# sangminwoo/SVOL

Hardware: AMD Instinct MI355X
Metric: frames/sec (fwd+matcher+bwd), T=32·P=196·d=256 (higher is better)
Workload: dtype bf16

## Files before the change

### include/svol_hip.h

```cpp
#ifndef SVOL_HIP_H
#define SVOL_HIP_H

#include <stdint.h>

#ifdef __cplusplus
extern "C" {
#endif

#define SVOL_F32 0
#define SVOL_BF16 1
#define SVOL_F16 2

#define SVOL_OK 0
#define SVOL_E_INVALID (-1)
#define SVOL_E_UNSUPPORTED (-2)
#define SVOL_E_LAUNCH (-3)

#define SVOL_ACT_NONE 0
#define SVOL_ACT_RELU 1
#define SVOL_ACT_GELU 2
#define SVOL_ACT_SIGMOID 3
#define SVOL_ACT_GELU_D 5
#define SVOL_ACT_RELU_RES 4

int svol_abi_version(void);
const char* svol_strerror(int code);

int svol_cast(const void* src, int dtype_src, void* dst, int dtype_dst, int64_t n, void* stream);
int svol_cast_transpose(const float* src, void* dst, void* dstT, int dtype, int64_t R, int64_t C, void* stream);
int svol_cast_transpose_multi(const void* descs, int32_t n_desc, int64_t total_tiles, int dtype, void* stream);
int svol_cast_split(const float* src, int64_t ld_src, void* dst_hilo, int64_t R, int64_t C, void* stream);

int svol_adamw_flat(float* p, const float* g, float* m, float* v, int64_t n, float lr, float beta1, float beta2, float eps,
                    float weight_decay, int64_t step, float grad_scale, void* stream);
int svol_adamw_flat_zero(float* p, float* g, float* m, float* v, int64_t n, float lr, float beta1, float beta2, float eps,
                         float weight_decay, int64_t step, float grad_scale, void* stream);
int svol_grad_finite(const float* g, int64_t n, float* scaler_state, void* stream);
int svol_adamw_flat_scaled(float* p, const float* g, float* m, float* v, int64_t n, float lr, float beta1, float beta2, float eps,
                           float weight_decay, float grad_mul, const float* scaler_state, void* stream);
int svol_loss_scaler_update(float* scaler_state, float growth_factor, float backoff_factor, int64_t growth_interval, float min_scale,
                            float max_scale, void* stream);
int svol_sgd_flat(float* p, const float* g, float* buf, int64_t n, float lr, float momentum, float weight_decay, float grad_scale,
                  void* stream);
int svol_sgd_flat_zero(float* p, float* g, float* buf, int64_t n, float lr, float momentum, float weight_decay, float grad_scale,
                       void* stream);
int svol_sgd_flat_scaled(float* p, const float* g, float* buf, int64_t n, float lr, float momentum, float weight_decay, float grad_mul,
                         const float* scaler_state, void* stream);
int svol_adam_flat(float* p, const float* g, float* m, float* v, int64_t n, float lr, float beta1, float beta2, float eps,
                   float weight_decay, int64_t step, float grad_scale, void* stream);
int svol_adam_flat_zero(float* p, float* g, float* m, float* v, int64_t n, float lr, float beta1, float beta2, float eps,
                        float weight_decay, int64_t step, float grad_scale, void* stream);
int svol_adam_flat_scaled(float* p, const float* g, float* m, float* v, int64_t n, float lr, float beta1, float beta2, float eps,
                          float weight_decay, float grad_mul, const float* scaler_state, void* stream);
int64_t svol_grad_sqnorm_ws_bytes(int64_t n);
int svol_grad_sqnorm(const float* g, int64_t n, float* ws, float* out, void* stream);
int svol_grad_clip_state(const float* sq, int32_t nb, float grad_mul, float max_norm, float loss_scale, int64_t steps_taken,
                         float* scaler_state, float* state_out, void* stream);
int svol_sgd_flat_grouped(float* p, float* g, float* buf, int64_t n, const int32_t* seg_end, const int32_t* seg_group, int32_t nseg,
                          const float* hyper, int32_t ngroups, const float* state, float grad_mul, int zero, void* stream);
int svol_adam_flat_grouped(float* p, float* g, float* m, float* v, int64_t n, const int32_t* seg_end, const int32_t* seg_group,
                           int32_t nseg, const float* hyper, int32_t ngroups, const float* state, const float* step_count,
                           float grad_mul, int zero, void* stream);
int svol_adamw_flat_grouped(float* p, float* g, float* m, float* v, int64_t n, const int32_t* seg_end, const int32_t* seg_group,
                            int32_t nseg, const float* hyper, int32_t ngroups, const float* state, const float* step_count,
                            float grad_mul, int zero, void* stream);
int svol_flat_step_advance(float* step_count, const float* state, void* stream);
int svol_ema_flat(float* ema, const float* p, int64_t n, float decay, int warmup, int64_t step, const float* state,
                  const float* step_count, void* stream);

int svol_gemm_nt(const void* A, int64_t lda, const void* A2, int64_t n_split, const void* B, int64_t ldb,
                 void* C, int64_t ldc, const float* bias, const float* colscale, int act, void* pre_act_out,
                 int64_t ldp, const void* residual, int64_t ldr, int out_f32, int64_t M, int64_t N, int64_t K,
                 int dtype, void* stream);
int svol_gemm_nt_split(const void* A, int64_t lda, const void* W_hilo, int64_t ldw, void* C, int64_t ldc, const float* bias,
                       int64_t M, int64_t N, int64_t K, void* stream);
int svol_gemm_nt_dgelu(const void* A, int64_t lda, const void* B, int64_t ldb, void* C, int64_t ldc,
                       const void* pre, int64_t ldp, float* colsum, int64_t M, int64_t N, int64_t K, int dtype,
                       void* stream);
int svol_gemm_nt_dact(const void* A, int64_t lda, const void* B, int64_t ldb, void* C, int64_t ldc,
                      const void* aux, int64_t ldaux, int act, float* colsum, int64_t M, int64_t N, int64_t K,
                      int dtype, void* stream);

int svol_gemm_tn(const void* A, int64_t lda, const void* B, int64_t ldb, float* C, int64_t ldc, float* colsum,
                 int64_t Mc, int64_t N, int64_t K, int dtype, void* stream);
#define SVOL_TN_GROUP_MAX 6
typedef struct svol_tn_problem {
    const void* A; int64_t lda;
    const void* B; int64_t ldb;
    float* C; int64_t ldc;
    float* colsum;
    int64_t Mc, N, K;
} svol_tn_problem;
int svol_gemm_tn_grouped(const svol_tn_problem* problems, int32_t n, int dtype, void* stream);
int svol_colsum(const void* X, int64_t ldx, float* out, int64_t M, int64_t N, int dtype, void* stream);
int svol_act_bwd(const void* dy, const void* aux, void* dpre, int act, int64_t n, int dtype, void* stream);

int svol_layernorm_fwd(const void* x, int x_f32, const float* gamma, const float* beta, float* y32, void* y,
                       void* ypos, const void* pos, int64_t pos_rows, float* mean, float* rstd, int64_t M, int64_t D,
                       float dropout_p, uint64_t seed, const int64_t* seed_offset_dev, int dtype, void* stream);
int svol_layernorm_bwd(const float* dy32, const void* dy, const void* dy2, const void* x, int x_f32,
                       const float* gamma, const float* mean, const float* rstd, float* dx32, void* dx,
                       float* dgamma, float* dbeta, float* dx_colsum, int64_t M, int64_t D, float dropout_p,
                       uint64_t seed, const int64_t* seed_offset_dev, int dtype, void* stream);

int svol_dropout(const void* x, void* y, int64_t n, int64_t row_len, float p, uint64_t seed, int dtype, void* stream);
int svol_dropout_add(const float* t32, const float* res32, float* out32, int64_t n, int64_t row_len, float p, uint64_t seed, void* stream);
int svol_dropout_sd(const void* x, void* y, int64_t n, int64_t row_len, float p, uint64_t seed, const int64_t* seed_step_dev, int dtype,
                    void* stream);
int svol_dropout_add_sd(const float* t32, const float* res32, float* out32, int64_t n, int64_t row_len, float p, uint64_t seed,
                        const int64_t* seed_step_dev, void* stream);

int svol_posenc_sine(const float* mask, void* pos, int64_t B, int64_t L, int64_t D, int dtype, void* stream);

int64_t svol_attn_ws_bytes(int64_t B, int64_t H, int64_t Lq, int64_t Lk, int64_t dh);
int svol_attn_fwd(const void* q, int64_t ldq, const void* k, int64_t ldk, const void* v, int64_t ldv, void* o,
                  int64_t ldo, float* lse2, const float* kbias, int64_t B, int64_t H, int64_t Lq, int64_t Lk,
                  int64_t dh, float scale, float q_premul, void* ws, int64_t ws_bytes, int dtype, void* stream);
int svol_attn_bwd(const void* q, int64_t ldq, const void* k, int64_t ldk, const void* v, int64_t ldv, const void* o,
                  int64_t ldo, const void* d_o, int64_t lddo, const float* lse2, float* delta, const float* kbias,
                  void* dq, int64_t lddq, void* dk, int64_t lddk, void* dv, int64_t lddv, int64_t B, int64_t H,
                  int64_t Lq, int64_t Lk, int64_t dh, float scale, float q_premul, void* ws, int64_t ws_bytes,
                  int dtype, void* stream);

#define SVOL_ATTN_DQ_PREZEROED 1
int64_t svol_attn_bwd_sp_image_bytes(int64_t B, int64_t H, int64_t Lq, int64_t Lk, int64_t dh, int64_t ws_bytes, int dtype);
int svol_attn_bwd_zero_ws(void* ws, int64_t ws_bytes, int64_t B, int64_t H, int64_t Lq, int64_t Lk, int64_t dh, int dtype, void* stream);
int svol_attn_bwd_ex(const void* q, int64_t ldq, const void* k, int64_t ldk, const void* v, int64_t ldv, const void* o,
                     int64_t ldo, const void* d_o, int64_t lddo, const float* lse2, float* delta, const float* kbias,
                     void* dq, int64_t lddq, void* dk, int64_t lddk, void* dv, int64_t lddv, int64_t B, int64_t H,
                     int64_t Lq, int64_t Lk, int64_t dh, float scale, float q_premul, void* ws, int64_t ws_bytes,
                     int dtype, int flags, void* ev_prep, void* stream);

int svol_attn_fwd_dropout(const void* q, int64_t ldq, const void* k, int64_t ldk, const void* v, int64_t ldv, void* o,
                          int64_t ldo, float* lse2, const float* kbias, int64_t B, int64_t H, int64_t Lq, int64_t Lk,
                          int64_t dh, float scale, float q_premul, void* ws, int64_t ws_bytes, float dropout_p, uint64_t seed,
                          int dtype, void* stream);
int svol_attn_bwd_dropout(const void* q, int64_t ldq, const void* k, int64_t ldk, const void* v, int64_t ldv, const void* o,
                          int64_t ldo, const void* d_o, int64_t lddo, const float* lse2, float* delta, const float* kbias,
                          void* dq, int64_t lddq, void* dk, int64_t lddk, void* dv, int64_t lddv, int64_t B, int64_t H,
                          int64_t Lq, int64_t Lk, int64_t dh, float scale, float q_premul, void* ws, int64_t ws_bytes,
                          float dropout_p, uint64_t seed, int dtype, void* stream);
int svol_attn_fwd_dropout_sd(const void* q, int64_t ldq, const void* k, int64_t ldk, const void* v, int64_t ldv, void* o,
                             int64_t ldo, float* lse2, const float* kbias, int64_t B, int64_t H, int64_t Lq, int64_t Lk,
                             int64_t dh, float scale, float q_premul, void* ws, int64_t ws_bytes, float dropout_p, uint64_t seed,
                             const int64_t* seed_step_dev, int dtype, void* stream);
int svol_attn_bwd_dropout_sd(const void* q, int64_t ldq, const void* k, int64_t ldk, const void* v, int64_t ldv, const void* o,
                             int64_t ldo, const void* d_o, int64_t lddo, const float* lse2, float* delta, const float* kbias,
                             void* dq, int64_t lddq, void* dk, int64_t lddk, void* dv, int64_t lddv, int64_t B, int64_t H,
                             int64_t Lq, int64_t Lk, int64_t dh, float scale, float q_premul, void* ws, int64_t ws_bytes,
                             float dropout_p, uint64_t seed, const int64_t* seed_step_dev, int dtype, void* stream);

int svol_gate_fwd(const float* x32, const void* pos, const float* u, const float* gamma, const float* beta,
                  float* y32, void* y, void* ypos, float* a, float* mean, float* rstd, float* ws, int64_t B,
                  int64_t L, int64_t D, int64_t H, int dtype, void* stream);
int svol_gate_bwd(const float* dy32, const void* dy, const void* dy2, const float* x32, const void* pos,
                  const float* u, const float* gamma, const float* a, const float* mean, const float* rstd,
                  const float* ws, float* ws2, float* dx32, float* du, float* dgamma, float* dbeta, int64_t B,
                  int64_t L, int64_t D, int64_t H, int dtype, void* stream);

int svol_layernorm_gate_scores_fwd(const float* x32, const float* gamma, const float* beta, float* y32, void* y, void* ypos,
                                   const void* pos, float* mean, float* rstd, const float* u_next, float* scores_next,
                                   int64_t B, int64_t L, int64_t D, int64_t H, int dtype, void* stream);
int svol_gate_fwd_scored(const float* x32, const void* pos, const float* u, const float* gamma, const float* beta,
                         float* y32, void* y, void* ypos, float* a, float* mean, float* rstd, float* ws, int64_t B,
                         int64_t L, int64_t D, int64_t H, int dtype, void* stream);

int svol_gate_vectors_fwd(const float* skch, const float* W_in, const float* b_in, float* q_out, float* u_out, int64_t B, int64_t D,
                          int64_t H, void* stream);
int svol_gate_vectors_bwd(const float* du, const float* skch, const float* W_in, const float* q, float* dq_ws, float* dskch,
                          float* dW_in, float* db_in, int64_t B, int64_t D, int64_t H, void* stream);
#define SVOL_GATE_VEC_MAX_LAYERS 8
int svol_gate_vectors_fwd_multi(const float* skch, const float* const* W_in, const float* const* b_in, float* const* q_out,
                                float* const* u_out, int64_t n_layers, int64_t B, int64_t D, int64_t H, void* stream);
int svol_gate_vectors_bwd_multi(const float* const* du, const float* skch, const float* const* W_in, const float* const* q,
                                float* const* dq_ws, float* const* dskch, float* const* dW_in, float* const* db_in, int64_t n_layers,
                                int64_t B, int64_t D, int64_t H, void* stream);

int svol_match_cost(const float* logits, const float* boxes, const float* tgt_boxes, const int32_t* pred_off,
                    const int32_t* pred_cnt, const int32_t* tgt_off, const int32_t* tgt_cnt,
                    const int64_t* cost_off, float* cost, int32_t n_problems, float w_bbox, float w_giou,
                    float w_class, int32_t* box_status, void* stream);
int svol_lsap_batched(const float* cost, const int64_t* cost_off, const int32_t* pred_off, const int32_t* pred_cnt,
                      const int32_t* tgt_off, const int32_t* tgt_cnt, int32_t* match, int32_t* status,
                      int32_t n_problems, int32_t max_dim, void* stream);
int svol_heads_fwd(const float* hs, const float* Wc, const float* bc, const float* W0, const float* b0, const float* W1, const float* b1,
                   const float* W2, const float* b2, float* logits, float* h1, float* h2, float* boxes, int64_t R, int64_t D, void* stream);
int svol_heads_bwd(const float* dlogits, const float* dboxes, const float* hs, const float* h1, const float* h2, const float* boxes,
                   const float* Wc, const float* W0, const float* W1, const float* W2, float* dhs, float* gp0, float* gp1, float* dWc,
                   float* dbc, float* dW2, float* db2, int64_t R, int64_t D, void* stream);
int svol_set_loss_bwd(const float* g_label, const float* g_bbox, const float* g_giou, const float* dl, float* dlogits, float* dboxes,
                      int64_t n_layers, int64_t rows_per_layer, void* stream);
int svol_weighted_total(const float* x, const float* w, int64_t n, float* out, void* stream);
int svol_weighted_total_bwd(const float* w, const float* dout, int64_t n, float* dx, void* stream);
int svol_lsap_solve(const double* cost, int64_t nr, int64_t nc, int64_t* rows, int64_t* cols);
int svol_set_loss(const float* logits, const float* boxes, const float* tgt_boxes, const int32_t* match,
                  float* losses, float* g_label, float* g_bbox, float* g_giou, int32_t n_layers,
                  int32_t rows_per_layer, float eos_coef, const int32_t* rebase_vid_off, int32_t rows_per_video,
                  const int32_t* status, const int32_t* box_status, int32_t problems_per_layer, void* stream);

int svol_postprocess(const float* logits, const float* boxes, float* out, int64_t B, int64_t N, int64_t chunk, void* stream);
int svol_eval_max_iou(const double* pred_box, const int32_t* pred_off, const double* gt_box, const int32_t* gt_off,
                      const int32_t* gt_rec, double* out, int64_t n_gt, int32_t k, void* stream);
int svol_eval_ap(const double* pred_box, const double* pred_score, const int32_t* pred_frame, const int32_t* grp_pred_off,
                 const double* gt_box, const int32_t* gt_frame, const int32_t* grp_gt_off, const double* thresholds,
                 int32_t n_thresholds, int32_t* ws_order, unsigned char* ws_u8, double* ws_f64, double* ap, int64_t n_pred,
                 int64_t n_gt, int64_t n_groups, void* stream);

int svol_ingest_resize(const uint8_t* src, int64_t n, int64_t H, int64_t W, int64_t s_n, int64_t s_h, int64_t s_w,
                       const int32_t* xtab, int64_t kx, const int32_t* ytab, int64_t ky, const float* lut, const uint8_t* flip,
                       void* out, int64_t o_n, int64_t o_c, int64_t o_h, int64_t o_w, int64_t OH, int64_t OW, int out_dtype,
                       void* stream);
int svol_ingest_resample(const uint8_t* src, int64_t n, int64_t H, int64_t W, int64_t s_n, int64_t s_h, int64_t s_w, int src_channels,
                         int invert, const int32_t* xtab, int64_t kx, const int32_t* ytab, int64_t ky, const float* lut,
                         const uint8_t* flip, void* out, int64_t o_n, int64_t o_c, int64_t o_h, int64_t o_w, int64_t OH, int64_t OW,
                         int out_dtype, void* stream);

int svol_patchify(const float* pixel_values, void* out, int64_t n, int64_t C, int64_t H, int64_t W, int64_t p, int dtype,
                  void* stream);
int svol_vit_embed(const float* patch_proj, const float* cls_token, const float* pos_embed, float* x32, void* x, int64_t n,
                   int64_t P, int64_t D, int dtype, void* stream);
int svol_im2col(const void* x, int64_t sn, int64_t sh, int64_t sw, int64_t sc, int src_dtype, void* cols, int64_t ldcols,
                int64_t N, int64_t H, int64_t W, int64_t C, int64_t kh, int64_t kw, int64_t stride, int64_t pad, int dtype,
                void* stream);
int svol_conv_nhwc(const void* x, const void* w, int64_t ldw, void* y, const float* bias, int act, const void* residual,
                   int64_t N, int64_t H, int64_t W, int64_t C, int64_t Cout, int64_t kh, int64_t kw, int64_t stride,
                   int64_t pad, int dtype, void* stream);
int svol_maxpool_nhwc(const void* x, void* y, int64_t N, int64_t H, int64_t W, int64_t C, int64_t k, int64_t stride,
                      int64_t pad, int dtype, void* stream);
int svol_avgpool_nhwc(const void* x, float* y, int64_t N, int64_t HW, int64_t C, int dtype, void* stream);
int svol_bn_colstats(const void* z, const float* shift, float shift_scale, float* sum, float* sumsq, int64_t M, int64_t C, int dtype,
                     void* stream);
int svol_bn_finalize(const float* sum, const float* sumsq_centered, const float* pivot, const float* gamma, const float* beta,
                     float* running_mean, float* running_var, float momentum, float eps, int64_t M, int64_t C, float* mean, float* rstd,
                     float* scale, float* shift, void* stream);
int svol_conv_weight_pack(const float* w, void* out, int64_t Cout, int64_t Cin, int64_t kh, int64_t kw, int64_t Kp, int flip, int dtype,
                          void* stream);
int svol_conv_weight_unpack_add(const float* dwp, float* grad, int64_t Cout, int64_t Cin, int64_t kh, int64_t kw, int64_t Kp, void* stream);
int svol_conv_wgrad_nhwc(const void* dz, const void* x, float* dwp, int64_t N, int64_t H, int64_t W, int64_t C, int64_t Cout, int64_t kh, int64_t kw,
                         int64_t stride, int64_t pad, int64_t Kp, int dtype, void* stream);
int svol_bn_apply(const void* z, const float* scale, const float* shift, const void* residual, int relu, void* y, int64_t M, int64_t C,
                  int dtype, void* stream);
int svol_bn_bwd_reduce(const void* dy, const void* y, const void* z, const float* mean, const float* rstd, float* sum_g, float* sum_gx,
                       int64_t M, int64_t C, int dtype, void* stream);
int svol_bn_bwd_apply(const void* dy, const void* y, const void* z, const float* mean, const float* rstd, const float* gamma,
                      const float* sum_g, const float* sum_gx, void* dz, void* dres, int64_t M, int64_t C, int dtype, void* stream);
int svol_col2im_nhwc(const void* dcols, int64_t ldcols, void* dx, int64_t N, int64_t H, int64_t W, int64_t C, int64_t kh, int64_t kw,
                     int64_t stride, int64_t pad, int dtype, void* stream);
int svol_maxpool_idx_nhwc(const void* x, void* y, uint8_t* idx, int64_t N, int64_t H, int64_t W, int64_t C, int64_t k, int64_t stride,
                          int64_t pad, int dtype, void* stream);
int svol_maxpool_bwd_nhwc(const void* dy, const uint8_t* idx, void* dx, int64_t N, int64_t H, int64_t W, int64_t C, int64_t k,
                          int64_t stride, int64_t pad, int dtype, void* stream);
int svol_attn_weights_mean(const void* q, int64_t ldq, const void* k, int64_t ldk, const float* lse2, const float* kbias,
                           float* att, int64_t B, int64_t H, int64_t Lq, int64_t Lk, int64_t dh, float scale,
                           float q_premul, int dtype, void* stream);
int svol_attn_small_fwd(const void* q, int64_t ldq, const void* k, int64_t ldk, const void* v, int64_t ldv, void* o, int64_t ldo,
                        int64_t n_seq, int64_t H, int64_t L, int64_t dh, float scale, int dtype, void* stream);
int svol_attn_small_fwd_lse(const void* q, int64_t ldq, const void* k, int64_t ldk, const void* v, int64_t ldv, void* o, int64_t ldo,
                            float* lse2, int64_t n_seq, int64_t H, int64_t L, int64_t dh, float scale, int dtype, void* stream);
int svol_attn_small_bwd(const void* q, int64_t ldq, const void* k, int64_t ldk, const void* v, int64_t ldv, const void* o, int64_t ldo,
                        const void* dout, int64_t lddo, const float* lse2, void* dq, int64_t lddq, void* dk, int64_t lddk, void* dv,
                        int64_t lddv, int64_t n_seq, int64_t H, int64_t L, int64_t dh, float scale, int dtype, void* stream);
int svol_attn_small_fwd_h16(const void* q, int64_t ldq, const void* k, int64_t ldk, const void* v, int64_t ldv, void* o, int64_t ldo,
                            int64_t n_seq, int64_t H, int64_t L, int64_t dh, float scale, int dtype, void* stream);
int svol_attn_small_fwd_lse_h16(const void* q, int64_t ldq, const void* k, int64_t ldk, const void* v, int64_t ldv, void* o, int64_t ldo,
                                float* lse2, int64_t n_seq, int64_t H, int64_t L, int64_t dh, float scale, int dtype, void* stream);
int svol_attn_small_bwd_h16(const void* q, int64_t ldq, const void* k, int64_t ldk, const void* v, int64_t ldv, const void* o, int64_t ldo,
                            const void* dout, int64_t lddo, const float* lse2, void* dq, int64_t lddq, void* dk, int64_t lddk, void* dv,
                            int64_t lddv, int64_t n_seq, int64_t H, int64_t L, int64_t dh, float scale, int dtype, void* stream);

int svol_attn_cls_fwd(const void* q, int64_t ldq, const void* k, int64_t ldk, const void* v, int64_t ldv, void* o, int64_t ldo, float* lse2,
                      int64_t n, int64_t H, int64_t L, int64_t dh, float scale, int dtype, void* stream);
int svol_attn_cls_bwd(const void* q, int64_t ldq, const void* k, int64_t ldk, const void* v, int64_t ldv, const void* o, int64_t ldo,
                      const void* dout, int64_t lddo, const float* lse2, void* dq, int64_t lddq, void* dk, int64_t lddk, void* dv,
                      int64_t lddv, int64_t n, int64_t H, int64_t L, int64_t dh, float scale, int dtype, void* stream);
int svol_attn_cls_fwd_h16(const void* q, int64_t ldq, const void* k, int64_t ldk, const void* v, int64_t ldv, void* o, int64_t ldo, float* lse2,
                          int64_t n, int64_t H, int64_t L, int64_t dh, float scale, int dtype, void* stream);
int svol_attn_cls_bwd_h16(const void* q, int64_t ldq, const void* k, int64_t ldk, const void* v, int64_t ldv, const void* o, int64_t ldo,
                          const void* dout, int64_t lddo, const float* lse2, void* dq, int64_t lddq, void* dk, int64_t lddk, void* dv,
                          int64_t lddv, int64_t n, int64_t H, int64_t L, int64_t dh, float scale, int dtype, void* stream);
int64_t svol_attn_fewkeys_chunk_rows(int64_t Lq);
int64_t svol_attn_fewkeys_ws_bytes(int64_t B, int64_t H, int64_t Lq, int64_t Lk, int64_t dh);
int svol_attn_fewkeys_fwd(const void* q, int64_t ldq, const void* k, int64_t ldk, const void* v, int64_t ldv, void* o, int64_t ldo, float* lse2,
                          const float* kbias, int64_t B, int64_t H, int64_t Lq, int64_t Lk, int64_t dh, float scale, float q_premul, int dtype,
                          void* stream);
int svol_attn_fewkeys_bwd(const void* q, int64_t ldq, const void* k, int64_t ldk, const void* v, int64_t ldv, const void* o, int64_t ldo,
                          const void* d_o, int64_t lddo, const float* lse2, const float* kbias, void* dq, int64_t lddq, void* dk, int64_t lddk,
                          void* dv, int64_t lddv, int64_t B, int64_t H, int64_t Lq, int64_t Lk, int64_t dh, float scale, float q_premul,
                          void* ws, int64_t ws_bytes, int dtype, void* stream);
int svol_softmax_xent(const float* logits, int64_t ld, const int64_t* targets, float* loss, float* dlogits, int64_t lddl, int32_t* correct,
                      int64_t n, int64_t C, void* stream);


#define SVOL_DIM_B 0
#define SVOL_DIM_L 1
#define SVOL_DIM_N 2
#define SVOL_DIM_D 3
#define SVOL_DIM_H 4
#define SVOL_DIM_F 5
#define SVOL_DIM_DTYPE 6
#define SVOL_DIM_QDTYPE 7
#define SVOL_DIM_ATTN_WS_BYTES 8
#define SVOL_DIM_COUNT 9

#define SVOL_BLK_VIDEO_HALF 0
#define SVOL_BLK_QUERY_SELF 1
#define SVOL_BLK_QUERY_CROSS 2
const char* svol_block_slot_names(int block);
int svol_block_trace_dump(char* buf, int64_t cap);
int svol_clock_probe(uint64_t* samples, int32_t* count, int32_t max_samples, const int32_t* stop, int64_t period_us,
                     int64_t max_ms, int32_t* wall_khz, void* stream);


#define SVOL_VH_SLOTS(X) \
    X(X32) X(POS) X(U) X(G1) X(BT1) X(G2) X(BT2) X(G3) X(BT3) X(B_IN) X(B_O) X(B_FC1) X(B_FC2) X(QSCALE) \
    X(W_IN) X(WV_HILO) X(W_O) X(W_FC1) X(W_FC2) X(W_IN_T) X(W_O_T) X(W_FC1_T) X(W_FC2_T) \
    X(Y1) X(Y1POS) X(A) X(MEAN1) X(RSTD1) X(GATE_WS) X(GATE_PRE) X(U_NEXT) X(GATE_WS_NEXT) \
    X(QKV) X(O) X(LSE) X(S2) X(Y2) X(MEAN2) X(RSTD2) X(PRE) X(HID) X(S3) \
    X(MEAN3) X(RSTD3) X(M32) X(M) X(MPOS) X(Y1_32) X(Y2_32) X(ATTN_WS) \
    X(DM32) X(DM) X(DMPOS) X(DS32_3) X(DS3) X(DPRE) X(DY2) X(DS32_2) X(G2D) X(DO) X(DQKV) X(DELTA) X(DXQP) X(DXQ) X(GATE_WS2) \
    X(DX32) X(DU) \
    X(DG1) X(DBT1) X(DG2) X(DBT2) X(DG3) X(DBT3) X(DW_IN) X(DB_IN) X(DW_O) X(DB_O) X(DW_FC1) X(DB_FC1) X(DW_FC2) X(DB_FC2) \
    X(EV_A0) X(EV_A1) X(EV_CLEAN_IN) X(EV_PREP) X(ATTN_WS_NEXT) X(ZERO_STREAM) X(EV_CLEAN_OUT)
#define SVOL_QS_SLOTS(X) \
    X(O32) X(O) X(OPOS) X(QPOS) X(B_IN) X(B_O) X(G4) X(BT4) X(QSCALE) X(W_IN) X(WV_HILO) X(W_O) X(W_IN_T) X(W_O_T) \
    X(QKV) X(OA) X(LSE) X(S4) X(MEAN4) X(RSTD4) X(Y32) X(Y) X(YPOS) X(ATTN_WS) \
    X(DY32) X(DY) X(DYPOS) X(G) X(DOA) X(DQKV) X(DELTA) X(DO32) X(DXQ) X(DXQP) X(DQPOS) \
    X(DW_IN) X(DB_IN) X(DW_O) X(DB_O) X(DG4) X(DBT4)
#define SVOL_QC_SLOTS(X) \
    X(O32) X(O) X(OPOS) X(MV) X(MPOS) X(KBIAS) X(QPOS) X(B_IN) X(B_O) X(G5) X(BT5) X(B_FC1) X(B_FC2) X(G6) X(BT6) X(QSCALE) \
    X(W_INQ) X(W_INQ_T) X(W_KV) X(W_KV_T) X(WV_HILO) X(W_O) X(W_O_T) X(W_FC1) X(W_FC1_T) X(W_FC2) X(W_FC2_T) \
    X(Q) X(QC) X(KV) X(OA) X(OAQ) X(LSE) X(S5) X(Y5_32) X(Y5) X(MEAN5) X(RSTD5) X(PRE) X(HID) X(S6) X(MEAN6) X(RSTD6) \
    X(Y32) X(Y) X(YPOS) X(ATTN_WS) \
    X(DY32) X(DY) X(DYPOS) X(DS32_6) X(DS6) X(DPRE) X(DY5) X(DS32_5) X(G5D) X(DOAQ) X(DOA) X(DQC) X(DQ) X(DKV) X(DELTA) \
    X(DO32) X(DXQP) X(DMPOS) X(DMV) X(DQPOS) \
    X(DW_IN) X(DB_IN) X(DW_O) X(DB_O) X(DG5) X(DBT5) X(DW_FC1) X(DB_FC1) X(DW_FC2) X(DB_FC2) X(DG6) X(DBT6)
#define SVOL_SLOT_ENUM_VH(n) SVOL_VH_##n,
#define SVOL_SLOT_ENUM_QS(n) SVOL_QS_##n,
#define SVOL_SLOT_ENUM_QC(n) SVOL_QC_##n,
enum { SVOL_VH_SLOTS(SVOL_SLOT_ENUM_VH) SVOL_VH_COUNT };
enum { SVOL_QS_SLOTS(SVOL_SLOT_ENUM_QS) SVOL_QS_COUNT };
enum { SVOL_QC_SLOTS(SVOL_SLOT_ENUM_QC) SVOL_QC_COUNT };

int svol_video_half_fwd(const int64_t* dims, void* const* slots, void* stream);
int svol_video_half_bwd(const int64_t* dims, void* const* slots, int phase, void* stream);
int svol_video_half_wgrad(const int64_t* dims, void* const* slots, void* stream);
int svol_video_half_wgrad_part(const int64_t* dims, void* const* slots, int part, void* stream);
int svol_query_self_fwd(const int64_t* dims, void* const* slots, void* stream);
int svol_query_self_bwd(const int64_t* dims, void* const* slots, void* stream);
int svol_query_self_wgrad(const int64_t* dims, void* const* slots, void* stream);
int svol_query_cross_fwd(const int64_t* dims, void* const* slots, void* stream);
int svol_query_cross_bwd(const int64_t* dims, void* const* slots, void* stream);
int svol_query_cross_wgrad(const int64_t* dims, void* const* slots, void* stream);

#ifdef __cplusplus
}
#endif
#endif
```

### svol_amd/_lib.py

```python
from __future__ import annotations

import ctypes
import os

_HERE = os.path.dirname(os.path.abspath(__file__))
LIB_PATH = os.path.join(_HERE, 'libsvol_hip.so')

_p = ctypes.c_void_p
_i64 = ctypes.c_int64
_i32 = ctypes.c_int32
_int = ctypes.c_int
_f32 = ctypes.c_float
_u64 = ctypes.c_uint64

SIGNATURES = {
    'svol_block_trace_dump': [ctypes.c_char_p, _i64],
    'svol_lsap_solve': [_p, _i64, _i64, _p, _p],
    'svol_heads_fwd': [_p] * 13 + [_i64, _i64, _p],
    'svol_heads_bwd': [_p] * 17 + [_i64, _i64, _p],
    'svol_set_loss_bwd': [_p] * 6 + [_i64, _i64, _p],
    'svol_weighted_total': [_p, _p, _i64, _p, _p],
    'svol_weighted_total_bwd': [_p, _p, _i64, _p, _p],
    'svol_cast': [_p, _int, _p, _int, _i64, _p],
    'svol_cast_transpose': [_p, _p, _p, _int, _i64, _i64, _p],
    'svol_cast_split': [_p, _i64, _p, _i64, _i64, _p],
    'svol_gemm_nt_split': [_p, _i64, _p, _i64, _p, _i64, _p, _i64, _i64, _i64, _p],
    'svol_gemm_nt': [_p, _i64, _p, _i64, _p, _i64, _p, _i64, _p, _p, _int, _p, _i64, _p, _i64, _int, _i64, _i64, _i64,
                     _int, _p],
    'svol_gemm_nt_dgelu': [_p, _i64, _p, _i64, _p, _i64, _p, _i64, _p, _i64, _i64, _i64, _int, _p],
    'svol_gemm_nt_dact': [_p, _i64, _p, _i64, _p, _i64, _p, _i64, _int, _p, _i64, _i64, _i64, _int, _p],
    'svol_gemm_tn': [_p, _i64, _p, _i64, _p, _i64, _p, _i64, _i64, _i64, _int, _p],
    'svol_gemm_tn_grouped': [_p, _i32, _int, _p],
    'svol_colsum': [_p, _i64, _p, _i64, _i64, _int, _p],
    'svol_act_bwd': [_p, _p, _p, _int, _i64, _int, _p],
    'svol_layernorm_fwd': [_p, _int, _p, _p, _p, _p, _p, _p, _i64, _p, _p, _i64, _i64, _f32, _u64, _p, _int, _p],
    'svol_layernorm_bwd': [_p, _p, _p, _p, _int, _p, _p, _p, _p, _p, _p, _p, _p, _i64, _i64, _f32, _u64, _p, _int, _p],
    'svol_cast_transpose_multi': [_p, _int, _i64, _int, _p],
    'svol_postprocess': [_p, _p, _p, _i64, _i64, _i64, _p],
    'svol_eval_max_iou': [_p, _p, _p, _p, _p, _p, _i64, _int, _p],
    'svol_eval_ap': [_p, _p, _p, _p, _p, _p, _p, _p, _int, _p, _p, _p, _p, _i64, _i64, _i64, _p],
    'svol_patchify': [_p, _p, _i64, _i64, _i64, _i64, _i64, _int, _p],
    'svol_vit_embed': [_p, _p, _p, _p, _p, _i64, _i64, _i64, _int, _p],
    'svol_ingest_resize': [_p, _i64, _i64, _i64, _i64, _i64, _i64, _p, _i64, _p, _i64, _p, _p, _p, _i64, _i64, _i64, _i64, _i64, _i64, _int, _p],
    'svol_ingest_resample': [_p, _i64, _i64, _i64, _i64, _i64, _i64, _int, _int, _p, _i64, _p, _i64, _p, _p, _p, _i64, _i64, _i64, _i64, _i64, _i64, _int, _p],
    'svol_adamw_flat': [_p, _p, _p, _p, _i64, _f32, _f32, _f32, _f32, _f32, _i64, _f32, _p],
    'svol_adamw_flat_zero': [_p, _p, _p, _p, _i64, _f32, _f32, _f32, _f32, _f32, _i64, _f32, _p],
    'svol_grad_finite': [_p, _i64, _p, _p],
    'svol_adamw_flat_scaled': [_p, _p, _p, _p, _i64, _f32, _f32, _f32, _f32, _f32, _f32, _p, _p],
    'svol_loss_scaler_update': [_p, _f32, _f32, _i64, _f32, _f32, _p],
    'svol_sgd_flat': [_p, _p, _p, _i64, _f32, _f32, _f32, _f32, _p],
    'svol_sgd_flat_zero': [_p, _p, _p, _i64, _f32, _f32, _f32, _f32, _p],
    'svol_sgd_flat_scaled': [_p, _p, _p, _i64, _f32, _f32, _f32, _f32, _p, _p],
    'svol_adam_flat': [_p, _p, _p, _p, _i64, _f32, _f32, _f32, _f32, _f32, _i64, _f32, _p],
    'svol_adam_flat_zero': [_p, _p, _p, _p, _i64, _f32, _f32, _f32, _f32, _f32, _i64, _f32, _p],
    'svol_adam_flat_scaled': [_p, _p, _p, _p, _i64, _f32, _f32, _f32, _f32, _f32, _f32, _p, _p],
    'svol_grad_sqnorm_ws_bytes': [_i64],
    'svol_grad_sqnorm': [_p, _i64, _p, _p, _p],
    'svol_grad_clip_state': [_p, _i32, _f32, _f32, _f32, _i64, _p, _p, _p],
    'svol_sgd_flat_grouped': [_p, _p, _p, _i64, _p, _p, _i32, _p, _i32, _p, _f32, _int, _p],
    'svol_adam_flat_grouped': [_p, _p, _p, _p, _i64, _p, _p, _i32, _p, _i32, _p, _p, _f32, _int, _p],
    'svol_adamw_flat_grouped': [_p, _p, _p, _p, _i64, _p, _p, _i32, _p, _i32, _p, _p, _f32, _int, _p],
    'svol_flat_step_advance': [_p, _p, _p],
    'svol_ema_flat': [_p, _p, _i64, _f32, _int, _i64, _p, _p, _p],
    'svol_conv_nhwc': [_p, _p, _i64, _p, _p, _int, _p, _i64, _i64, _i64, _i64, _i64, _i64, _i64, _i64, _i64, _int, _p],
    'svol_im2col': [_p, _i64, _i64, _i64, _i64, _int, _p, _i64, _i64, _i64, _i64, _i64, _i64, _i64, _i64, _i64, _int, _p],
    'svol_maxpool_nhwc': [_p, _p, _i64, _i64, _i64, _i64, _i64, _i64, _i64, _int, _p],
    'svol_avgpool_nhwc': [_p, _p, _i64, _i64, _i64, _int, _p],
    'svol_bn_colstats': [_p, _p, _f32, _p, _p, _i64, _i64, _int, _p],
    'svol_bn_finalize': [_p, _p, _p, _p, _p, _p, _p, _f32, _f32, _i64, _i64, _p, _p, _p, _p, _p],
    'svol_conv_weight_pack': [_p, _p, _i64, _i64, _i64, _i64, _i64, _int, _int, _p],
    'svol_conv_weight_unpack_add': [_p, _p, _i64, _i64, _i64, _i64, _i64, _p],
    'svol_conv_wgrad_nhwc': [_p, _p, _p, _i64, _i64, _i64, _i64, _i64, _i64, _i64, _i64, _i64, _i64, _int, _p],
    'svol_bn_apply': [_p, _p, _p, _p, _int, _p, _i64, _i64, _int, _p],
    'svol_bn_bwd_reduce': [_p, _p, _p, _p, _p, _p, _p, _i64, _i64, _int, _p],
    'svol_bn_bwd_apply': [_p, _p, _p, _p, _p, _p, _p, _p, _p, _p, _i64, _i64, _int, _p],
    'svol_col2im_nhwc': [_p, _i64, _p, _i64, _i64, _i64, _i64, _i64, _i64, _i64, _i64, _int, _p],
    'svol_maxpool_idx_nhwc': [_p, _p, _p, _i64, _i64, _i64, _i64, _i64, _i64, _i64, _int, _p],
    'svol_maxpool_bwd_nhwc': [_p, _p, _p, _i64, _i64, _i64, _i64, _i64, _i64, _i64, _int, _p],
    'svol_attn_weights_mean': [_p, _i64, _p, _i64, _p, _p, _p, _i64, _i64, _i64, _i64, _i64, _f32, _f32, _int, _p],
    'svol_attn_small_fwd': [_p, _i64, _p, _i64, _p, _i64, _p, _i64, _i64, _i64, _i64, _i64, _f32, _int, _p],
    'svol_attn_small_fwd_lse': [_p, _i64, _p, _i64, _p, _i64, _p, _i64, _p, _i64, _i64, _i64, _i64, _f32, _int, _p],
    'svol_attn_small_bwd': [_p, _i64, _p, _i64, _p, _i64, _p, _i64, _p, _i64, _p, _p, _i64, _p, _i64, _p, _i64, _i64, _i64, _i64,
                            _i64, _f32, _int, _p],
    'svol_attn_cls_fwd': [_p, _i64, _p, _i64, _p, _i64, _p, _i64, _p, _i64, _i64, _i64, _i64, _f32, _int, _p],
    'svol_attn_cls_bwd': [_p, _i64, _p, _i64, _p, _i64, _p, _i64, _p, _i64, _p, _p, _i64, _p, _i64, _p, _i64, _i64, _i64, _i64,
                          _i64, _f32, _int, _p],
    'svol_attn_small_fwd_h16': [_p, _i64, _p, _i64, _p, _i64, _p, _i64, _i64, _i64, _i64, _i64, _f32, _int, _p],
    'svol_attn_small_fwd_lse_h16': [_p, _i64, _p, _i64, _p, _i64, _p, _i64, _p, _i64, _i64, _i64, _i64, _f32, _int, _p],
    'svol_attn_small_bwd_h16': [_p, _i64, _p, _i64, _p, _i64, _p, _i64, _p, _i64, _p, _p, _i64, _p, _i64, _p, _i64, _i64, _i64, _i64,
                                _i64, _f32, _int, _p],
    'svol_attn_cls_fwd_h16': [_p, _i64, _p, _i64, _p, _i64, _p, _i64, _p, _i64, _i64, _i64, _i64, _f32, _int, _p],
    'svol_attn_cls_bwd_h16': [_p, _i64, _p, _i64, _p, _i64, _p, _i64, _p, _i64, _p, _p, _i64, _p, _i64, _p, _i64, _i64, _i64, _i64,
                              _i64, _f32, _int, _p],
    'svol_attn_fewkeys_chunk_rows': [_i64],
    'svol_attn_fewkeys_ws_bytes': [_i64, _i64, _i64, _i64, _i64],
    'svol_attn_fewkeys_fwd': [_p, _i64, _p, _i64, _p, _i64, _p, _i64, _p, _p, _i64, _i64, _i64, _i64, _i64, _f32, _f32, _int, _p],
    'svol_attn_fewkeys_bwd': [_p, _i64, _p, _i64, _p, _i64, _p, _i64, _p, _i64, _p, _p, _p, _i64, _p, _i64, _p, _i64,
                              _i64, _i64, _i64, _i64, _i64, _f32, _f32, _p, _i64, _int, _p],
    'svol_softmax_xent': [_p, _i64, _p, _p, _p, _i64, _p, _i64, _i64, _p],
    'svol_posenc_sine': [_p, _p, _i64, _i64, _i64, _int, _p],
    'svol_attn_ws_bytes': [_i64, _i64, _i64, _i64, _i64],
    'svol_attn_fwd': [_p, _i64, _p, _i64, _p, _i64, _p, _i64, _p, _p, _i64, _i64, _i64, _i64, _i64, _f32, _f32, _p, _i64,
                      _int, _p],
    'svol_attn_bwd': [_p, _i64, _p, _i64, _p, _i64, _p, _i64, _p, _i64, _p, _p, _p, _p, _i64, _p, _i64, _p, _i64,
                      _i64, _i64, _i64, _i64, _i64, _f32, _f32, _p, _i64, _int, _p],
    'svol_attn_bwd_ex': [_p, _i64, _p, _i64, _p, _i64, _p, _i64, _p, _i64, _p, _p, _p, _p, _i64, _p, _i64, _p, _i64,
                         _i64, _i64, _i64, _i64, _i64, _f32, _f32, _p, _i64, _int, _int, _p, _p],
    'svol_attn_bwd_sp_image_bytes': [_i64, _i64, _i64, _i64, _i64, _i64, _int],
    'svol_attn_bwd_zero_ws': [_p, _i64, _i64, _i64, _i64, _i64, _i64, _int, _p],
    'svol_attn_fwd_dropout': [_p, _i64, _p, _i64, _p, _i64, _p, _i64, _p, _p, _i64, _i64, _i64, _i64, _i64, _f32, _f32, _p, _i64,
                              _f32, _u64, _int, _p],
    'svol_attn_bwd_dropout': [_p, _i64, _p, _i64, _p, _i64, _p, _i64, _p, _i64, _p, _p, _p, _p, _i64, _p, _i64, _p, _i64,
                              _i64, _i64, _i64, _i64, _i64, _f32, _f32, _p, _i64, _f32, _u64, _int, _p],
    'svol_dropout': [_p, _p, _i64, _i64, _f32, _u64, _int, _p],
    'svol_dropout_add': [_p, _p, _p, _i64, _i64, _f32, _u64, _p],
    'svol_attn_fwd_dropout_sd': [_p, _i64, _p, _i64, _p, _i64, _p, _i64, _p, _p, _i64, _i64, _i64, _i64, _i64, _f32, _f32, _p, _i64,
                                 _f32, _u64, _p, _int, _p],
    'svol_attn_bwd_dropout_sd': [_p, _i64, _p, _i64, _p, _i64, _p, _i64, _p, _i64, _p, _p, _p, _p, _i64, _p, _i64, _p, _i64,
                                 _i64, _i64, _i64, _i64, _i64, _f32, _f32, _p, _i64, _f32, _u64, _p, _int, _p],
    'svol_dropout_sd': [_p, _p, _i64, _i64, _f32, _u64, _p, _int, _p],
    'svol_dropout_add_sd': [_p, _p, _p, _i64, _i64, _f32, _u64, _p, _p],
    'svol_gate_fwd': [_p, _p, _p, _p, _p, _p, _p, _p, _p, _p, _p, _p, _i64, _i64, _i64, _i64, _int, _p],
    'svol_gate_bwd': [_p, _p, _p, _p, _p, _p, _p, _p, _p, _p, _p, _p, _p, _p, _p, _p, _i64, _i64, _i64, _i64, _int,
                      _p],
    'svol_clock_probe': [_p, _p, _int, _p, _i64, _i64, _p, _p],
    'svol_gate_fwd_scored': [_p, _p, _p, _p, _p, _p, _p, _p, _p, _p, _p, _p, _i64, _i64, _i64, _i64, _int, _p],
    'svol_layernorm_gate_scores_fwd': [_p, _p, _p, _p, _p, _p, _p, _p, _p, _p, _p, _i64, _i64, _i64, _i64, _int, _p],
    'svol_gate_vectors_fwd': [_p, _p, _p, _p, _p, _i64, _i64, _i64, _p],
    'svol_gate_vectors_bwd': [_p, _p, _p, _p, _p, _p, _p, _p, _i64, _i64, _i64, _p],
    'svol_gate_vectors_fwd_multi': [_p, _p, _p, _p, _p, _i64, _i64, _i64, _i64, _p],
    'svol_gate_vectors_bwd_multi': [_p, _p, _p, _p, _p, _p, _p, _p, _i64, _i64, _i64, _i64, _p],
    'svol_match_cost': [_p, _p, _p, _p, _p, _p, _p, _p, _p, _i32, _f32, _f32, _f32, _p, _p],
    'svol_lsap_batched': [_p, _p, _p, _p, _p, _p, _p, _p, _i32, _i32, _p],
    'svol_set_loss': [_p, _p, _p, _p, _p, _p, _p, _p, _i32, _i32, _f32, _p, _i32, _p, _p, _i32, _p],
    'svol_video_half_fwd': [_p, _p, _p],
    'svol_video_half_bwd': [_p, _p, _int, _p],
    'svol_video_half_wgrad': [_p, _p, _p],
    'svol_video_half_wgrad_part': [_p, _p, _int, _p],
    'svol_query_self_fwd': [_p, _p, _p],
    'svol_query_self_bwd': [_p, _p, _p],
    'svol_query_self_wgrad': [_p, _p, _p],
    'svol_query_cross_fwd': [_p, _p, _p],
    'svol_query_cross_bwd': [_p, _p, _p],
    'svol_query_cross_wgrad': [_p, _p, _p],
}



class TnProblem(ctypes.Structure):
    _fields_ = [('A', _p), ('lda', _i64), ('B', _p), ('ldb', _i64), ('C', _p), ('ldc', _i64), ('colsum', _p),
                ('Mc', _i64), ('N', _i64), ('K', _i64)]


_LIB = None


class SvolHipError(RuntimeError):
    pass


def lib():
    global _LIB
    if _LIB is None:
        if not os.path.exists(LIB_PATH):
            raise SvolHipError(
                f'{LIB_PATH} not found: the SVOL hot path has no CPU fallback. '
                'Build it with `python -m svol_amd.build` (hipcc, gfx950).')
        L = ctypes.CDLL(LIB_PATH)
        L.svol_abi_version.restype = _int
        L.svol_abi_version.argtypes = []
        L.svol_strerror.restype = ctypes.c_char_p
        L.svol_strerror.argtypes = [_int]
        for name, at in SIGNATURES.items():
            f = getattr(L, name)
            f.restype = _int
            f.argtypes = at
        L.svol_attn_ws_bytes.restype = _i64
        L.svol_attn_bwd_sp_image_bytes.restype = _i64
        L.svol_grad_sqnorm_ws_bytes.restype = _i64
        L.svol_attn_fewkeys_chunk_rows.restype = _i64
        L.svol_attn_fewkeys_ws_bytes.restype = _i64
        L.svol_block_slot_names.restype = ctypes.c_char_p
        L.svol_block_slot_names.argtypes = [_int]
        _LIB = L
    return _LIB


def check(rc: int, name: str):
    if rc != 0:
        msg = lib().svol_strerror(rc).decode()
        raise SvolHipError(f'{name} failed: {msg} (code {rc})')
```

### svol_amd/blocks.py

```python
from __future__ import annotations

import ctypes
import math
import os
import weakref

import torch

from . import _lib, layers, ops, params, wgrad

ENABLED = os.environ.get('SVOL_NO_BLOCKS') is None
GATE_SCORES_FUSE = os.environ.get('SVOL_GATE_SCORES_FUSE') is not None
VH, QS, QC = 0, 1, 2
_F32, _BF16 = 0, 1
_ESZ = {torch.float32: 4, torch.bfloat16: 2, torch.float16: 2}
_SLOTS = {}


def _slots(block):
    m = _SLOTS.get(block)
    if m is None:
        names = _lib.lib().svol_block_slot_names(block).decode().rstrip(',').split(',')
        m = _SLOTS[block] = {n: i for i, n in enumerate(names)}
    return m
# ... 30 lines not shown
            self.off[name] = (n, nbytes)
            n += _align(nbytes)
        self.total = max(n, 256)

    def fill(self, tbl, base):
        for name, (o, _) in self.off.items():
            tbl.arr[tbl.idx[name]] = base + o

    def view(self, arena, name, dtype, shape):
        o, nb = self.off[name]
        return arena[o:o + nb].view(dtype).view(shape)


_LAYOUTS = {}


def _layout(key, make):
    lay = _LAYOUTS.get(key)
    if lay is None:
        lay = _LAYOUTS[key] = _Layout(make())
    return lay


_SCRATCH = {}


def _scratch(dev, nbytes):
    key = (dev, ops._stream())
    t = _SCRATCH.get(key)
    if t is None or t.numel() < nbytes:
        t = _SCRATCH[key] = torch.empty((_align(nbytes, 1 << 20),), dtype=torch.uint8, device=dev)
    return t


def _dims(B, L, N, D, H, F, dt, qdt, ws_bytes):
    return (ctypes.c_int64 * 9)(B, L, N, D, H, F, ops._DT[dt], ops._DT[qdt], ws_bytes)


def _c(t):
    return t if t is None or t.is_contiguous() else t.contiguous()


_VH_PARAMS = [
    ('DG1', lambda l: l.norm1.weight), ('DBT1', lambda l: l.norm1.bias),
    ('DW_IN', lambda l: l.content_self_attn.in_proj_weight), ('DB_IN', lambda l: l.content_self_attn.in_proj_bias),
    ('DW_O', lambda l: l.content_self_attn.out_proj.weight), ('DB_O', lambda l: l.content_self_attn.out_proj.bias),
    ('DG2', lambda l: l.norm2.weight), ('DBT2', lambda l: l.norm2.bias),
    ('DW_FC1', lambda l: l.mlp1.fc1.weight), ('DB_FC1', lambda l: l.mlp1.fc1.bias),
    ('DW_FC2', lambda l: l.mlp1.fc2.weight), ('DB_FC2', lambda l: l.mlp1.fc2.bias),
    ('DG3', lambda l: l.norm3.weight), ('DBT3', lambda l: l.norm3.bias)]
_QS_PARAMS = [
    ('DW_IN', lambda l: l.token_self_attn.in_proj_weight), ('DB_IN', lambda l: l.token_self_attn.in_proj_bias),
    ('DW_O', lambda l: l.token_self_attn.out_proj.weight), ('DB_O', lambda l: l.token_self_attn.out_proj.bias),
    ('DG4', lambda l: l.norm4.weight), ('DBT4', lambda l: l.norm4.bias)]
_QC_PARAMS = [
    ('DW_IN', lambda l: l.content_token_cross_attn.in_proj_weight), ('DB_IN', lambda l: l.content_token_cross_attn.in_proj_bias),
    ('DW_O', lambda l: l.content_token_cross_attn.out_proj.weight), ('DB_O', lambda l: l.content_token_cross_attn.out_proj.bias),
    ('DG5', lambda l: l.norm5.weight), ('DBT5', lambda l: l.norm5.bias),
    ('DW_FC1', lambda l: l.mlp2.fc1.weight), ('DB_FC1', lambda l: l.mlp2.fc1.bias),
    ('DW_FC2', lambda l: l.mlp2.fc2.weight), ('DB_FC2', lambda l: l.mlp2.fc2.bias),
    ('DG6', lambda l: l.norm6.weight), ('DBT6', lambda l: l.norm6.bias)]
_PARAMS = {VH: _VH_PARAMS, QS: _QS_PARAMS, QC: _QC_PARAMS}


class BlockPlan:

    def __init__(self, block, layer, dt, qdt):
        self.block, self.dt, self.qdt = block, dt, qdt
        self.layer = weakref.ref(layer)
        self.params = [g(layer) for _, g in _PARAMS[block]]
        self.grad_slots = [n for n, _ in _PARAMS[block]]
        self.tpl = _Table(block)
        self.keep = []
        D = layer.d_model
        self.split_v = params.SPLIT_V and D % 32 == 0
        t = self.tpl
        W = params.weights
        dev = self.params[0].device

        self.casts = []
        self.epoch = W.epoch

        def both(name, w, dtype):
            got = wc, wt = W.get(w, dtype)
            t.set_t(name, wc)
            t.set_t(name + '_T', wt)
            self.keep += [wc, wt]
            self.casts.append((W.get, (w, dtype), got))

        wdt = dt if block == VH else qdt
        adt = qdt if block == QS else dt
        for slot, p in zip(self.grad_slots, self.params):
            if p.dim() == 1:
                t.set_t(slot[1:], p)
            elif block == QC and slot == 'DW_IN':
                both('W_INQ', p, qdt)
                both('W_KV', p, dt)
            else:
                both(slot[1:], p, wdt)
        if adt == torch.bfloat16 and self.split_v:
            w_in = self.params[self.grad_slots.index('DW_IN')]
            hl = W.get_split(w_in, 2 * D, D)
            t.set_t('WV_HILO', hl)
            self.keep.append(hl)
            self.casts.append((W.get_split, (w_in, 2 * D, D), hl))
        if adt != torch.float32:
            q = layers._qscale(D, layers.LOG2E / math.sqrt(D // layer.nhead), dev)
            t.set_t('QSCALE', q)
            self.keep.append(q)
        self.sinks = [params.claim(p, p.requires_grad) for p in self.params]
        self.nosink = [(i, p.numel()) for i, (p, s) in enumerate(zip(self.params, self.sinks)) if s is None]
        for name, s in zip(self.grad_slots, self.sinks):
            if s is not None:
                t.set_t(name, s.view)
        self.graph_params = self.params if (self.nosink or any(s.owner is None for s in self.sinks)) else []
        cnt = {}
        for s in self.sinks:
            if s is not None and s.owner is not None:
                cnt[(id(s.owner), s.bucket)] = (s.owner, s.bucket, cnt.get((id(s.owner), s.bucket), (None, None, 0))[2] + 1)
        self.notify = list(cnt.values())
        self.key = self._key()

    def _key(self):
        k = []
        for p in self.params:
            g = p.grad
            s = getattr(p, '_svol_sink', None)
            k.append((p.data_ptr(), g.data_ptr() if (g is not None and s is not None) else 0, p.requires_grad))
        return (params.SPLIT_V, tuple(k))

    def valid(self):
        return self.layer() is not None and self._key() == self.key

    def fresh_copies(self):
        for again, args, got in self.casts:
            if again(*args) is not got:
                return False
        return True

    def grad_buffers(self, tbl, dev):
        if not self.nosink:
            return None
        offs, n = [], 0
        for _, numel in self.nosink:
            offs.append(n)
            n += (numel + 3) // 4 * 4
        flat = torch.zeros((n,), dtype=torch.float32, device=dev)
        out = {}
        base = flat.data_ptr()
        for (i, numel), o in zip(self.nosink, offs):
            tbl.set(self.grad_slots[i], base + o * 4)
            out[i] = flat[o:o + numel].view_as(self.params[i])
        return out

    def inputs(self, *tensors):
        if self.graph_params or not any(t_.requires_grad for t_ in tensors):
            return self.params
        return ()

    def done(self, in_graph):
        if not in_graph:
            for owner, bi, n in self.notify:
                owner.params_done(bi, n)

    def grads_out(self, bufs, needs, in_graph):
        res = []
        if not in_graph:
            return res
        for i, p in enumerate(self.params):
            if bufs is not None and i in bufs and needs[i]:
                res.append(bufs[i])
            else:
                res.append(None)
        return res


_PLANS = weakref.WeakKeyDictionary()


def plan(layer, block, dt, qdt):
    per = _PLANS.get(layer)
    if per is None:
        per = _PLANS[layer] = {}
    k = (block, dt, qdt)
    pl = per.get(k)
    if pl is None or not pl.valid() or not pl.fresh_copies():
        pl = per[k] = BlockPlan(block, layer, dt, qdt)
    return pl


def _call(name, ctx, *extra, stream=None):
    rc = getattr(_lib.lib(), name)(ctx.dims, ctx.tbl.arr, *extra, ops._stream() if stream is None else stream)
    _lib.check(rc, name)


def _open(ctx, pl, block, key, dims, n_par, dev, fwd_items, scr_items, **inputs):
    ctx.set_materialize_grads(False)
    lay = _layout(('f', block) + key, fwd_items)
    slay = _layout(('s', block) + key, scr_items)
    arena = torch.empty((lay.total,), dtype=torch.uint8, device=dev)
    tbl = _Table(block, pl.tpl)
    lay.fill(tbl, arena.data_ptr())
    slay.fill(tbl, _scratch(dev, slay.total).data_ptr())
    for name, t in inputs.items():
        tbl.set(name, t.data_ptr())
    ctx.pl, ctx.tbl, ctx.dims, ctx.arena, ctx.key, ctx.n_par = pl, tbl, dims, arena, (block,) + key, n_par
    return lay


def _no_grads(ctx, n_in):
    ctx.pl.done(ctx.n_par > 0)
    return (None,) * (n_in + ctx.n_par)


def _open_bwd(ctx, dev, bwd_items, **grads):
    tbl = ctx.tbl
    lay = _layout(('b',) + ctx.key, bwd_items)
    tmp = torch.empty((lay.total,), dtype=torch.uint8, device=dev)
    lay.fill(tbl, tmp.data_ptr())
    gs = []
    for name, g in grads.items():
        g = _c(g)
        tbl.set_t(name, g)
        if g is not None:
            gs.append(g)
    slay = _layout(('s',) + ctx.key, None)
    slay.fill(tbl, _scratch(dev, slay.total).data_ptr())
    return lay, tmp, ctx.pl.grad_buffers(tbl, dev), gs


def _close_bwd(ctx, name, bufs, keep, n_in):
    if bufs is not None or not wgrad.issue(lambda ws: _call(name, ctx, stream=ws.cuda_stream), keep, ops._current_stream_obj()):
        _call(name, ctx)
    in_graph = ctx.n_par > 0
    ctx.pl.done(in_graph)
    return tuple(ctx.pl.grads_out(bufs, ctx.needs_input_grad[n_in:], in_graph))


def _maybe_events(name, meta):
    tm = ops.timer
    if not tm.enabled or name not in tm.names:
        return None
    e0, e1 = torch.cuda.Event(enable_timing=True), torch.cuda.Event(enable_timing=True)
    e0.record()
    e1.record()
    tm.records.setdefault((name, meta), []).append((e0, e1))
    return e0, e1


DQ_PREZERO = os.environ.get('SVOL_DQ_PREZERO') is not None and os.environ.get('SVOL_NO_DQ_PREZERO') is None
_DQ_PREZERO = {}


class _DqPrezero:
    __slots__ = ('bufs', 'side', 'ev_prep', 'clean_ev', 'clean', 'nxt')

    def __init__(self, dev, wsb):
        self.bufs = [torch.empty((_align(wsb, 1 << 20),), dtype=torch.uint8, device=dev) for _ in range(2)]
        self.side = torch.cuda.Stream(device=dev)
        self.ev_prep = torch.cuda.Event()
        self.clean_ev = [torch.cuda.Event(), torch.cuda.Event()]
        for e_ in [self.ev_prep] + self.clean_ev:
            e_.record()
        self.clean = [False, False]
        self.nxt = 0

    def bind(self, tbl):
        i = self.nxt
        tbl.set('ATTN_WS', self.bufs[i].data_ptr())
        tbl.set('EV_CLEAN_IN', self.clean_ev[i].cuda_event if self.clean[i] else None)
        tbl.set('EV_PREP', self.ev_prep.cuda_event)
        tbl.set('ATTN_WS_NEXT', self.bufs[1 - i].data_ptr())
        tbl.set('ZERO_STREAM', self.side.cuda_stream)
        tbl.set('EV_CLEAN_OUT', self.clean_ev[1 - i].cuda_event)
        self.clean[i] = False

    def advance(self, tbl):
        i = self.nxt
        self.clean[1 - i] = True
        self.nxt = 1 - i
        for n_ in ('EV_CLEAN_IN', 'EV_PREP', 'ATTN_WS_NEXT', 'ZERO_STREAM', 'EV_CLEAN_OUT'):
            tbl.set(n_, None)


def _dq_prezero(dev, B, H, L, dh, dt, wsb):
    if not DQ_PREZERO or dt == torch.float32 or torch.cuda.is_current_stream_capturing():
        return None
    key = (dev, ops._stream(), B, H, L, dh, dt, wsb)
    st = _DQ_PREZERO.get(key)
    if st is None:
        img = _lib.lib().svol_attn_bwd_sp_image_bytes(B, H, L, L, dh, wsb, ops._DT[dt])
        st = _DQ_PREZERO[key] = _DqPrezero(dev, wsb) if img > 0 else False
    return st or None


def _vh_fwd_layout(B, L, D, H, F, e):
    M = B * L
    return [('Y1', M * D * e), ('Y1POS', M * D * e), ('A', M * 4), ('MEAN1', M * 4), ('RSTD1', M * 4), ('GATE_WS', B * H * (L + 2) * 4),
            ('QKV', M * 3 * D * e), ('O', M * D * e), ('LSE', B * H * L * 4), ('S2', M * D * 4), ('Y2', M * D * e), ('MEAN2', M * 4),
            ('RSTD2', M * 4), ('PRE', M * F * e), ('HID', M * F * e), ('S3', M * D * 4), ('MEAN3', M * 4), ('RSTD3', M * 4),
            ('M32', M * D * 4), ('M', M * D * e), ('MPOS', M * D * e)]


def _vh_bwd_layout(B, L, D, H, F, e):
    M = B * L
    return [('DS32_3', M * D * 4), ('DS3', M * D * e), ('DPRE', M * F * e), ('DY2', M * D * e), ('DS32_2', M * D * 4), ('G2D', M * D * e),
            ('DO', M * D * e), ('DQKV', M * 3 * D * e), ('DELTA', 3 * B * H * L * 4), ('DXQ', M * D * e),
            ('GATE_WS2', (B * L + B * H) * 4), ('DX32', M * D * 4)]


def _attn_events(tbl, ev):
    tbl.set('EV_A0', ev[0].cuda_event if ev else None)
    tbl.set('EV_A1', ev[1].cuda_event if ev else None)


class VideoHalfFn(torch.autograd.Function):

    @staticmethod
    def forward(ctx, pl, x32, pos, u, u_next, sc_in, *params):
        B, L, D = x32.shape
        layer = pl.layer()
        H, F = layer.nhead, layer.mlp1.fc1.weight.shape[0]
        dt = pl.dt
        e = _ESZ[dt]
        dev = x32.device
        M = B * L
        x2, pos2, u = _c(x32.reshape(M, D)), _c(pos.reshape(M, D)), _c(u)
        assert x2.dtype == torch.float32 and pos2.dtype == dt and u.dtype == torch.float32
        wsb = ops.attn_ws_bytes(dt, B, H, L, L, D // H)
        lay = _open(ctx, pl, VH, (B, L, D, H, F, dt), _dims(B, L, 0, D, H, F, dt, dt, wsb), len(params), dev,
                    lambda: _vh_fwd_layout(B, L, D, H, F, e),
                    lambda: [('Y1_32', M * D * 4), ('Y2_32', M * D * 4), ('ATTN_WS', max(wsb, 16))], X32=x2, POS=pos2, U=u)
        tbl = ctx.tbl
        if sc_in is not None:
            assert sc_in.dtype == torch.float32 and sc_in.numel() == B * H * (L + 2) and sc_in.is_contiguous()
            tbl.set('GATE_WS', sc_in.data_ptr())
            tbl.set('GATE_PRE', sc_in.data_ptr())
        if u_next is not None:
            u_next = u_next.contiguous()
            assert u_next.dtype == torch.float32 and u_next.shape == u.shape and L % 4 == 0
            sc_next = torch.empty((B * H * (L + 2),), dtype=torch.float32, device=dev)
            tbl.set('U_NEXT', u_next.data_ptr())
            tbl.set('GATE_WS_NEXT', sc_next.data_ptr())
        else:
            sc_next = torch.empty((0,), dtype=torch.float32, device=dev)
        ctx.big = wgrad.attn_forward(B * H * L * L)
        _attn_events(tbl, _maybe_events('attn_fwd', (B, H, L, L, D // H)))
        _call('svol_video_half_fwd', ctx)
        _attn_events(tbl, None)
        tbl.set('U_NEXT', None)
        tbl.set('GATE_WS_NEXT', None)
        ctx.shape = (B, L, D, H, F)
        ctx.sc_in = sc_in
        ctx.save_for_backward(x2, pos2, u)
        ctx.mark_non_differentiable(sc_next)
        return (lay.view(ctx.arena, 'M32', torch.float32, (B, L, D)), lay.view(ctx.arena, 'M', dt, (B, L, D)),
                lay.view(ctx.arena, 'MPOS', dt, (B, L, D)), sc_next)

    @staticmethod
    def backward(ctx, dm32, dm, dmpos, _dsc=None):
        if dm32 is None and dm is None and dmpos is None:
            return _no_grads(ctx, 6)
        tbl = ctx.tbl
        B, L, D, H, F = ctx.shape
        dt = ctx.pl.dt
        dev = ctx.saved_tensors[0].device
        du = torch.zeros((B, H, D), dtype=torch.float32, device=dev)
        tbl.set('DU', du.data_ptr())
        lay, tmp, bufs, gs = _open_bwd(ctx, dev, lambda: _vh_bwd_layout(B, L, D, H, F, _ESZ[dt]), DM32=dm32, DM=dm, DMPOS=dmpos)
        _call('svol_video_half_bwd', ctx, 1)
        wgrad.attn_backward(B * H * L * L)
        _attn_events(tbl, _maybe_events('attn_bwd', (B, H, L, L, D // H)))
        pz = _dq_prezero(dev, B, H, L, D // H, dt, ctx.dims[8]) if ctx.big else None
        if pz is not None:
            pz.bind(tbl)
        _call('svol_video_half_bwd', ctx, 2)
        if pz is not None:
            pz.advance(tbl)
        _attn_events(tbl, None)
        pg = _close_bwd(ctx, 'svol_video_half_wgrad', bufs, [ctx.arena, tmp] + gs, 6)
        dx32 = lay.view(tmp, 'DX32', torch.float32, (B, L, D))
        return (None, dx32, None, du if ctx.needs_input_grad[3] else None, None, None) + pg


def gate_scores_fusable(L, D, H):
    return GATE_SCORES_FUSE and L % 4 == 0 and D % 4 == 0 and D <= 256 and H <= 8


def video_half(layer, x32, pos, u, dt, u_next=None, sc_in=None):
    pl = plan(layer, VH, dt, dt)
    if u_next is not None and not gate_scores_fusable(x32.shape[1], x32.shape[2], layer.nhead):
        u_next = None
    m32, m, mpos, sc = VideoHalfFn.apply(pl, x32, pos, u, u_next, sc_in, *pl.inputs(x32, u))
    return m32, m, mpos, (sc if u_next is not None else None)


def _qpos_target(ctx, qpos, need, N, D):
    g = s = None
    if need and qpos.requires_grad:
        s = params.claim(qpos, True) if (qpos.is_leaf and qpos.dtype == torch.float32) else None
        if s is None:
            g = torch.zeros((N, D), dtype=torch.float32, device=qpos.device)
    ctx.tbl.set_t('DQPOS', s.view if s is not None else g)
    return g


def _qpos_grad(g, qdt):
    return ops.cast(g, qdt) if (g is not None and qdt != torch.float32) else g


class QuerySelfFn(torch.autograd.Function):

    @staticmethod
    def forward(ctx, pl, o32, o, opos, qpos, *params):
        B, N, D = o.shape
        H, qdt = pl.layer().nhead, pl.qdt
        e, R = _ESZ[qdt], B * N
        o32_, o_, opos_, qpos_ = _c(o32), _c(o), _c(opos), _c(qpos)
        assert o32_.dtype == torch.float32 and o_.dtype == qdt and opos_.dtype == qdt and qpos_.dtype == qdt
        wsb = ops.attn_ws_bytes(qdt, B, H, N, N, D // H)
        lay = _open(ctx, pl, QS, (B, N, D, H, qdt), _dims(B, 0, N, D, H, 0, qdt, qdt, wsb), len(params), o.device,
                    lambda: [('QKV', R * 3 * D * e), ('OA', R * D * e), ('LSE', B * H * N * 4), ('S4', R * D * 4), ('MEAN4', R * 4),
                             ('RSTD4', R * 4), ('Y32', R * D * 4), ('Y', R * D * e), ('YPOS', R * D * e)],
                    lambda: [('ATTN_WS', max(wsb, 16))], O32=o32_, O=o_, OPOS=opos_, QPOS=qpos_)
        _call('svol_query_self_fwd', ctx)
        ctx.shape = (B, N, D, H)
        ctx.save_for_backward(o32_, o_, opos_, qpos)
        return (lay.view(ctx.arena, 'Y32', torch.float32, (B, N, D)), lay.view(ctx.arena, 'Y', qdt, (B, N, D)),
                lay.view(ctx.arena, 'YPOS', qdt, (B, N, D)))

    @staticmethod
    def backward(ctx, dy32, dy, dypos):
        if dy32 is None and dy is None and dypos is None:
            return _no_grads(ctx, 5)
        B, N, D, H = ctx.shape
        o32_, o_, opos_, qpos = ctx.saved_tensors
        qdt = ctx.pl.qdt
        e, R = _ESZ[qdt], B * N
        gq = _qpos_target(ctx, qpos, ctx.needs_input_grad[4], N, D)
        lay, tmp, bufs, gs = _open_bwd(ctx, o_.device, lambda: [('G', R * D * e), ('DOA', R * D * e), ('DQKV', R * 3 * D * e),
                                                               ('DELTA', 3 * B * H * N * 4), ('DO32', R * D * 4), ('DXQ', R * D * e),
                                                               ('DXQP', R * D * e)], DY32=dy32, DY=dy, DYPOS=dypos)
        _call('svol_query_self_bwd', ctx)
        pg = _close_bwd(ctx, 'svol_query_self_wgrad', bufs, [ctx.arena, tmp, o_, opos_], 5)
        v = lambda n_, dt_: lay.view(tmp, n_, dt_, (B, N, D))
        return (None, v('DO32', torch.float32), v('DXQ', qdt), v('DXQP', qdt), _qpos_grad(gq, qdt)) + pg


def query_self(layer, out, qpos, dt, qdt):
    pl = plan(layer, QS, dt, qdt)
    o32, o, opos = out
    return QuerySelfFn.apply(pl, o32, o, opos, qpos, *pl.inputs(o32, o, opos))


def _qc_fwd_layout(B, N, L, D, H, F, e, qe):
    R, M = B * N, B * L
    return [('Q', R * D * qe), ('QC', R * D * e), ('KV', M * 2 * D * e), ('OA', R * D * e), ('OAQ', R * D * qe), ('LSE', B * H * N * 4),
            ('S5', R * D * 4), ('Y5_32', R * D * 4), ('Y5', R * D * qe), ('MEAN5', R * 4), ('RSTD5', R * 4), ('PRE', R * F * qe),
            ('HID', R * F * qe), ('S6', R * D * 4), ('MEAN6', R * 4), ('RSTD6', R * 4), ('Y32', R * D * 4), ('Y', R * D * qe),
            ('YPOS', R * D * qe)]


def _qc_bwd_layout(B, N, L, D, H, F, e, qe, merged):
    R, M = B * N, B * L
    return [('DS32_6', R * D * 4), ('DS6', R * D * qe), ('DPRE', R * F * qe), ('DY5', R * D * qe), ('G5D', R * D * qe), ('DOAQ', R * D * qe),
            ('DOA', R * D * e), ('DQC', R * D * e), ('DQ', R * D * qe), ('DKV', M * 2 * D * e), ('DELTA', 3 * B * H * N * 4),
            ('DO32', R * D * 4), ('DXQP', R * D * qe)] + ([] if merged else [('DMPOS', M * D * e)]) + [('DMV', M * D * e)]


class QueryCrossFn(torch.autograd.Function):

    @staticmethod
    def forward(ctx, pl, o32, o, opos, mv, mpos, kbias, qpos, merged, *params):
        B, N, D = o.shape
        L = mv.shape[1]
        layer = pl.layer()
        H, F = layer.nhead, layer.mlp2.fc1.weight.shape[0]
        dt, qdt = pl.dt, pl.qdt
        e, qe = _ESZ[dt], _ESZ[qdt]
        o32_, o_, opos_, mv_, mpos_, kb_, qpos_ = _c(o32), _c(o), _c(opos), _c(mv), _c(mpos), _c(kbias), _c(qpos)
        assert o32_.dtype == torch.float32 and o_.dtype == qdt and opos_.dtype == qdt and qpos_.dtype == qdt
        assert mv_.dtype == dt and mpos_.dtype == dt and kb_.dtype == torch.float32
        wsb = ops.attn_ws_bytes(dt, B, H, N, L, D // H)
        lay = _open(ctx, pl, QC, (B, N, L, D, H, F, dt, qdt, merged), _dims(B, L, N, D, H, F, dt, qdt, wsb), len(params), o.device,
                    lambda: _qc_fwd_layout(B, N, L, D, H, F, e, qe), lambda: [('ATTN_WS', max(wsb, 16))],
                    O32=o32_, O=o_, OPOS=opos_, MV=mv_, MPOS=mpos_, KBIAS=kb_, QPOS=qpos_)
        _call('svol_query_cross_fwd', ctx)
        ctx.shape = (B, N, L, D, H, F)
        ctx.merged = merged
        ctx.save_for_backward(o32_, o_, opos_, mv_, mpos_, kb_, qpos)
        return (lay.view(ctx.arena, 'Y32', torch.float32, (B, N, D)), lay.view(ctx.arena, 'Y', qdt, (B, N, D)),
                lay.view(ctx.arena, 'YPOS', qdt, (B, N, D)))

    @staticmethod
    def backward(ctx, dy32, dy, dypos):
        if dy32 is None and dy is None and dypos is None:
            return _no_grads(ctx, 9)
        B, N, L, D, H, F = ctx.shape
        o32_, o_, opos_, mv_, mpos_, kb_, qpos = ctx.saved_tensors
        dt, qdt = ctx.pl.dt, ctx.pl.qdt
        gq = _qpos_target(ctx, qpos, ctx.needs_input_grad[7], N, D)
        lay, tmp, bufs, gs = _open_bwd(ctx, o_.device, lambda: _qc_bwd_layout(B, N, L, D, H, F, _ESZ[dt], _ESZ[qdt], ctx.merged),
                                       DY32=dy32, DY=dy, DYPOS=dypos)
        _call('svol_query_cross_bwd', ctx)
        pg = _close_bwd(ctx, 'svol_query_cross_wgrad', bufs, [ctx.arena, tmp, opos_, mv_, mpos_], 9)
        vq = lambda n_, dt_: lay.view(tmp, n_, dt_, (B, N, D))
        vm = lambda n_: lay.view(tmp, n_, dt, (B, L, D))
        return (None, vq('DO32', torch.float32), None, vq('DXQP', qdt), vm('DMV'), None if ctx.merged else vm('DMPOS'), None,
                _qpos_grad(gq, qdt), None) + pg


def query_cross(layer, out, mv, mpos, kbias, qpos, dt, qdt):
    pl = plan(layer, QC, dt, qdt)
    o32, o, opos = out
    fn = mv.grad_fn
    merged = fn is not None and fn is mpos.grad_fn and isinstance(fn, VideoHalfFn._backward_cls)
    return QueryCrossFn.apply(pl, o32, o, opos, mv, mpos, kbias, qpos, merged, *pl.inputs(o32, opos, mv, mpos))


def trace_dump() -> str:
    buf = ctypes.create_string_buffer(1 << 20)
    _lib.check(_lib.lib().svol_block_trace_dump(buf, len(buf)), 'svol_block_trace_dump')
    return buf.value.decode()
```

### svol_amd/csrc/blocks.hip

```cpp
#include <math.h>
#include <stdio.h>
#include <stdlib.h>
#include <string.h>

#include <map>
#include <mutex>
#include <string>
#include <vector>

#include "common.h"

namespace {

const bool kTrace = getenv("SVOL_BLOCK_TRACE") != nullptr;
struct TraceRec { const char* prog; const char* site; hipEvent_t e0, e1; };
std::mutex g_trace_mu;
std::vector<TraceRec> g_trace_log;
struct Trace {
    const char* prog;
    hipStream_t s;
    hipEvent_t last = nullptr;
    Trace* prev;
    static thread_local Trace* cur;
    Trace(const char* prog_, void* s_) : prog(prog_), s(static_cast<hipStream_t>(s_)), prev(cur) {
        cur = this;
        if (kTrace && hipEventCreate(&last) == hipSuccess) (void)hipEventRecord(last, s);
    }
    ~Trace() { cur = prev; }
    void mark(const char* site) {
        if (!kTrace || !last) return;
        hipEvent_t e;
        if (hipEventCreate(&e) != hipSuccess) return;
        (void)hipEventRecord(e, s);
        std::lock_guard<std::mutex> lk(g_trace_mu);
        g_trace_log.push_back({prog, site, last, e});
        last = e;
    }
};
thread_local Trace* Trace::cur = nullptr;

struct Dims {
    int64_t B, L, N, D, H, F, ws_bytes;
    int dt, qdt;
    explicit Dims(const int64_t* d)
        : B(d[SVOL_DIM_B]), L(d[SVOL_DIM_L]), N(d[SVOL_DIM_N]), D(d[SVOL_DIM_D]), H(d[SVOL_DIM_H]), F(d[SVOL_DIM_F]),
          ws_bytes(d[SVOL_DIM_ATTN_WS_BYTES]), dt((int)d[SVOL_DIM_DTYPE]), qdt((int)d[SVOL_DIM_QDTYPE]) {}
    bool ok() const {
        return B > 0 && D > 0 && H > 0 && D % H == 0 && (dt == SVOL_F32 || svol_is16(dt)) && (qdt == SVOL_F32 || svol_is16(qdt));
    }
};

inline int esz(int dtype) { return svol_is16(dtype) ? 2 : 4; }
inline void* at(void* p, int64_t elems, int dtype) { return p ? static_cast<char*>(p) + elems * esz(dtype) : nullptr; }
inline const void* at(const void* p, int64_t elems, int dtype) { return p ? static_cast<const char*>(p) + elems * esz(dtype) : nullptr; }
inline float* f32(void* p) { return static_cast<float*>(p); }

inline float attn_scale(int64_t dh) { return (float)(1.0 / sqrt((double)dh)); }
inline float attn_premul(int64_t dh, int dtype) { return svol_is16(dtype) ? (float)(1.4426950408889634 / sqrt((double)dh)) : 0.f; }

inline int nt(const void* A, int64_t lda, const void* W, int64_t ldw, void* C, int64_t ldc, const void* bias, const void* colscale,
              int64_t M, int64_t N, int64_t K, int dtype, void* s) {
    return svol_gemm_nt(A, lda, nullptr, 0, W, ldw, C, ldc, static_cast<const float*>(bias), static_cast<const float*>(colscale),
                        SVOL_ACT_NONE, nullptr, 0, nullptr, 0, 0, M, N, K, dtype, s);
}
inline int nt_res(const void* A, int64_t lda, const void* W, int64_t ldw, void* C32, const void* bias, const void* res32, int64_t M,
                  int64_t N, int64_t K, int dtype, void* s) {
    return svol_gemm_nt(A, lda, nullptr, 0, W, ldw, C32, N, static_cast<const float*>(bias), nullptr, SVOL_ACT_NONE, nullptr, 0, res32, N,
                        1, M, N, K, dtype, s);
}

#define RUN(expr)                                 \
    do {                                          \
        const int rc_ = (expr);                   \
        if (rc_) return rc_;                      \
        if (kTrace && Trace::cur) Trace::cur->mark(#expr); \
    } while (0)

#define SLOT_NAME(n) #n ","
const char* const kVhNames = SVOL_VH_SLOTS(SLOT_NAME);
const char* const kQsNames = SVOL_QS_SLOTS(SLOT_NAME);
const char* const kQcNames = SVOL_QC_SLOTS(SLOT_NAME);

inline void record(void* ev, void* stream) {
    if (ev) (void)hipEventRecord(static_cast<hipEvent_t>(ev), static_cast<hipStream_t>(stream));
}

}


extern "C" {

int svol_block_trace_dump(char* buf, int64_t cap) {
    if (!buf || cap <= 0) return SVOL_E_INVALID;
    buf[0] = 0;
    if (!kTrace) return SVOL_OK;
    if (hipDeviceSynchronize() != hipSuccess) return SVOL_E_LAUNCH;
    std::lock_guard<std::mutex> lk(g_trace_mu);
    static const bool timeline = getenv("SVOL_BLOCK_TRACE") && atoi(getenv("SVOL_BLOCK_TRACE")) == 2;
    if (timeline && !g_trace_log.empty()) {
        std::string out;
        char line[256];
        const hipEvent_t ref = g_trace_log.front().e0;
        for (const TraceRec& r : g_trace_log) {
            float t0 = 0.f, t1 = 0.f;
            if (hipEventElapsedTime(&t0, ref, r.e0) != hipSuccess || hipEventElapsedTime(&t1, ref, r.e1) != hipSuccess) continue;
            std::string site(r.site);
            const size_t c = site.find(',');
            if (c != std::string::npos) site.resize(c);
            snprintf(line, sizeof line, "%9.3f %9.3f  %-20s %s\n", t0, t1, r.prog, site.c_str());
            out += line;
        }
        std::map<hipEvent_t, int> seen_;
        for (const TraceRec& r : g_trace_log) { seen_[r.e0] = 1; seen_[r.e1] = 1; }
        for (auto& kv : seen_) (void)hipEventDestroy(kv.first);
        g_trace_log.clear();
        strncpy(buf, out.c_str(), (size_t)cap - 1);
        buf[cap - 1] = 0;
        return SVOL_OK;
    }
    std::map<std::string, std::pair<double, int>> acc;
    std::vector<std::string> order;
    std::map<hipEvent_t, int> seen;
    for (const TraceRec& r : g_trace_log) {
        float ms = 0.f;
        if (hipEventElapsedTime(&ms, r.e0, r.e1) != hipSuccess) continue;
        std::string site(r.site);
        const size_t c = site.find(',');
        if (c != std::string::npos) site.resize(c);
        const std::string key = std::string(r.prog) + " | " + site;
        if (!acc.count(key)) order.push_back(key);
        acc[key].first += ms;
        acc[key].second += 1;
    }
    for (const TraceRec& r : g_trace_log) { seen[r.e0] = 1; seen[r.e1] = 1; }
    for (auto& kv : seen) (void)hipEventDestroy(kv.first);
    g_trace_log.clear();
    std::string out;
    char line[256];
    for (const std::string& k : order) {
        snprintf(line, sizeof line, "%-110s calls %6d  avg_us %9.1f  total_ms %9.3f\n", k.c_str(), acc[k].second,
                 acc[k].first / acc[k].second * 1e3, acc[k].first);
        out += line;
    }
    strncpy(buf, out.c_str(), (size_t)cap - 1);
    buf[cap - 1] = 0;
    return SVOL_OK;
}

const char* svol_block_slot_names(int block) {
    switch (block) {
        case SVOL_BLK_VIDEO_HALF: return kVhNames;
        case SVOL_BLK_QUERY_SELF: return kQsNames;
        case SVOL_BLK_QUERY_CROSS: return kQcNames;
        default: return "";
    }
}

int svol_video_half_fwd(const int64_t* dims, void* const* p, void* s) {
    if (!dims || !p) return SVOL_E_INVALID;
    Trace tr_("video_half_fwd", s);
    const Dims d(dims);
    if (!d.ok() || d.L <= 0 || d.F <= 0) return SVOL_E_INVALID;
    const int64_t M = d.B * d.L, D = d.D, F = d.F, dh = D / d.H;
    const int dt = d.dt, xf = dt != SVOL_F32;
#define P(n) p[SVOL_VH_##n]
    if (P(GATE_PRE))
        RUN(svol_gate_fwd_scored(f32(P(X32)), P(POS), f32(P(U)), f32(P(G1)), f32(P(BT1)), f32(P(Y1_32)), P(Y1), P(Y1POS), f32(P(A)),
                                 f32(P(MEAN1)), f32(P(RSTD1)), f32(P(GATE_WS)), d.B, d.L, D, d.H, dt, s));
    else
        RUN(svol_gate_fwd(f32(P(X32)), P(POS), f32(P(U)), f32(P(G1)), f32(P(BT1)), f32(P(Y1_32)), P(Y1), P(Y1POS), f32(P(A)), f32(P(MEAN1)),
                          f32(P(RSTD1)), f32(P(GATE_WS)), d.B, d.L, D, d.H, dt, s));
    RUN(nt(P(Y1POS), D, P(W_IN), D, P(QKV), 3 * D, P(B_IN), P(QSCALE), M, 2 * D, D, dt, s));
    if (P(WV_HILO))
        RUN(svol_gemm_nt_split(P(Y1), D, P(WV_HILO), 2 * D, at(P(QKV), 2 * D, dt), 3 * D, f32(P(B_IN)) + 2 * D, M, D, D, s));
    else
        RUN(nt(P(Y1), D, at(P(W_IN), 2 * D * D, dt), D, at(P(QKV), 2 * D, dt), 3 * D, f32(P(B_IN)) + 2 * D, nullptr, M, D, D, dt, s));
    record(P(EV_A0), s);
    RUN(svol_attn_fwd(P(QKV), 3 * D, at(P(QKV), D, dt), 3 * D, at(P(QKV), 2 * D, dt), 3 * D, P(O), D, f32(P(LSE)), nullptr, d.B, d.H, d.L,
                      d.L, dh, attn_scale(dh), attn_premul(dh, dt), P(ATTN_WS), d.ws_bytes, dt, s));
    record(P(EV_A1), s);
    RUN(nt_res(P(O), D, P(W_O), D, P(S2), P(B_O), P(Y1_32), M, D, D, dt, s));
    RUN(svol_layernorm_fwd(P(S2), xf, f32(P(G2)), f32(P(BT2)), f32(P(Y2_32)), P(Y2), nullptr, nullptr, 0, f32(P(MEAN2)), f32(P(RSTD2)), M,
                           D, 0.f, 0, nullptr, dt, s));
    RUN(svol_gemm_nt(P(Y2), D, nullptr, 0, P(W_FC1), D, P(HID), F, f32(P(B_FC1)), nullptr, SVOL_ACT_GELU_D, P(PRE), F, nullptr, 0, 0, M, F, D, dt, s));
    RUN(nt_res(P(HID), F, P(W_FC2), F, P(S3), P(B_FC2), P(Y2_32), M, D, F, dt, s));
    if (P(U_NEXT) && P(GATE_WS_NEXT))
        RUN(svol_layernorm_gate_scores_fwd(f32(P(S3)), f32(P(G3)), f32(P(BT3)), f32(P(M32)), P(M), P(MPOS), P(POS), f32(P(MEAN3)),
                                           f32(P(RSTD3)), f32(P(U_NEXT)), f32(P(GATE_WS_NEXT)), d.B, d.L, D, d.H, dt, s));
    else
        RUN(svol_layernorm_fwd(P(S3), xf, f32(P(G3)), f32(P(BT3)), f32(P(M32)), P(M), P(MPOS), P(POS), M, f32(P(MEAN3)), f32(P(RSTD3)), M, D,
                               0.f, 0, nullptr, dt, s));
    return SVOL_OK;
}

int svol_video_half_bwd(const int64_t* dims, void* const* p, int phase, void* s) {
    if (!dims || !p || phase < 0 || phase > 2) return SVOL_E_INVALID;
    Trace tr_(phase == 2 ? "video_half_bwd.2" : "video_half_bwd.1", s);
    const Dims d(dims);
    if (!d.ok() || d.L <= 0 || d.F <= 0) return SVOL_E_INVALID;
    const int64_t M = d.B * d.L, D = d.D, F = d.F, dh = D / d.H;
    const int dt = d.dt, xf = dt != SVOL_F32;
    if (phase != 2) {
        RUN(svol_layernorm_bwd(f32(P(DM32)), P(DM), P(DMPOS), P(S3), xf, f32(P(G3)), f32(P(MEAN3)), f32(P(RSTD3)), f32(P(DS32_3)), P(DS3),
                               f32(P(DG3)), f32(P(DBT3)), f32(P(DB_FC2)), M, D, 0.f, 0, nullptr, dt, s));
        RUN(svol_gemm_nt_dact(P(DS3), D, P(W_FC2_T), D, P(DPRE), F, P(PRE), F, SVOL_ACT_GELU_D, f32(P(DB_FC1)), M, F, D, dt, s));
        RUN(nt(P(DPRE), F, P(W_FC1_T), F, P(DY2), D, nullptr, nullptr, M, D, F, dt, s));
        RUN(svol_layernorm_bwd(f32(P(DS32_3)), P(DY2), nullptr, P(S2), xf, f32(P(G2)), f32(P(MEAN2)), f32(P(RSTD2)), f32(P(DS32_2)), P(G2D),
                               f32(P(DG2)), f32(P(DBT2)), f32(P(DB_O)), M, D, 0.f, 0, nullptr, dt, s));
        RUN(nt(P(G2D), D, P(W_O_T), D, P(DO), D, nullptr, nullptr, M, D, D, dt, s));
    }
    if (phase != 1) {
        int aflags = 0;
        if (P(EV_CLEAN_IN)) {
            if (hipStreamWaitEvent(static_cast<hipStream_t>(s), static_cast<hipEvent_t>(P(EV_CLEAN_IN)), 0) != hipSuccess) return SVOL_E_LAUNCH;
            aflags = SVOL_ATTN_DQ_PREZEROED;
        }
        record(P(EV_A0), s);
        RUN(svol_attn_bwd_ex(P(QKV), 3 * D, at(P(QKV), D, dt), 3 * D, at(P(QKV), 2 * D, dt), 3 * D, P(O), D, P(DO), D, f32(P(LSE)),
                             f32(P(DELTA)), nullptr, P(DQKV), 3 * D, at(P(DQKV), D, dt), 3 * D, at(P(DQKV), 2 * D, dt), 3 * D, d.B, d.H, d.L,
                             d.L, dh, attn_scale(dh), attn_premul(dh, dt), P(ATTN_WS), d.ws_bytes, dt, aflags, P(EV_PREP), s));
        record(P(EV_A1), s);
        if (P(ATTN_WS_NEXT) && P(ZERO_STREAM) && P(EV_PREP) && P(EV_CLEAN_OUT)) {
            hipStream_t zs = static_cast<hipStream_t>(P(ZERO_STREAM));
            if (hipStreamWaitEvent(zs, static_cast<hipEvent_t>(P(EV_PREP)), 0) != hipSuccess) return SVOL_E_LAUNCH;
            const int zrc = svol_attn_bwd_zero_ws(P(ATTN_WS_NEXT), d.ws_bytes, d.B, d.H, d.L, d.L, dh, dt, zs);
            if (zrc) return zrc;
            record(P(EV_CLEAN_OUT), zs);
        }
        RUN(nt(P(DQKV), 3 * D, P(W_IN_T), 3 * D, P(DXQ), D, nullptr, nullptr, M, D, 3 * D, dt, s));
        RUN(svol_gate_bwd(f32(P(DS32_2)), P(DXQ), nullptr, f32(P(X32)), P(POS), f32(P(U)), f32(P(G1)), f32(P(A)), f32(P(MEAN1)),
                          f32(P(RSTD1)), f32(P(GATE_WS)), f32(P(GATE_WS2)), f32(P(DX32)), f32(P(DU)), f32(P(DG1)), f32(P(DBT1)), d.B, d.L,
                          D, d.H, dt, s));
    }
    return SVOL_OK;
}

int svol_video_half_wgrad_part(const int64_t* dims, void* const* p, int part, void* s) {
    if (!dims || !p || part < 0 || part > 2) return SVOL_E_INVALID;
    Trace tr_(part == 1 ? "video_half_wgrad.1" : part == 2 ? "video_half_wgrad.2" : "video_half_wgrad", s);
    const Dims d(dims);
    if (!d.ok()) return SVOL_E_INVALID;
    const int64_t M = d.B * d.L, D = d.D, F = d.F;
    const int dt = d.dt;
    const svol_tn_problem pr[5] = {
        {P(DS3), D, P(HID), F, f32(P(DW_FC2)), F, nullptr, M, D, F},
        {P(DPRE), F, P(Y2), D, f32(P(DW_FC1)), D, nullptr, M, F, D},
        {P(G2D), D, P(O), D, f32(P(DW_O)), D, nullptr, M, D, D},
        {P(DQKV), 3 * D, P(Y1POS), D, f32(P(DW_IN)), D, f32(P(DB_IN)), M, 2 * D, D},
        {at(P(DQKV), 2 * D, dt), 3 * D, P(Y1), D, f32(P(DW_IN)) + 2 * D * D, D, f32(P(DB_IN)) + 2 * D, M, D, D}};
    if (part == 1) RUN(svol_gemm_tn_grouped(pr, 3, dt, s));
    else if (part == 2) RUN(svol_gemm_tn_grouped(pr + 3, 2, dt, s));
    else RUN(svol_gemm_tn_grouped(pr, 5, dt, s));
    return SVOL_OK;
}

int svol_video_half_wgrad(const int64_t* dims, void* const* p, void* s) { return svol_video_half_wgrad_part(dims, p, 0, s); }
#undef P

int svol_query_self_fwd(const int64_t* dims, void* const* p, void* s) {
    if (!dims || !p) return SVOL_E_INVALID;
    Trace tr_("query_self_fwd", s);
    const Dims d(dims);
    if (!d.ok() || d.N <= 0) return SVOL_E_INVALID;
    const int64_t R = d.B * d.N, D = d.D, dh = D / d.H;
    const int qdt = d.qdt, xf = qdt != SVOL_F32;
#define P(n) p[SVOL_QS_##n]
    RUN(nt(P(OPOS), D, P(W_IN), D, P(QKV), 3 * D, P(B_IN), P(QSCALE), R, 2 * D, D, qdt, s));
    if (P(WV_HILO))
        RUN(svol_gemm_nt_split(P(O), D, P(WV_HILO), 2 * D, at(P(QKV), 2 * D, qdt), 3 * D, f32(P(B_IN)) + 2 * D, R, D, D, s));
    else
        RUN(nt(P(O), D, at(P(W_IN), 2 * D * D, qdt), D, at(P(QKV), 2 * D, qdt), 3 * D, f32(P(B_IN)) + 2 * D, nullptr, R, D, D, qdt, s));
    RUN(svol_attn_fwd(P(QKV), 3 * D, at(P(QKV), D, qdt), 3 * D, at(P(QKV), 2 * D, qdt), 3 * D, P(OA), D, f32(P(LSE)), nullptr, d.B, d.H,
                      d.N, d.N, dh, attn_scale(dh), attn_premul(dh, qdt), P(ATTN_WS), d.ws_bytes, qdt, s));
    RUN(nt_res(P(OA), D, P(W_O), D, P(S4), P(B_O), P(O32), R, D, D, qdt, s));
    RUN(svol_layernorm_fwd(P(S4), xf, f32(P(G4)), f32(P(BT4)), f32(P(Y32)), P(Y), P(YPOS), P(QPOS), d.N, f32(P(MEAN4)), f32(P(RSTD4)), R, D,
                           0.f, 0, nullptr, qdt, s));
    return SVOL_OK;
}

int svol_query_self_bwd(const int64_t* dims, void* const* p, void* s) {
    if (!dims || !p) return SVOL_E_INVALID;
    Trace tr_("query_self_bwd", s);
    const Dims d(dims);
    if (!d.ok() || d.N <= 0) return SVOL_E_INVALID;
    const int64_t R = d.B * d.N, D = d.D, dh = D / d.H;
    const int qdt = d.qdt, xf = qdt != SVOL_F32;
    RUN(svol_layernorm_bwd(f32(P(DY32)), P(DY), P(DYPOS), P(S4), xf, f32(P(G4)), f32(P(MEAN4)), f32(P(RSTD4)), f32(P(DO32)), P(G),
                           f32(P(DG4)), f32(P(DBT4)), f32(P(DB_O)), R, D, 0.f, 0, nullptr, qdt, s));
    if (P(DQPOS) && P(DYPOS))
        RUN(svol_colsum(P(DYPOS), d.N * D, f32(P(DQPOS)), d.B, d.N * D, qdt, s));
    RUN(nt(P(G), D, P(W_O_T), D, P(DOA), D, nullptr, nullptr, R, D, D, qdt, s));
    RUN(svol_attn_bwd(P(QKV), 3 * D, at(P(QKV), D, qdt), 3 * D, at(P(QKV), 2 * D, qdt), 3 * D, P(OA), D, P(DOA), D, f32(P(LSE)),
                      f32(P(DELTA)), nullptr, P(DQKV), 3 * D, at(P(DQKV), D, qdt), 3 * D, at(P(DQKV), 2 * D, qdt), 3 * D, d.B, d.H, d.N,
                      d.N, dh, attn_scale(dh), attn_premul(dh, qdt), P(ATTN_WS), d.ws_bytes, qdt, s));
    RUN(nt(P(DQKV), 3 * D, P(W_IN_T), 3 * D, P(DXQP), D, nullptr, nullptr, R, D, 2 * D, qdt, s));
    RUN(nt(at(P(DQKV), 2 * D, qdt), 3 * D, at(P(W_IN_T), 2 * D, qdt), 3 * D, P(DXQ), D, nullptr, nullptr, R, D, D, qdt, s));
    return SVOL_OK;
}

int svol_query_self_wgrad(const int64_t* dims, void* const* p, void* s) {
    if (!dims || !p) return SVOL_E_INVALID;
    Trace tr_("query_self_wgrad", s);
    const Dims d(dims);
    if (!d.ok()) return SVOL_E_INVALID;
    const int64_t R = d.B * d.N, D = d.D;
    const int qdt = d.qdt;
    const svol_tn_problem pr[3] = {
        {P(G), D, P(OA), D, f32(P(DW_O)), D, nullptr, R, D, D},
        {P(DQKV), 3 * D, P(OPOS), D, f32(P(DW_IN)), D, f32(P(DB_IN)), R, 2 * D, D},
        {at(P(DQKV), 2 * D, qdt), 3 * D, P(O), D, f32(P(DW_IN)) + 2 * D * D, D, f32(P(DB_IN)) + 2 * D, R, D, D}};
    RUN(svol_gemm_tn_grouped(pr, 3, qdt, s));
    return SVOL_OK;
#undef P
}

int svol_query_cross_fwd(const int64_t* dims, void* const* p, void* s) {
    if (!dims || !p) return SVOL_E_INVALID;
    Trace tr_("query_cross_fwd", s);
    const Dims d(dims);
    if (!d.ok() || d.N <= 0 || d.L <= 0 || d.F <= 0) return SVOL_E_INVALID;
    const int64_t R = d.B * d.N, M = d.B * d.L, D = d.D, F = d.F, dh = D / d.H;
    const int dt = d.dt, qdt = d.qdt, xf = qdt != SVOL_F32;
    const bool mixed = qdt != dt;
#define P(n) p[SVOL_QC_##n]
    if (mixed) {
        RUN(nt(P(OPOS), D, P(W_INQ), D, P(Q), D, P(B_IN), P(QSCALE), R, D, D, qdt, s));
        RUN(svol_cast(P(Q), qdt, P(QC), dt, R * D, s));
    } else {
        RUN(nt(P(OPOS), D, P(W_KV), D, P(QC), D, P(B_IN), P(QSCALE), R, D, D, dt, s));
    }
    RUN(nt(P(MPOS), D, at(P(W_KV), D * D, dt), D, P(KV), 2 * D, f32(P(B_IN)) + D, nullptr, M, D, D, dt, s));
    if (P(WV_HILO))
        RUN(svol_gemm_nt_split(P(MV), D, P(WV_HILO), 2 * D, at(P(KV), D, dt), 2 * D, f32(P(B_IN)) + 2 * D, M, D, D, s));
    else
        RUN(nt(P(MV), D, at(P(W_KV), 2 * D * D, dt), D, at(P(KV), D, dt), 2 * D, f32(P(B_IN)) + 2 * D, nullptr, M, D, D, dt, s));
    RUN(svol_attn_fwd(P(QC), D, P(KV), 2 * D, at(P(KV), D, dt), 2 * D, P(OA), D, f32(P(LSE)), f32(P(KBIAS)), d.B, d.H, d.N, d.L, dh,
                      attn_scale(dh), attn_premul(dh, dt), P(ATTN_WS), d.ws_bytes, dt, s));
    const void* oq = P(OA);
    if (mixed) {
        RUN(svol_cast(P(OA), dt, P(OAQ), qdt, R * D, s));
        oq = P(OAQ);
    }
    RUN(nt_res(oq, D, P(W_O), D, P(S5), P(B_O), P(O32), R, D, D, qdt, s));
    RUN(svol_layernorm_fwd(P(S5), xf, f32(P(G5)), f32(P(BT5)), f32(P(Y5_32)), P(Y5), nullptr, nullptr, 0, f32(P(MEAN5)), f32(P(RSTD5)), R,
                           D, 0.f, 0, nullptr, qdt, s));
    RUN(svol_gemm_nt(P(Y5), D, nullptr, 0, P(W_FC1), D, P(HID), F, f32(P(B_FC1)), nullptr, SVOL_ACT_GELU, P(PRE), F, nullptr, 0, 0, R, F, D,
                     qdt, s));
    RUN(nt_res(P(HID), F, P(W_FC2), F, P(S6), P(B_FC2), P(Y5_32), R, D, F, qdt, s));
    RUN(svol_layernorm_fwd(P(S6), xf, f32(P(G6)), f32(P(BT6)), f32(P(Y32)), P(Y), P(YPOS), P(QPOS), d.N, f32(P(MEAN6)), f32(P(RSTD6)), R, D,
                           0.f, 0, nullptr, qdt, s));
    return SVOL_OK;
}

int svol_query_cross_bwd(const int64_t* dims, void* const* p, void* s) {
    if (!dims || !p) return SVOL_E_INVALID;
    Trace tr_("query_cross_bwd", s);
    const Dims d(dims);
    if (!d.ok() || d.N <= 0 || d.L <= 0 || d.F <= 0) return SVOL_E_INVALID;
    const int64_t R = d.B * d.N, M = d.B * d.L, D = d.D, F = d.F, dh = D / d.H;
    const int dt = d.dt, qdt = d.qdt, xf = qdt != SVOL_F32;
    const bool mixed = qdt != dt;
    RUN(svol_layernorm_bwd(f32(P(DY32)), P(DY), P(DYPOS), P(S6), xf, f32(P(G6)), f32(P(MEAN6)), f32(P(RSTD6)), f32(P(DS32_6)), P(DS6),
                           f32(P(DG6)), f32(P(DBT6)), f32(P(DB_FC2)), R, D, 0.f, 0, nullptr, qdt, s));
    if (P(DQPOS) && P(DYPOS)) RUN(svol_colsum(P(DYPOS), d.N * D, f32(P(DQPOS)), d.B, d.N * D, qdt, s));
    RUN(svol_gemm_nt_dact(P(DS6), D, P(W_FC2_T), D, P(DPRE), F, P(PRE), F, SVOL_ACT_GELU, f32(P(DB_FC1)), R, F, D, qdt, s));
    RUN(nt(P(DPRE), F, P(W_FC1_T), F, P(DY5), D, nullptr, nullptr, R, D, F, qdt, s));
    RUN(svol_layernorm_bwd(f32(P(DS32_6)), P(DY5), nullptr, P(S5), xf, f32(P(G5)), f32(P(MEAN5)), f32(P(RSTD5)), f32(P(DO32)), P(G5D),
                           f32(P(DG5)), f32(P(DBT5)), f32(P(DB_O)), R, D, 0.f, 0, nullptr, qdt, s));
    RUN(nt(P(G5D), D, P(W_O_T), D, P(DOAQ), D, nullptr, nullptr, R, D, D, qdt, s));
    const void* d_o = P(DOAQ);
    if (mixed) {
        RUN(svol_cast(P(DOAQ), qdt, P(DOA), dt, R * D, s));
        d_o = P(DOA);
    }
    RUN(svol_attn_bwd(P(QC), D, P(KV), 2 * D, at(P(KV), D, dt), 2 * D, P(OA), D, d_o, D, f32(P(LSE)), f32(P(DELTA)), f32(P(KBIAS)), P(DQC), D,
                      P(DKV), 2 * D, at(P(DKV), D, dt), 2 * D, d.B, d.H, d.N, d.L, dh, attn_scale(dh), attn_premul(dh, dt), P(ATTN_WS),
                      d.ws_bytes, dt, s));
    if (P(DMPOS)) {
        RUN(nt(P(DKV), 2 * D, at(P(W_KV_T), D, dt), 3 * D, P(DMPOS), D, nullptr, nullptr, M, D, D, dt, s));
        RUN(nt(at(P(DKV), D, dt), 2 * D, at(P(W_KV_T), 2 * D, dt), 3 * D, P(DMV), D, nullptr, nullptr, M, D, D, dt, s));
    } else {
        RUN(nt(P(DKV), 2 * D, at(P(W_KV_T), D, dt), 3 * D, P(DMV), D, nullptr, nullptr, M, D, 2 * D, dt, s));
    }
    const void* dq = P(DQC);
    if (mixed) {
        RUN(svol_cast(P(DQC), dt, P(DQ), qdt, R * D, s));
        dq = P(DQ);
    }
    RUN(nt(dq, D, mixed ? P(W_INQ_T) : P(W_KV_T), 3 * D, P(DXQP), D, nullptr, nullptr, R, D, D, qdt, s));
    return SVOL_OK;
}

int svol_query_cross_wgrad(const int64_t* dims, void* const* p, void* s) {
    if (!dims || !p) return SVOL_E_INVALID;
    Trace tr_("query_cross_wgrad", s);
    const Dims d(dims);
    if (!d.ok()) return SVOL_E_INVALID;
    const int64_t R = d.B * d.N, M = d.B * d.L, D = d.D, F = d.F;
    const int dt = d.dt, qdt = d.qdt;
    const bool mixed = qdt != dt;
    const svol_tn_problem pv[2] = {
        {P(DKV), 2 * D, P(MPOS), D, f32(P(DW_IN)) + D * D, D, f32(P(DB_IN)) + D, M, D, D},
        {at(P(DKV), D, dt), 2 * D, P(MV), D, f32(P(DW_IN)) + 2 * D * D, D, f32(P(DB_IN)) + 2 * D, M, D, D}};
    RUN(svol_gemm_tn_grouped(pv, 2, dt, s));
    const svol_tn_problem pq[4] = {
        {P(DS6), D, P(HID), F, f32(P(DW_FC2)), F, nullptr, R, D, F},
        {P(DPRE), F, P(Y5), D, f32(P(DW_FC1)), D, nullptr, R, F, D},
        {P(G5D), D, mixed ? P(OAQ) : P(OA), D, f32(P(DW_O)), D, nullptr, R, D, D},
        {mixed ? P(DQ) : P(DQC), D, P(OPOS), D, f32(P(DW_IN)), D, f32(P(DB_IN)), R, D, D}};
    RUN(svol_gemm_tn_grouped(pq, 4, qdt, s));
    return SVOL_OK;
#undef P
}

}
```

### svol_amd/csrc/common.h

```cpp
#pragma once
#include <hip/hip_runtime.h>
#include <stdint.h>

#include "../../include/svol_hip.h"

typedef __bf16 bf16_t;
typedef __attribute__((ext_vector_type(8))) __bf16 bf16x8;
typedef __attribute__((ext_vector_type(4))) __bf16 bf16x4;
typedef __attribute__((ext_vector_type(2))) __bf16 bf16x2;
typedef _Float16 f16_t;
typedef __attribute__((ext_vector_type(8))) _Float16 f16x8;
typedef __attribute__((ext_vector_type(4))) _Float16 f16x4;
typedef __attribute__((ext_vector_type(2))) _Float16 f16x2;
typedef __attribute__((ext_vector_type(4))) float f32x4;
typedef __attribute__((ext_vector_type(16))) float f32x16;

#ifdef SVOL_H16_FP16
typedef f16_t h16_t;
typedef f16x8 h16x8;
typedef f16x4 h16x4;
typedef f16x2 h16x2;
#define SVOL_MFMA_16x16x32_H16 __builtin_amdgcn_mfma_f32_16x16x32_f16
#define SVOL_MFMA_32x32x16_H16 __builtin_amdgcn_mfma_f32_32x32x16_f16
#define SVOL_DS_READ_TR16_H16 svol_ds_read_tr16_f16
#define SVOL_H16_ASM "f16"
#define SVOL_H16_ONE2 0x3C003C00u
#define SVOL_H16_NINF_LO 0x0000FC00u
#define SVOL_H16_DTYPE SVOL_F16
#define SVOL_H16_NEG_BIG (-6.0e4f)
#define SVOL_H16_PSUM_MAX 6.5e4f
#define svol_gemm_nt_bf16_fast svol_gemm_nt_f16_fast
#define svol_gemm_tn_bf16_fast svol_gemm_tn_f16_fast
#define svol_gemm_tn_bf16_grouped svol_gemm_tn_f16_grouped
#define svol_conv_wgrad_bf16_fast svol_conv_wgrad_f16_fast
#define svol_conv_nhwc_bf16_launch svol_conv_nhwc_f16_launch
#define svol_gemm_ws_bf16 svol_gemm_ws_f16
#define svol_gemm_n256_bf16 svol_gemm_n256_f16
#define svol_attn_fwd_bf16_launch svol_attn_fwd_f16_launch
#define svol_attn_bwd_bf16_launch svol_attn_bwd_f16_launch
#define svol_attn_ws_floats_bf16 svol_attn_ws_floats_f16
#define svol_attn_sp_image_bytes_bf16 svol_attn_sp_image_bytes_f16
#define svol_attn_sp_zero_bf16_launch svol_attn_sp_zero_f16_launch
#else
typedef bf16_t h16_t;
typedef bf16x8 h16x8;
typedef bf16x4 h16x4;
typedef bf16x2 h16x2;
#define SVOL_MFMA_16x16x32_H16 __builtin_amdgcn_mfma_f32_16x16x32_bf16
#define SVOL_MFMA_32x32x16_H16 __builtin_amdgcn_mfma_f32_32x32x16_bf16
#define SVOL_DS_READ_TR16_H16 __builtin_amdgcn_ds_read_tr16_b64_v4bf16
#define SVOL_H16_ASM "bf16"
#define SVOL_H16_ONE2 0x3F803F80u
#define SVOL_H16_NINF_LO 0x0000FF80u
#define SVOL_H16_DTYPE SVOL_BF16
#define SVOL_H16_NEG_BIG (-3.0e38f)
#define SVOL_H16_PSUM_MAX 1.0e30f
#endif
typedef __attribute__((ext_vector_type(4))) short i16x4;
__device__ __forceinline__ f16x4 svol_ds_read_tr16_f16(__attribute__((address_space(3))) f16x4* p) {
    return __builtin_bit_cast(f16x4, __builtin_amdgcn_ds_read_tr16_b64_v4i16((__attribute__((address_space(3))) i16x4*)p));
}
typedef __attribute__((ext_vector_type(2))) float f32x2;
__device__ __forceinline__ h16x2 cvt_pk_h16(float a, float b) {
#ifdef SVOL_H16_FP16
    return __builtin_convertvector((f32x2){a, b}, f16x2);
#else
    return h16x2{(bf16_t)a, (bf16_t)b};
#endif
}
static inline bool svol_is16(int dtype) { return dtype == SVOL_BF16 || dtype == SVOL_F16; }

template <typename T> struct H16;
template <> struct H16<bf16_t> {
    typedef bf16x8 v8;
    typedef bf16x4 v4;
    typedef __attribute__((address_space(3))) bf16x4* lds_v4_ptr;
    static __device__ __forceinline__ f32x4 mfma16(v8 a, v8 b, f32x4 c) { return __builtin_amdgcn_mfma_f32_16x16x32_bf16(a, b, c, 0, 0, 0); }
    static __device__ __forceinline__ f32x16 mfma32(v8 a, v8 b, f32x16 c) { return __builtin_amdgcn_mfma_f32_32x32x16_bf16(a, b, c, 0, 0, 0); }
    static __device__ __forceinline__ v4 read_tr(lds_v4_ptr p) { return __builtin_amdgcn_ds_read_tr16_b64_v4bf16(p); }
    static __device__ __forceinline__ v4 cvt4(f32x4 x) { return v4{(bf16_t)x[0], (bf16_t)x[1], (bf16_t)x[2], (bf16_t)x[3]}; }
};
template <> struct H16<f16_t> {
    typedef f16x8 v8;
    typedef f16x4 v4;
    typedef __attribute__((address_space(3))) f16x4* lds_v4_ptr;
    static __device__ __forceinline__ f32x4 mfma16(v8 a, v8 b, f32x4 c) { return __builtin_amdgcn_mfma_f32_16x16x32_f16(a, b, c, 0, 0, 0); }
    static __device__ __forceinline__ f32x16 mfma32(v8 a, v8 b, f32x16 c) { return __builtin_amdgcn_mfma_f32_32x32x16_f16(a, b, c, 0, 0, 0); }
    static __device__ __forceinline__ v4 read_tr(lds_v4_ptr p) { return svol_ds_read_tr16_f16(p); }
    static __device__ __forceinline__ v4 cvt4(f32x4 x) { return __builtin_convertvector(x, f16x4); }
};

#define SVOL_CHECK_LAUNCH()                                   \
    do {                                                      \
        if (hipGetLastError() != hipSuccess) return SVOL_E_LAUNCH; \
    } while (0)

static inline bool aligned16(const void* p) { return (reinterpret_cast<uintptr_t>(p) & 15u) == 0; }
__device__ __forceinline__ bool nonfinite(float x) { return !(fabsf(x) <= 3.0e38f); }

#include <cstdlib>
static inline bool svol_deterministic() {
    static const bool det = getenv("SVOL_DETERMINISTIC") != nullptr;
    return det;
}

struct DetScratch {
    float* p = nullptr;
    hipStream_t s;
    DetScratch(size_t floats, hipStream_t s_, bool zero = false) : s(s_) {
        if (floats == 0) return;
        hipStreamCaptureStatus cap = hipStreamCaptureStatusNone;
        if (hipStreamIsCapturing(s, &cap) != hipSuccess || cap != hipStreamCaptureStatusNone) return;
        if (hipMallocAsync(reinterpret_cast<void**>(&p), floats * sizeof(float), s) != hipSuccess) p = nullptr;
        if (p && zero && hipMemsetAsync(p, 0, floats * sizeof(float), s) != hipSuccess) { (void)hipFreeAsync(p, s); p = nullptr; }
    }
    ~DetScratch() { if (p) (void)hipFreeAsync(p, s); }
    DetScratch(const DetScratch&) = delete;
    DetScratch& operator=(const DetScratch&) = delete;
};
#ifdef __HIPCC__
namespace {
__global__ __launch_bounds__(256) void det_fold_kernel(const float* __restrict__ part, int parts, int64_t pstride, float* __restrict__ dst,
                                                       int64_t n, int64_t bpart, int64_t bdst) {
    const int64_t j = (int64_t)blockIdx.x * 256 + threadIdx.x;
    if (j >= n) return;
    const float* q = part + (int64_t)blockIdx.y * bpart + j;
    float* d = dst + (int64_t)blockIdx.y * bdst + j;
    float acc = *d;
    for (int i = 0; i < parts; ++i) acc += q[(int64_t)i * pstride];
    *d = acc;
}
inline void det_fold(const float* part, int parts, int64_t pstride, float* dst, int64_t n, hipStream_t s, int batches = 1, int64_t bpart = 0,
                     int64_t bdst = 0) {
    if (!dst || n <= 0 || parts <= 0) return;
    hipLaunchKernelGGL(det_fold_kernel, dim3((unsigned)((n + 255) / 256), (unsigned)batches), dim3(256), 0, s, part, parts, pstride, dst, n,
                       bpart, bdst);
}
}
#endif

struct HalfPair { unsigned lo, hi; };
__device__ __forceinline__ HalfPair swap_halves(unsigned x) {
    unsigned y = x;
    asm volatile("" : "+v"(y));
    const auto sw = __builtin_amdgcn_permlane32_swap(x, y, false, false);
    return HalfPair{sw[0], sw[1]};
}

__device__ __forceinline__ float to_f32(float x) { return x; }
__device__ __forceinline__ float to_f32(bf16_t x) { return (float)x; }
__device__ __forceinline__ float to_f32(f16_t x) { return (float)x; }
template <typename T> __device__ __forceinline__ T from_f32(float x);
template <> __device__ __forceinline__ float from_f32<float>(float x) { return x; }
template <> __device__ __forceinline__ bf16_t from_f32<bf16_t>(float x) { return (bf16_t)x; }
template <> __device__ __forceinline__ f16_t from_f32<f16_t>(float x) { return (f16_t)x; }

template <typename T> struct Vec4;
template <> struct Vec4<float> {
    f32x4 v;
    __device__ __forceinline__ void load(const float* p) { v = *reinterpret_cast<const f32x4*>(p); }
    __device__ __forceinline__ void store(float* p) const { *reinterpret_cast<f32x4*>(p) = v; }
    __device__ __forceinline__ float get(int i) const { return v[i]; }
    __device__ __forceinline__ void set(int i, float x) { v[i] = x; }
};
template <> struct Vec4<bf16_t> {
    bf16x4 v;
    __device__ __forceinline__ void load(const bf16_t* p) { v = *reinterpret_cast<const bf16x4*>(p); }
    __device__ __forceinline__ void store(bf16_t* p) const { *reinterpret_cast<bf16x4*>(p) = v; }
    __device__ __forceinline__ float get(int i) const { return (float)v[i]; }
    __device__ __forceinline__ void set(int i, float x) { v[i] = (bf16_t)x; }
};

template <> struct Vec4<f16_t> {
    f16x4 v;
    __device__ __forceinline__ void load(const f16_t* p) { v = *reinterpret_cast<const f16x4*>(p); }
    __device__ __forceinline__ void store(f16_t* p) const { *reinterpret_cast<f16x4*>(p) = v; }
    __device__ __forceinline__ float get(int i) const { return (float)v[i]; }
    __device__ __forceinline__ void set(int i, float x) { v[i] = (f16_t)x; }
};

template <int CTRL>
__device__ __forceinline__ float dpp_f32(float x) {
    return __builtin_bit_cast(float, __builtin_amdgcn_mov_dpp(__builtin_bit_cast(int, x), CTRL, 0xf, 0xf, false));
}
__device__ __forceinline__ HalfPair swap_rows16(unsigned x) {
    unsigned y = x;
    asm volatile("" : "+v"(y));
    const auto sw = __builtin_amdgcn_permlane16_swap(x, y, false, false);
    return HalfPair{sw[0], sw[1]};
}
__device__ __forceinline__ float wave_sum(float x) {
    x += dpp_f32<0xB1>(x);
    x += dpp_f32<0x4E>(x);
    x += dpp_f32<0x141>(x);
    x += dpp_f32<0x140>(x);
    const HalfPair a = swap_rows16(__builtin_bit_cast(unsigned, x));
    x = __builtin_bit_cast(float, a.lo) + __builtin_bit_cast(float, a.hi);
    const HalfPair b = swap_halves(__builtin_bit_cast(unsigned, x));
    return __builtin_bit_cast(float, b.lo) + __builtin_bit_cast(float, b.hi);
}
__device__ __forceinline__ float wave_max(float x) {
    x = fmaxf(x, dpp_f32<0xB1>(x));
    x = fmaxf(x, dpp_f32<0x4E>(x));
    x = fmaxf(x, dpp_f32<0x141>(x));
    x = fmaxf(x, dpp_f32<0x140>(x));
    const HalfPair a = swap_rows16(__builtin_bit_cast(unsigned, x));
    x = fmaxf(__builtin_bit_cast(float, a.lo), __builtin_bit_cast(float, a.hi));
    const HalfPair b = swap_halves(__builtin_bit_cast(unsigned, x));
    return fmaxf(__builtin_bit_cast(float, b.lo), __builtin_bit_cast(float, b.hi));
}

__device__ __forceinline__ uint32_t hash_u64(uint64_t x) {
    x ^= x >> 33; x *= 0xff51afd7ed558ccdULL;
    x ^= x >> 33; x *= 0xc4ceb9fe1a85ec53ULL;
    x ^= x >> 33;
    return (uint32_t)x;
}
__device__ __forceinline__ uint32_t drop_seed32(uint64_t seed) { return hash_u64(seed * 0x9E3779B97F4A7C15ULL + 0x632BE59BD9B4E019ULL); }
__device__ __forceinline__ uint64_t drop_seed_at(uint64_t seed, const int64_t* __restrict__ step) {
    return seed + (step ? ((uint64_t)step[0] << 12) : 0ull);
}
__device__ __forceinline__ uint32_t drop_row(uint32_t s0, uint64_t r) {
    return s0 ^ ((uint32_t)r * 0x9E3779B1u) ^ ((uint32_t)(r >> 32) * 0x7F4A7C15u);
}
__device__ __forceinline__ uint32_t drop_bits(uint32_t rowmix, uint32_t khalf) {
    uint32_t x = rowmix ^ (khalf * 0x85EBCA6Bu);
    x ^= x >> 16; x *= 0x7FEB352Du;
    x ^= x >> 15; x *= 0x846CA68Bu;
    x ^= x >> 16;
    return x;
}
__device__ __forceinline__ uint32_t drop_thr16(float p) { return (uint32_t)ceilf(p * 65536.0f); }
__device__ __forceinline__ float drop_pick(uint32_t bits, uint32_t odd, uint32_t thr16, float inv_keep) {
    const uint32_t u = odd ? bits >> 16 : bits & 0xffffu;
    return u < thr16 ? 0.0f : inv_keep;
}
__device__ __forceinline__ float drop_scale_rk(uint32_t rowmix, uint32_t k, float p, float inv_keep) {
    return drop_pick(drop_bits(rowmix, k >> 1), k & 1u, drop_thr16(p), inv_keep);
}
__device__ __forceinline__ float dropout_scale(uint64_t seed, uint64_t r, uint32_t k, float p, float inv_keep) {
    return drop_scale_rk(drop_row(drop_seed32(seed), r), k, p, inv_keep);
}

__device__ __forceinline__ void gelu_parts(float x, float& Phi, float& E) {
    const float z = fabsf(x) * 0.70710678118654752440f;
    const float t = __builtin_amdgcn_rcpf(fmaf(0.3275911f, z, 1.0f));
    E = __builtin_amdgcn_exp2f(x * x * -0.72134752044448170368f);
    float q = fmaf(1.061405429f, t, -1.453152027f);
    q = fmaf(q, t, 1.421413741f);
    q = fmaf(q, t, -0.284496736f);
    q = fmaf(q, t, 0.254829592f);
    const float h = 0.5f * q * t * E;
    Phi = x >= 0.f ? 1.0f - h : h;
}
__device__ __forceinline__ float gelu_fast(float x) {
    float Phi, E;
    gelu_parts(x, Phi, E);
    return x * Phi;
}
__device__ __forceinline__ float dgelu_fast(float x) {
    float Phi, E;
    gelu_parts(x, Phi, E);
    return fmaf(x * 0.39894228040143267794f, E, Phi);
}

__device__ __forceinline__ float dact_fast(float aux, int act) {
    return act == SVOL_ACT_RELU ? (aux > 0.f ? 1.f : 0.f) : (act == SVOL_ACT_GELU_D ? aux : dgelu_fast(aux));
}
__device__ __forceinline__ bool act_is_gelu(int act) { return act == SVOL_ACT_GELU || act == SVOL_ACT_GELU_D; }
__device__ __forceinline__ float pre_save_fast(float v, int act) { return act == SVOL_ACT_GELU_D ? dgelu_fast(v) : v; }

__device__ __forceinline__ float gelu_f(float x) { return 0.5f * x * (1.0f + erff(x * 0.70710678118654752440f)); }
__device__ __forceinline__ float dgelu_f(float x) {
    return 0.5f * (1.0f + erff(x * 0.70710678118654752440f)) + x * 0.39894228040143267794f * __expf(-0.5f * x * x);
}
```

### svol_amd/csrc/gemm.hip

```cpp
#include "gemm_call.h"

namespace {

template <typename T> struct Tr;
template <> struct Tr<bf16_t> { static constexpr int EPC = 8; };
template <> struct Tr<f16_t> { static constexpr int EPC = 8; };
template <> struct Tr<float> { static constexpr int EPC = 4; };

__device__ __forceinline__ void mma_chunk(f32x4& acc, const uint4& a, const uint4& b, bf16_t) {
    acc = __builtin_amdgcn_mfma_f32_16x16x32_bf16(__builtin_bit_cast(bf16x8, a), __builtin_bit_cast(bf16x8, b), acc,
                                                  0, 0, 0);
}
__device__ __forceinline__ void mma_chunk(f32x4& acc, const uint4& a, const uint4& b, f16_t) {
    acc = __builtin_amdgcn_mfma_f32_16x16x32_f16(__builtin_bit_cast(f16x8, a), __builtin_bit_cast(f16x8, b), acc, 0, 0, 0);
}
__device__ __forceinline__ void mma_chunk(f32x4& acc, const uint4& a, const uint4& b, float) {
    f32x4 af = __builtin_bit_cast(f32x4, a), bf = __builtin_bit_cast(f32x4, b);
#pragma unroll
    for (int e = 0; e < 4; ++e) acc = __builtin_amdgcn_mfma_f32_16x16x4f32(af[e], bf[e], acc, 0, 0, 0);
}

struct NtArgs {
    const void* A; const void* A2; const void* B; void* C;
    const float* bias; const float* colscale; void* pre; const void* res;
// ... 327 lines not shown
    if (i >= (int64_t)R * C) return;
    const int r = (int)(i / C), c = (int)(i % C);
    store_split(dstS, r, c, C, src[(int64_t)r * lds + c]);
}
template <typename T>
__global__ __launch_bounds__(256) void cast_transpose_multi_kernel(const CastDesc* __restrict__ descs, int n_desc) {
    __shared__ float tile[32][33];
    __shared__ int which;
    if (threadIdx.x == 0) {
        int lo = 0, hi = n_desc - 1;
        while (lo < hi) {
            const int mid = (lo + hi + 1) >> 1;
            if (descs[mid].tile_begin <= (int)blockIdx.x) lo = mid; else hi = mid - 1;
        }
        which = lo;
    }
    __syncthreads();
    const CastDesc d = descs[which];
    const int t = blockIdx.x - d.tile_begin;
    const int tx = threadIdx.x & 31, ty = threadIdx.x >> 5;
    const int r0 = (t / d.tiles_c) * 32, c0 = (t % d.tiles_c) * 32;
    T* dst = reinterpret_cast<T*>(d.dst);
    T* dstT = reinterpret_cast<T*>(d.dstT);
#pragma unroll
    for (int j = 0; j < 4; ++j) {
        const int r = r0 + ty + 8 * j, c = c0 + tx;
        float v = (r < d.R && c < d.C) ? d.src[(int64_t)r * d.C + c] : 0.f;
        tile[ty + 8 * j][tx] = v;
        if (dst && r < d.R && c < d.C) dst[(int64_t)r * d.C + c] = from_f32<T>(v);
        if (d.dstS && r < d.R && c < d.C) store_split(d.dstS, r, c, d.C, v);
    }
    __syncthreads();
    if (dstT) {
#pragma unroll
        for (int j = 0; j < 4; ++j) {
            const int c = c0 + ty + 8 * j, r = r0 + tx;
            if (r < d.R && c < d.C) dstT[(int64_t)c * d.R + r] = from_f32<T>(tile[tx][ty + 8 * j]);
        }
    }
}

template <typename T>
__global__ void act_bwd_kernel(const T* dy, const T* aux, T* dpre, int act, int64_t n) {
    int64_t i = (int64_t)blockIdx.x * blockDim.x + threadIdx.x;
    const int64_t stride = (int64_t)gridDim.x * blockDim.x;
    for (; i < n; i += stride) {
        const float g = to_f32(dy[i]), a = to_f32(aux[i]);
        float d;
        if (act == SVOL_ACT_RELU) d = a > 0.f ? g : 0.f;
        else if (act == SVOL_ACT_GELU) d = g * dgelu_f(a);
        else if (act == SVOL_ACT_GELU_D) d = g * a;
        else if (act == SVOL_ACT_SIGMOID) d = g * a * (1.f - a);
        else d = g;
        dpre[i] = from_f32<T>(d);
    }
}

struct SkArgs {
    const float* A; const float* B; float* C;
    const float* bias; const float* colscale; float* pre; const float* res; const float* aux; float* colsum;
    int64_t lda, ldb, ldc, ldp, ldr, ldaux;
    int M, N, K, act, epi;
};
constexpr int SKF_T = 32, SKF_LD = SKF_T + 4;

__global__ __launch_bounds__(256) void gemm_nt_f32_skinny(SkArgs p) {
    __shared__ __attribute__((aligned(16))) float red[4][SKF_T][SKF_LD];
    const int tid = threadIdx.x, lane = tid & 63, wave = tid >> 6;
    const int r = lane & 31, h = lane >> 5;
    const int bm = blockIdx.y * SKF_T, bn = blockIdx.x * SKF_T;
    const int kslice = p.K >> 2;
    const int nb = kslice >> 5;
    const bool va = bm + r < p.M, vb = bn + r < p.N;
    const float* pa = p.A + (int64_t)(bm + r) * p.lda + wave * kslice + h * 4;
    const float* pb = p.B + (int64_t)(bn + r) * p.ldb + wave * kslice + h * 4;
    const f32x4 z4 = f32x4{0.f, 0.f, 0.f, 0.f};
    f32x4 a[4], b[4], na[4], nb_[4];
    auto load = [&](f32x4 (&xa)[4], f32x4 (&xb)[4], int bt) {
#pragma unroll
        for (int c = 0; c < 4; ++c) {
            xa[c] = va ? *reinterpret_cast<const f32x4*>(pa + bt * 32 + c * 8) : z4;
            xb[c] = vb ? *reinterpret_cast<const f32x4*>(pb + bt * 32 + c * 8) : z4;
        }
    };
    f32x16 acc;
#pragma unroll
    for (int i = 0; i < 16; ++i) acc[i] = 0.f;
    load(a, b, 0);
    for (int bt = 0; bt < nb; ++bt) {
        if (bt + 1 < nb) load(na, nb_, bt + 1);
#pragma unroll
        for (int c = 0; c < 4; ++c)
#pragma unroll
            for (int e = 0; e < 4; ++e) acc = __builtin_amdgcn_mfma_f32_32x32x2f32(a[c][e], b[c][e], acc, 0, 0, 0);
        if (bt + 1 < nb) {
#pragma unroll
            for (int c = 0; c < 4; ++c) { a[c] = na[c]; b[c] = nb_[c]; }
        }
    }
#pragma unroll
    for (int g = 0; g < 4; ++g)
#pragma unroll
        for (int e = 0; e < 4; ++e) red[wave][8 * g + 4 * h + e][r] = acc[4 * g + e];
    __syncthreads();
    const int row = tid >> 3, c0 = (tid & 7) * 4;
    const int m = bm + row, n0 = bn + c0;
    f32x4 v = *reinterpret_cast<const f32x4*>(&red[0][row][c0]);
#pragma unroll
    for (int w = 1; w < 4; ++w) {
        const f32x4 u = *reinterpret_cast<const f32x4*>(&red[w][row][c0]);
#pragma unroll
        for (int e = 0; e < 4; ++e) v[e] += u[e];
    }
    const bool mv = m < p.M;
    if (p.epi == 0) {
        if (mv) {
#pragma unroll
            for (int e = 0; e < 4; ++e) {
                if (p.bias) v[e] += p.bias[n0 + e];
                if (p.colscale) v[e] *= p.colscale[n0 + e];
            }
            if (p.pre) {
                f32x4 sv = v;
                if (p.act == SVOL_ACT_GELU_D) {
#pragma unroll
                    for (int e = 0; e < 4; ++e) sv[e] = dgelu_f(v[e]);
                }
                *reinterpret_cast<f32x4*>(p.pre + (int64_t)m * p.ldp + n0) = sv;
            }
#pragma unroll
            for (int e = 0; e < 4; ++e) {
                if (p.act == SVOL_ACT_RELU) v[e] = fmaxf(v[e], 0.f);
                else if (act_is_gelu(p.act)) v[e] = gelu_f(v[e]);
                else if (p.act == SVOL_ACT_SIGMOID) v[e] = 1.f / (1.f + __expf(-v[e]));
            }
            if (p.res) {
                const f32x4 rr = *reinterpret_cast<const f32x4*>(p.res + (int64_t)m * p.ldr + n0);
#pragma unroll
                for (int e = 0; e < 4; ++e) v[e] += rr[e];
            }
            if (p.act == SVOL_ACT_RELU_RES) {
#pragma unroll
                for (int e = 0; e < 4; ++e) v[e] = fmaxf(v[e], 0.f);
            }
        }
    } else {
        if (mv) {
            const f32x4 x = *reinterpret_cast<const f32x4*>(p.aux + (int64_t)m * p.ldaux + n0);
#pragma unroll
            for (int e = 0; e < 4; ++e) v[e] *= p.act == SVOL_ACT_RELU ? (x[e] > 0.f ? 1.f : 0.f) : (p.act == SVOL_ACT_GELU_D ? x[e] : dgelu_f(x[e]));
        } else {
            v = f32x4{0.f, 0.f, 0.f, 0.f};
        }
        if (p.colsum) {
            __syncthreads();
            *reinterpret_cast<f32x4*>(&red[0][row][c0]) = v;
            __syncthreads();
            if (tid < SKF_T) {
                float sacc = 0.f;
#pragma unroll 8
                for (int i = 0; i < SKF_T; ++i) sacc += red[0][i][tid];
                atomicAdd(p.colsum + bn + tid, sacc);
            }
        }
    }
    if (mv) *reinterpret_cast<f32x4*>(p.C + (int64_t)m * p.ldc + n0) = v;
}

inline bool skinny_f32_ok(const GemmCall& c) {
    constexpr int64_t max_m = 2048;
    auto rows16 = [](const void* p, int64_t ld) { return !p || (ld % 4 == 0 && aligned16(p)); };
    return c.kwrap == c.K && c.M <= max_m && c.K % 128 == 0 && c.N % 32 == 0 && c.lda % 4 == 0 && c.ldb % 4 == 0 && c.ldc % 4 == 0 && aligned16(c.A) &&
           aligned16(c.B) && aligned16(c.C) && (c.M + 31) / 32 <= 65535 && rows16(c.res, c.ldr) && rows16(c.pre, c.ldp) && rows16(c.aux, c.ldaux);
}

inline int grid_1d(int64_t n, int block) {
    int64_t g = (n + block - 1) / block;
    return (int)(g > 4096 ? 4096 : (g < 1 ? 1 : g));
}

}

static int tn_generic_plan(const svol_tn_problem& q, int dtype, TnArgs& out, int64_t& wgs) {
    const int64_t Mc = q.Mc, N = q.N, K = q.K;
    const int epc = svol_is16(dtype) ? 8 : 4;
    if (N % epc || K % epc || q.lda % epc || q.ldb % epc) return SVOL_E_UNSUPPORTED;
    if (!aligned16(q.A) || !aligned16(q.B)) return SVOL_E_INVALID;
    if (Mc > (1 << 30) || N > (1 << 30) || K > (1 << 30)) return SVOL_E_UNSUPPORTED;
    const int ct = svol_is16(dtype) ? 64 : 32;
    const int64_t tiles = ((N + 127) / 128) * ((K + 127) / 128);
    constexpr int small_wgs = 64;
    const int target_wgs = (dtype == SVOL_F32 && Mc <= 4096) ? small_wgs : (tiles <= 8 ? 256 : 512);
    int64_t want = (target_wgs + tiles - 1) / tiles;
    if (svol_deterministic()) want = 1;
    int64_t chunk = (Mc + want - 1) / want;
    chunk = ((chunk + ct - 1) / ct) * ct;
    const int64_t floor_rows = (dtype == SVOL_F32 && Mc <= 4096) ? ct : 4 * ct;
    if (chunk < floor_rows) chunk = floor_rows;
    int64_t splits = (Mc + chunk - 1) / chunk;
    if (splits > 8 && splits % 8) {
        const int64_t s8 = (splits + 7) / 8 * 8;
        int64_t c8 = (Mc + s8 - 1) / s8;
        c8 = ((c8 + ct - 1) / ct) * ct;
        if (c8 >= floor_rows && (Mc + c8 - 1) / c8 == s8) { chunk = c8; splits = s8; }
    }
    const int64_t ktiles = (K + 127) / 128;
    if (splits * tiles > (1ll << 30)) return SVOL_E_UNSUPPORTED;
    out = TnArgs{q.A, q.B, q.C, q.colsum, q.lda, q.ldb, q.ldc, (int)Mc, (int)N, (int)K, (int)chunk, (int)ktiles, (int)splits};
    wgs = splits * tiles;
    return SVOL_OK;
}

extern "C" {

int svol_abi_version(void) { return 7; }

const char* svol_strerror(int code) {
    switch (code) {
        case SVOL_OK: return "ok";
        case SVOL_E_INVALID: return "invalid argument (null pointer, bad size or misaligned buffer)";
        case SVOL_E_UNSUPPORTED: return "shape not supported by the gfx950 kernels";
        case SVOL_E_LAUNCH: return "kernel launch failed";
        default: return "unknown error";
    }
}

static int gemm_nt_dispatch(const GemmCall& c, const void* A2, int64_t n_split, int dtype) {
    const int64_t M = c.M, N = c.N, K = c.K;
    if (!c.A || !c.B || !c.C || (c.epi && !c.aux) || M < 0 || N < 0 || K <= 0) return SVOL_E_INVALID;
    const bool act_ok = c.epi ? (c.act == SVOL_ACT_GELU || c.act == SVOL_ACT_RELU || c.act == SVOL_ACT_GELU_D) : (c.act != SVOL_ACT_GELU_D || c.pre);
    if (!act_ok) return SVOL_E_INVALID;
    if (M == 0 || N == 0) return SVOL_OK;
    if (c.epi && c.colsum && svol_deterministic()) {
        GemmCall d = c; d.colsum = nullptr;
        const int rc = gemm_nt_dispatch(d, A2, n_split, dtype);
        return rc ? rc : svol_colsum(c.C, c.ldc, c.colsum, M, N, dtype, c.stream);
    }
    if (!c.epi) {
        const int epc = svol_is16(dtype) ? 8 : 4;
        if (!svol_is16(dtype) && dtype != SVOL_F32) return SVOL_E_INVALID;
        if (K % epc || c.lda % epc || c.ldb % epc) return SVOL_E_UNSUPPORTED;
        if (!aligned16(c.A) || !aligned16(c.B) || (A2 && !aligned16(A2))) return SVOL_E_INVALID;
        if (A2 && (n_split % 128)) return SVOL_E_UNSUPPORTED;
        if (M > (1 << 30) || N > (1 << 30) || K > (1 << 30)) return SVOL_E_UNSUPPORTED;
        if ((M + 127) / 128 > 65535) return SVOL_E_UNSUPPORTED;
    }
    if (svol_is16(dtype) && !A2) {
        const int rc = (dtype == SVOL_BF16 ? svol_gemm_nt_bf16_fast : svol_gemm_nt_f16_fast)(c);
        if (rc != SVOL_E_UNSUPPORTED) return rc;
    }
    if (dtype == SVOL_F32 && !A2 && skinny_f32_ok(c)) {
        SkArgs q{(const float*)c.A, (const float*)c.B, (float*)c.C, c.bias, c.colscale, (float*)c.pre, (const float*)c.res, (const float*)c.aux,
                 c.colsum, c.lda, c.ldb, c.ldc, c.ldp, c.ldr, c.ldaux, (int)M, (int)N, (int)K, c.act, c.epi};
        hipLaunchKernelGGL(gemm_nt_f32_skinny, dim3((unsigned)(N / 32), (unsigned)((M + 31) / 32)), dim3(256), 0, c.stream, q);
        SVOL_CHECK_LAUNCH();
        return SVOL_OK;
    }
    if (c.epi) {
        if (c.ldc != N || c.ldaux != N) return SVOL_E_UNSUPPORTED;
        GemmCall g = c;
        g.aux = nullptr; g.ldaux = 0; g.colsum = nullptr; g.act = SVOL_ACT_NONE; g.epi = 0;
        if (const int rc = gemm_nt_dispatch(g, nullptr, 0, dtype)) return rc;
        if (const int rc = svol_act_bwd(c.C, c.aux, c.C, c.act, M * N, dtype, c.stream)) return rc;
        return c.colsum ? svol_colsum(c.C, c.ldc, c.colsum, M, N, dtype, c.stream) : SVOL_OK;
    }
    NtArgs p{c.A, A2, c.B, c.C, c.bias, c.colscale, c.pre, c.res, c.lda, c.ldb, c.ldc, c.ldr, c.ldp, n_split, (int)M, (int)N, (int)K, c.act, (int)c.kwrap};
    const dim3 grid((unsigned)((N + 127) / 128), (unsigned)((M + 127) / 128)), g64((unsigned)((N + 63) / 64), (unsigned)((M + 63) / 64));
    const bool small = (int64_t)grid.x * grid.y < 256 && (M + 63) / 64 <= 65535;
    void (*kern)(NtArgs) = dtype == SVOL_BF16 ? (c.out_f32 ? gemm_nt_kernel<bf16_t, float> : gemm_nt_kernel<bf16_t, bf16_t>)
                           : dtype == SVOL_F16 ? (c.out_f32 ? gemm_nt_kernel<f16_t, float> : gemm_nt_kernel<f16_t, f16_t>)
                           : small ? gemm_nt_kernel<float, float, 64> : gemm_nt_kernel<float, float>;
    hipLaunchKernelGGL(kern, dtype == SVOL_F32 && small ? g64 : grid, dim3(256), 0, c.stream, p);
    SVOL_CHECK_LAUNCH();
    return SVOL_OK;
}

int svol_gemm_nt(const void* A, int64_t lda, const void* A2, int64_t n_split, const void* B, int64_t ldb, void* C,
                 int64_t ldc, const float* bias, const float* colscale, int act, void* pre_act_out, int64_t ldp,
                 const void* residual, int64_t ldr, int out_f32, int64_t M, int64_t N, int64_t K, int dtype, void* stream) {
    GemmCall c{};
    c.A = A; c.lda = lda; c.B = B; c.ldb = ldb; c.C = C; c.ldc = ldc; c.pre = pre_act_out; c.ldp = ldp; c.res = residual; c.ldr = ldr;
    c.bias = bias; c.colscale = colscale; c.act = act; c.out_f32 = out_f32; c.M = M; c.N = N; c.K = K; c.kwrap = K;
    c.stream = reinterpret_cast<hipStream_t>(stream);
    return gemm_nt_dispatch(c, A2, n_split, dtype);
}

int svol_gemm_nt_split(const void* A, int64_t lda, const void* W_hilo, int64_t ldw, void* C, int64_t ldc, const float* bias,
                       int64_t M, int64_t N, int64_t K, void* stream) {
    if (K <= 0 || K % 8) return SVOL_E_UNSUPPORTED;
    GemmCall c{};
    c.A = A; c.lda = lda; c.B = W_hilo; c.ldb = ldw; c.C = C; c.ldc = ldc; c.bias = bias;
    c.M = M; c.N = N; c.K = 2 * K; c.kwrap = K;
    c.stream = reinterpret_cast<hipStream_t>(stream);
    return gemm_nt_dispatch(c, nullptr, 0, SVOL_BF16);
}

int svol_gemm_nt_dact(const void* A, int64_t lda, const void* B, int64_t ldb, void* C, int64_t ldc, const void* aux,
                      int64_t ldaux, int act, float* colsum, int64_t M, int64_t N, int64_t K, int dtype, void* stream) {
    GemmCall c{};
    c.A = A; c.lda = lda; c.B = B; c.ldb = ldb; c.C = C; c.ldc = ldc; c.aux = aux; c.ldaux = ldaux; c.colsum = colsum;
    c.M = M; c.N = N; c.K = K; c.kwrap = K; c.act = act; c.epi = 1;
    c.stream = reinterpret_cast<hipStream_t>(stream);
    return gemm_nt_dispatch(c, nullptr, 0, dtype);
}

int svol_gemm_nt_dgelu(const void* A, int64_t lda, const void* B, int64_t ldb, void* C, int64_t ldc, const void* pre,
                       int64_t ldp, float* colsum, int64_t M, int64_t N, int64_t K, int dtype, void* stream) {
    return svol_gemm_nt_dact(A, lda, B, ldb, C, ldc, pre, ldp, SVOL_ACT_GELU, colsum, M, N, K, dtype, stream);
}

static int gemm_tn_dispatch(const svol_tn_problem& q, int dtype, hipStream_t s) {
    if (!q.A || !q.B || !q.C || q.Mc < 0 || q.N <= 0 || q.K <= 0) return SVOL_E_INVALID;
    if (q.Mc == 0) return SVOL_OK;
    if (!svol_is16(dtype) && dtype != SVOL_F32) return SVOL_E_INVALID;
    if (svol_is16(dtype)) {
        const int rc = (dtype == SVOL_BF16 ? svol_gemm_tn_bf16_fast : svol_gemm_tn_f16_fast)(q, s);
        if (rc != SVOL_E_UNSUPPORTED) return rc;
    }
    TnArgs p{};
    int64_t wgs = 0;
    if (const int rc = tn_generic_plan(q, dtype, p, wgs)) return rc;
    if (dtype == SVOL_BF16) hipLaunchKernelGGL(gemm_tn_kernel<bf16_t>, dim3((unsigned)wgs), dim3(256), 0, s, p);
    else if (dtype == SVOL_F16) hipLaunchKernelGGL(gemm_tn_kernel<f16_t>, dim3((unsigned)wgs), dim3(256), 0, s, p);
    else hipLaunchKernelGGL(gemm_tn_kernel<float>, dim3((unsigned)wgs), dim3(256), 0, s, p);
    SVOL_CHECK_LAUNCH();
    return SVOL_OK;
}

int svol_gemm_tn(const void* A, int64_t lda, const void* B, int64_t ldb, float* C, int64_t ldc, float* colsum, int64_t Mc,
                 int64_t N, int64_t K, int dtype, void* stream) {
    return gemm_tn_dispatch(svol_tn_problem{A, lda, B, ldb, C, ldc, colsum, Mc, N, K}, dtype, reinterpret_cast<hipStream_t>(stream));
}

int svol_gemm_tn_grouped(const svol_tn_problem* pr, int32_t n, int dtype, void* stream) {
    if (!pr || n < 0) return SVOL_E_INVALID;
    if (!svol_is16(dtype) && dtype != SVOL_F32) return SVOL_E_INVALID;
    hipStream_t s = reinterpret_cast<hipStream_t>(stream);
    for (int32_t i0 = 0; i0 < n; i0 += SVOL_TN_GROUP_MAX) {
        const int m = (int)((n - i0 < SVOL_TN_GROUP_MAX) ? n - i0 : SVOL_TN_GROUP_MAX);
        int rc = SVOL_E_UNSUPPORTED;
        bool ok = m > 1;
        for (int i = 0; ok && i < m; ++i) ok = pr[i0 + i].A && pr[i0 + i].B && pr[i0 + i].C && pr[i0 + i].Mc > 0 && pr[i0 + i].N > 0 && pr[i0 + i].K > 0;
        if (ok && svol_is16(dtype)) {
            rc = (dtype == SVOL_BF16 ? svol_gemm_tn_bf16_grouped : svol_gemm_tn_f16_grouped)(pr + i0, m, s);
        } else if (ok) {
            TnGroupArgsG g{};
            g.n = m;
            int64_t tot = 0;
            rc = SVOL_OK;
            for (int i = 0; i < m && rc == SVOL_OK; ++i) {
                int64_t wgs = 0;
                rc = tn_generic_plan(pr[i0 + i], dtype, g.a[i], wgs);
                g.begin[i] = (int)tot;
                tot += wgs;
            }
            if (rc == SVOL_OK && tot <= (1ll << 30)) {
                for (int i = m; i <= SVOL_TN_GROUP_MAX; ++i) g.begin[i] = (int)tot;
                hipLaunchKernelGGL(gemm_tn_grouped_kernel<float>, dim3((unsigned)tot), dim3(256), 0, s, g);
                SVOL_CHECK_LAUNCH();
            } else {
                rc = SVOL_E_UNSUPPORTED;
            }
        }
        if (rc == SVOL_E_UNSUPPORTED) {
            for (int i = 0; i < m; ++i) {
                const int r1 = gemm_tn_dispatch(pr[i0 + i], dtype, s);
                if (r1) return r1;
            }
        } else if (rc) {
            return rc;
        }
    }
    return SVOL_OK;
}

int svol_colsum(const void* X, int64_t ldx, float* out, int64_t M, int64_t N, int dtype, void* stream) {
    if (!X || !out || M < 0 || N <= 0) return SVOL_E_INVALID;
    if (M == 0) return SVOL_OK;
    if (M > (1 << 30) || N > (1 << 30)) return SVOL_E_UNSUPPORTED;
    const int colblocks = (int)((N + 255) / 256);
    int rowblocks = (int)((M + 255) / 256);
    int maxrb = 2048 / colblocks;
    if (maxrb < 1) maxrb = 1;
    if (rowblocks > maxrb) rowblocks = maxrb;
    const int rpb = (int)((M + rowblocks - 1) / rowblocks);
    dim3 grid(colblocks, (unsigned)((M + rpb - 1) / rpb));
    hipStream_t s = reinterpret_cast<hipStream_t>(stream);
    const bool det_mode = svol_deterministic();
    DetScratch det(det_mode ? (size_t)grid.y * (size_t)N : 0, s);
    if (det_mode && !det.p) return SVOL_E_LAUNCH;
    if (dtype == SVOL_BF16)
        hipLaunchKernelGGL(colsum_kernel<bf16_t>, grid, dim3(256), 0, s, (const bf16_t*)X, ldx, out, (int)M, (int)N, rpb, det.p);
    else if (dtype == SVOL_F16)
        hipLaunchKernelGGL(colsum_kernel<f16_t>, grid, dim3(256), 0, s, (const f16_t*)X, ldx, out, (int)M, (int)N, rpb, det.p);
    else if (dtype == SVOL_F32)
        hipLaunchKernelGGL(colsum_kernel<float>, grid, dim3(256), 0, s, (const float*)X, ldx, out, (int)M, (int)N, rpb, det.p);
    else return SVOL_E_INVALID;
    if (det_mode) det_fold(det.p, (int)grid.y, N, out, N, s);
    SVOL_CHECK_LAUNCH();
    return SVOL_OK;
}

int svol_cast(const void* src, int dtype_src, void* dst, int dtype_dst, int64_t n, void* stream) {
    if (!src || !dst || n < 0) return SVOL_E_INVALID;
    if (n == 0) return SVOL_OK;
    hipStream_t s = reinterpret_cast<hipStream_t>(stream);
    const int g = grid_1d(n, 256);
    if (dtype_src == SVOL_F32 && dtype_dst == SVOL_BF16 && n % 8 == 0 && aligned16(src) && aligned16(dst) && n / 8 / 256 < (1ll << 31))
        hipLaunchKernelGGL(cast_f32_bf16_vec8_kernel, dim3((unsigned)((n / 8 + 255) / 256)), dim3(256), 0, s, (const float*)src,
                           (bf16_t*)dst, n / 8);
    else {
#define SVOL_CAST(TS, TD) hipLaunchKernelGGL((cast_kernel<TS, TD>), dim3(g), dim3(256), 0, s, (const TS*)src, (TD*)dst, n)
#define SVOL_CAST_FROM(TS)                                      \
    do {                                                        \
        if (dtype_dst == SVOL_F32) SVOL_CAST(TS, float);        \
        else if (dtype_dst == SVOL_BF16) SVOL_CAST(TS, bf16_t); \
        else if (dtype_dst == SVOL_F16) SVOL_CAST(TS, f16_t);   \
        else return SVOL_E_INVALID;                             \
    } while (0)
        if (dtype_src == SVOL_F32) SVOL_CAST_FROM(float);
        else if (dtype_src == SVOL_BF16) SVOL_CAST_FROM(bf16_t);
        else if (dtype_src == SVOL_F16) SVOL_CAST_FROM(f16_t);
        else return SVOL_E_INVALID;
#undef SVOL_CAST_FROM
#undef SVOL_CAST
    }
    SVOL_CHECK_LAUNCH();
    return SVOL_OK;
}

int svol_cast_transpose(const float* src, void* dst, void* dstT, int dtype, int64_t R, int64_t C, void* stream) {
    if (!src || R <= 0 || C <= 0 || (!dst && !dstT)) return SVOL_E_INVALID;
    if (R > (1 << 30) || C > (1 << 30)) return SVOL_E_UNSUPPORTED;
    dim3 grid((unsigned)((C + 31) / 32), (unsigned)((R + 31) / 32));
    if (grid.y > 65535u) return SVOL_E_UNSUPPORTED;
    hipStream_t s = reinterpret_cast<hipStream_t>(stream);
    if (dtype == SVOL_BF16)
        hipLaunchKernelGGL(cast_transpose_kernel<bf16_t>, grid, dim3(256), 0, s, src, (bf16_t*)dst, (bf16_t*)dstT, (int)R, (int)C);
    else if (dtype == SVOL_F16)
        hipLaunchKernelGGL(cast_transpose_kernel<f16_t>, grid, dim3(256), 0, s, src, (f16_t*)dst, (f16_t*)dstT, (int)R, (int)C);
    else if (dtype == SVOL_F32)
        hipLaunchKernelGGL(cast_transpose_kernel<float>, grid, dim3(256), 0, s, src, (float*)dst, (float*)dstT, (int)R, (int)C);
    else return SVOL_E_INVALID;
    SVOL_CHECK_LAUNCH();
    return SVOL_OK;
}

int svol_cast_split(const float* src, int64_t ld_src, void* dst_hilo, int64_t R, int64_t C, void* stream) {
    if (!src || !dst_hilo || R <= 0 || C <= 0 || ld_src < C) return SVOL_E_INVALID;
    if (R * C > (1ll << 38)) return SVOL_E_UNSUPPORTED;
    hipLaunchKernelGGL(cast_split_kernel<bf16_t>, dim3((unsigned)((R * C + 255) / 256)), dim3(256), 0, reinterpret_cast<hipStream_t>(stream),
                       src, ld_src, dst_hilo, (int)R, (int)C);
    SVOL_CHECK_LAUNCH();
    return SVOL_OK;
}

int svol_cast_transpose_multi(const void* descs, int32_t n_desc, int64_t total_tiles, int dtype, void* stream) {
    static_assert(sizeof(CastDesc) == 48, "descriptor layout is part of the ABI (include/svol_hip.h)");
    if (!descs || n_desc <= 0 || total_tiles <= 0) return SVOL_E_INVALID;
    if (total_tiles > (1ll << 30)) return SVOL_E_UNSUPPORTED;
    hipStream_t s = reinterpret_cast<hipStream_t>(stream);
    const CastDesc* d = reinterpret_cast<const CastDesc*>(descs);
    if (dtype == SVOL_BF16) hipLaunchKernelGGL(cast_transpose_multi_kernel<bf16_t>, dim3((unsigned)total_tiles), dim3(256), 0, s, d, n_desc);
    else if (dtype == SVOL_F16) hipLaunchKernelGGL(cast_transpose_multi_kernel<f16_t>, dim3((unsigned)total_tiles), dim3(256), 0, s, d, n_desc);
    else if (dtype == SVOL_F32) hipLaunchKernelGGL(cast_transpose_multi_kernel<float>, dim3((unsigned)total_tiles), dim3(256), 0, s, d, n_desc);
    else return SVOL_E_INVALID;
    SVOL_CHECK_LAUNCH();
    return SVOL_OK;
}

int svol_act_bwd(const void* dy, const void* aux, void* dpre, int act, int64_t n, int dtype, void* stream) {
    if (!dy || !aux || !dpre || n < 0) return SVOL_E_INVALID;
    if (n == 0) return SVOL_OK;
    hipStream_t s = reinterpret_cast<hipStream_t>(stream);
    const int g = grid_1d(n, 256);
    if (dtype == SVOL_BF16)
        hipLaunchKernelGGL(act_bwd_kernel<bf16_t>, dim3(g), dim3(256), 0, s, (const bf16_t*)dy, (const bf16_t*)aux, (bf16_t*)dpre, act, n);
    else if (dtype == SVOL_F16)
        hipLaunchKernelGGL(act_bwd_kernel<f16_t>, dim3(g), dim3(256), 0, s, (const f16_t*)dy, (const f16_t*)aux, (f16_t*)dpre, act, n);
    else if (dtype == SVOL_F32)
        hipLaunchKernelGGL(act_bwd_kernel<float>, dim3(g), dim3(256), 0, s, (const float*)dy, (const float*)aux, (float*)dpre, act, n);
    else return SVOL_E_INVALID;
    SVOL_CHECK_LAUNCH();
    return SVOL_OK;
}

}
```

### svol_amd/csrc/gemm_call.h

```cpp
#pragma once
#include "common.h"

struct GemmCall {
    const void *A, *B, *res, *aux;
    void *C, *pre;
    const float *bias, *colscale;
    float* colsum;
    int64_t lda, ldb, ldc, ldp, ldr, ldaux, M, N, K, kwrap;
    int act, epi, out_f32;
    hipStream_t stream;
};

#define SVOL_GEMM_H16_ENTRIES(T)                                                                                                  \
    int svol_gemm_nt_##T##_fast(const GemmCall& c);                                                                               \
    int svol_gemm_ws_##T(const GemmCall& c);                                                                                      \
    int svol_gemm_n256_##T(const GemmCall& c);                                                                                    \
    int svol_gemm_tn_##T##_fast(const svol_tn_problem& q, hipStream_t s);                                                         \
    int svol_gemm_tn_##T##_grouped(const svol_tn_problem* pr, int n, hipStream_t s);                                              \
    int svol_conv_wgrad_##T##_fast(const void* dz, const void* x, float* dwp, int64_t N, int64_t H, int64_t W, int64_t C,         \
                                   int64_t Cout, int64_t kh, int64_t kw, int64_t stride, int64_t pad, int64_t Kp, hipStream_t s);  \
    int svol_conv_nhwc_##T##_launch(const void* x, const void* w, int64_t ldw, void* y, const float* bias, int act,               \
                                    const void* residual, int64_t N, int64_t H, int64_t W, int64_t C, int64_t Cout, int64_t kh,  \
                                    int64_t kw, int64_t stride, int64_t pad, hipStream_t s);
SVOL_GEMM_H16_ENTRIES(bf16)
SVOL_GEMM_H16_ENTRIES(f16)
#undef SVOL_GEMM_H16_ENTRIES
```

### svol_amd/csrc/gemm_n256_bf16.hip

```cpp
#include <type_traits>

#include "gemm_call.h"

namespace {

struct N256Args {
    const h16_t* A; const h16_t* W; void* C;
    const float* bias; const float* res;
    int64_t lda, ldw, ldc, ldr;
    int M, K, act, nrt;
    int rpw;
    int kwt;
};

typedef __attribute__((address_space(3))) void* lds_void_ptr;

constexpr int BM = 128, BN = 256, BK = 32, BAL_BM = 256;
constexpr int W_ST = BN * BK * 2;
constexpr int BAL_STG = 3;
template <bool BAL> struct Ring {
    static constexpr int bm = BAL ? BAL_BM : BM, waves = bm / 32, stg = BAL ? BAL_STG : 3;
    static constexpr int a_st = bm * BK * 2, slot = a_st + W_ST, bytes = stg * slot;
    static constexpr int wpw = 16 / waves;
    static constexpr int pieces = 2 + wpw;
    static constexpr int w_base = BAL ? stg * a_st : 0;
    static constexpr int offa(int s) { return BAL ? s * a_st : s * slot; }
    static constexpr int offw(int s) { return BAL ? s * W_ST : s * slot + a_st; }
    static_assert(offa(stg - 1) < 65536 && offw(stg - 1) < 65536 && bytes <= 160 * 1024, "ring does not fit");
};

__device__ __forceinline__ int slot32(int row, int ch) { return ch ^ ((0x78 >> (2 * ((row >> 2) & 3))) & 3); }
__device__ __forceinline__ int wcol(int nt, int i) { return (nt >> 1) * 32 + (i >> 2) * 8 + (nt & 1) * 4 + (i & 3); }

template <int N> __device__ __forceinline__ void n256_wait_vm() { asm volatile("s_waitcnt vmcnt(%0)" ::"n"(N) : "memory"); }
template <int PIECES, int F> __device__ __forceinline__ void n256_wait_slabs(int fly) {
    if constexpr (F == 0) n256_wait_vm<0>();
    else if (fly >= F) n256_wait_vm<PIECES * F>();
    else n256_wait_slabs<PIECES, F - 1>(fly);
}

template <int OFFA, int OFFW>
__device__ __forceinline__ void read_frags(uint4 (&af)[4], uint4 (&wf)[8], const unsigned (&aa)[4], const unsigned (&wa)[8]) {
    asm volatile(
        "ds_read_b128 %0, %12 offset:%c24\n\t"
        "ds_read_b128 %1, %13 offset:%c24\n\t"
        "ds_read_b128 %2, %14 offset:%c24\n\t"
        "ds_read_b128 %3, %15 offset:%c24\n\t"
        "ds_read_b128 %4, %16 offset:%c25\n\t"
        "ds_read_b128 %5, %17 offset:%c25\n\t"
        "ds_read_b128 %6, %18 offset:%c25\n\t"
        "ds_read_b128 %7, %19 offset:%c25\n\t"
        "ds_read_b128 %8, %20 offset:%c25\n\t"
        "ds_read_b128 %9, %21 offset:%c25\n\t"
        "ds_read_b128 %10, %22 offset:%c25\n\t"
        "ds_read_b128 %11, %23 offset:%c25\n\t"
        "s_waitcnt lgkmcnt(0)"
        : "=&v"(af[0]), "=&v"(af[1]), "=&v"(af[2]), "=&v"(af[3]), "=&v"(wf[0]), "=&v"(wf[1]), "=&v"(wf[2]), "=&v"(wf[3]),
          "=&v"(wf[4]), "=&v"(wf[5]), "=&v"(wf[6]), "=&v"(wf[7])
        : "v"(aa[0]), "v"(aa[1]), "v"(aa[2]), "v"(aa[3]), "v"(wa[0]), "v"(wa[1]), "v"(wa[2]), "v"(wa[3]), "v"(wa[4]), "v"(wa[5]),
          "v"(wa[6]), "v"(wa[7]), "n"(OFFA), "n"(OFFW)
        : "memory");
}

template <int S, int STG, class F> __device__ __forceinline__ void ring_pass(F& step, int kt) {
    if constexpr (S < STG) { step(std::integral_constant<int, S>{}, kt + S); ring_pass<S + 1, STG>(step, kt); }
}
template <int S, int STG, class F> __device__ __forceinline__ void ring_tail(F& step, int kt, int nk) {
    if constexpr (S < STG - 1) {
        if (kt < nk) { step(std::integral_constant<int, S>{}, kt); ring_tail<S + 1, STG>(step, kt + 1, nk); }
    }
}

template <bool OUT_F32, bool BAL>
__device__ __forceinline__ void gemm_n256_body(const N256Args& p) {
    using R = Ring<BAL>;
    constexpr int STG = R::stg;
    __shared__ __attribute__((aligned(1024))) char smem[R::bytes];
    const int tid = threadIdx.x, lane = tid & 63;
    const int wave = __builtin_amdgcn_readfirstlane(tid >> 6);
    const int wm = wave >> 1, wn = wave & 1;
    const int fr = lane & 15, fq = lane >> 4;
    const int rt = BAL ? blockIdx.x : blockIdx.x % p.nrt, cg = BAL ? 0 : blockIdx.x / p.nrt;
    const int bm = rt * (BAL ? p.rpw : BM);
    if (bm >= p.M) return;
    const int rows = min(BAL ? p.rpw : BM, p.M - bm);
    const int bn = cg * BN;
    const int ntile = (rows + 15) >> 4;
    const int t0 = BAL ? (wm * ntile) >> 2 : wm * 4;
    const int cnt = BAL ? (((wm + 1) * ntile) >> 2) - t0 : 4;

    const __amdgpu_buffer_rsrc_t rA = __builtin_amdgcn_make_buffer_rsrc(
        (void*)(p.A + (int64_t)bm * p.lda), 0, (int)((((int64_t)rows - 1) * p.lda + p.kwt * BK) * 2), 0x00020000);
    const __amdgpu_buffer_rsrc_t rW =
        __builtin_amdgcn_make_buffer_rsrc((void*)(p.W + (int64_t)bn * p.ldw), 0, (int)((((int64_t)BN - 1) * p.ldw + p.K) * 2), 0x00020000);
    int voffA[2], voffW[R::wpw];
#pragma unroll
    for (int j = 0; j < 2; ++j) {
        const int row = (wave * 2 + j) * 16 + (lane >> 2);
        voffA[j] = (int)(((int64_t)row * p.lda + slot32(row, lane & 3) * 8) * 2);
    }
#pragma unroll
    for (int j = 0; j < R::wpw; ++j) {
        const int rho = (wave * R::wpw + j) * 16 + (lane >> 2);
        const int n = (rho >> 7) * 128 + wcol((rho & 127) >> 4, rho & 15);
        voffW[j] = (int)(((int64_t)n * p.ldw + slot32(rho, lane & 3) * 8) * 2);
    }
    auto issue = [&](int slot, int kt) {
        char* slA = smem + (BAL ? slot * R::a_st : slot * R::slot);
        char* slW = smem + (BAL ? R::w_base + slot * W_ST : slot * R::slot + R::a_st);
        const int so = kt * BK * 2;
        const int soA = (kt >= p.kwt ? kt - p.kwt : kt) * BK * 2;
#pragma unroll
        for (int j = 0; j < 2; ++j)
            __builtin_amdgcn_raw_ptr_buffer_load_lds(rA, (lds_void_ptr)(slA + (wave * 2 + j) * 1024), 16, voffA[j], soA, 0, 0);
#pragma unroll
        for (int j = 0; j < R::wpw; ++j)
            __builtin_amdgcn_raw_ptr_buffer_load_lds(rW, (lds_void_ptr)(slW + (wave * R::wpw + j) * 1024), 16, voffW[j], so, 0, 0);
    };

    const unsigned lds0 = (unsigned)(size_t)(lds_void_ptr)smem;
    unsigned aa[4], wa[8];
#pragma unroll
    for (int mt = 0; mt < 4; ++mt) {
        const int row = (t0 + mt) * 16 + fr;
        aa[mt] = lds0 + (unsigned)(row * 64 + (slot32(row, fq) << 4));
    }
#pragma unroll
    for (int nt = 0; nt < 8; ++nt) {
        const int rho = wn * 128 + nt * 16 + fr;
        wa[nt] = lds0 + (unsigned)(R::w_base + rho * 64 + (slot32(rho, fq) << 4));
    }

    f32x4 acc[8][4];
#pragma unroll
    for (int i = 0; i < 8; ++i)
#pragma unroll
        for (int j = 0; j < 4; ++j) acc[i][j] = f32x4{0.f, 0.f, 0.f, 0.f};

    const int nk = p.K / BK;
#pragma unroll
    for (int s = 0; s < STG - 1; ++s)
        if (s < nk) issue(s, s);
    auto step = [&](auto slot_tag, int kt) {
        constexpr int S = decltype(slot_tag)::value;
        n256_wait_slabs<R::pieces, STG - 2>(nk - 1 - kt);
        __builtin_amdgcn_s_barrier();
        if (kt + STG - 1 < nk) issue((S + STG - 1) % STG, kt + STG - 1);
        uint4 af[4], wf[8];
        read_frags<R::offa(S), R::offw(S)>(af, wf, aa, wa);
        if constexpr (BAL) {
#pragma unroll
            for (int mt = 0; mt < 4; ++mt)
                if (mt < cnt) {
#pragma unroll
                    for (int nt = 0; nt < 8; ++nt)
                        acc[nt][mt] = SVOL_MFMA_16x16x32_H16(__builtin_bit_cast(h16x8, wf[nt]),
                                                                              __builtin_bit_cast(h16x8, af[mt]), acc[nt][mt], 0, 0, 0);
                }
        } else {
#pragma unroll
            for (int nt = 0; nt < 8; ++nt)
#pragma unroll
                for (int mt = 0; mt < 4; ++mt)
                    acc[nt][mt] = SVOL_MFMA_16x16x32_H16(__builtin_bit_cast(h16x8, wf[nt]),
                                                                          __builtin_bit_cast(h16x8, af[mt]), acc[nt][mt], 0, 0, 0);
        }
    };
    int kt = 0;
    for (; kt + STG <= nk; kt += STG) ring_pass<0, STG>(step, kt);
    ring_tail<0, STG>(step, kt, nk);

#pragma unroll
    for (int mt = 0; mt < 4; ++mt) {
        const int lr = (t0 + mt) * 16 + fr;
        const int m = bm + lr;
        if (mt >= cnt || lr >= rows) continue;
#pragma unroll
        for (int pr = 0; pr < 4; ++pr) {
            const int n0 = bn + wn * 128 + pr * 32 + fq * 8;
            float v[8];
#pragma unroll
            for (int e = 0; e < 8; ++e) v[e] = acc[2 * pr + (e >> 2)][mt][e & 3];
            if (p.bias) {
#pragma unroll
                for (int e = 0; e < 8; ++e) v[e] += p.bias[n0 + e];
            }
            if constexpr (OUT_F32) {
                float* C = reinterpret_cast<float*>(p.C) + (int64_t)m * p.ldc + n0;
                if (p.res) {
                    const float* R = p.res + (int64_t)m * p.ldr + n0;
                    const f32x4 r0 = *reinterpret_cast<const f32x4*>(R), r1 = *reinterpret_cast<const f32x4*>(R + 4);
#pragma unroll
                    for (int e = 0; e < 4; ++e) { v[e] += r0[e]; v[4 + e] += r1[e]; }
                }
                *reinterpret_cast<f32x4*>(C) = f32x4{v[0], v[1], v[2], v[3]};
                *reinterpret_cast<f32x4*>(C + 4) = f32x4{v[4], v[5], v[6], v[7]};
            } else {
                if (act_is_gelu(p.act)) {
#pragma unroll
                    for (int e = 0; e < 8; ++e) v[e] = gelu_fast(v[e]);
                }
                if (p.act == SVOL_ACT_RELU) {
#pragma unroll
                    for (int e = 0; e < 8; ++e) v[e] = fmaxf(v[e], 0.f);
                }
                h16x8 o;
#pragma unroll
                for (int e = 0; e < 8; ++e) o[e] = (h16_t)v[e];
                *reinterpret_cast<h16x8*>(reinterpret_cast<h16_t*>(p.C) + (int64_t)m * p.ldc + n0) = o;
            }
        }
    }
}

__global__ __launch_bounds__(256, 2) void gemm_n256_bf16_f32(N256Args p) { gemm_n256_body<true, false>(p); }
__global__ __launch_bounds__(256, 2) void gemm_n256_bf16_b16(N256Args p) { gemm_n256_body<false, false>(p); }
__global__ __launch_bounds__(512, 2) void gemm_n256_bal_bf16_f32(N256Args p) { gemm_n256_body<true, true>(p); }
__global__ __launch_bounds__(512, 2) void gemm_n256_bal_bf16_b16(N256Args p) { gemm_n256_body<false, true>(p); }

}

static int n256_cus() {
    static const int n = [] {
        int dev = 0, cus = 0;
        if (hipGetDevice(&dev) != hipSuccess || hipDeviceGetAttribute(&cus, hipDeviceAttributeMultiprocessorCount, dev) != hipSuccess) return 0;
        return cus;
    }();
    return n;
}

static int n256_plan(const GemmCall& c, N256Args& p, dim3& grid, bool& bal) {
    const int64_t M = c.M, N = c.N, K = c.K;
    if (N % BN || K % BK || K < 512 || M < 4096) return SVOL_E_UNSUPPORTED;
    if (c.epi != 0 || c.pre || c.colscale) return SVOL_E_UNSUPPORTED;
    if (c.kwrap != K && (c.kwrap % BK || 2 * c.kwrap != K)) return SVOL_E_UNSUPPORTED;
    if (c.act != SVOL_ACT_NONE && ((c.act != SVOL_ACT_GELU && c.act != SVOL_ACT_RELU) || c.out_f32)) return SVOL_E_UNSUPPORTED;
    if (c.res && !c.out_f32) return SVOL_E_UNSUPPORTED;
    if (c.lda % 8 || c.ldb % 8 || !aligned16(c.A) || !aligned16(c.B) || !aligned16(c.C)) return SVOL_E_UNSUPPORTED;
    if (c.out_f32 ? (c.ldc % 4 || (c.res && (c.ldr % 4 || !aligned16(c.res)))) : (c.ldc % 8 != 0)) return SVOL_E_UNSUPPORTED;
    if ((int64_t)BM * c.lda * 2 >= (1ll << 31) || (int64_t)BN * c.ldb * 2 >= (1ll << 31)) return SVOL_E_UNSUPPORTED;
    const int64_t ncg = N / BN, cus = n256_cus();
    bal = ncg == 1 && cus > 0 && M > BM * cus && (int64_t)BAL_BM * c.lda * 2 < (1ll << 31);
    int64_t nrt = (M + BM - 1) / BM, rpw = 0;
    if (bal) {
        nrt = cus * ((M + BAL_BM * cus - 1) / (BAL_BM * cus));
        rpw = (M + nrt - 1) / nrt;
    } else if (ncg > 1) nrt = (nrt + 7) / 8 * 8;
    if (nrt * ncg > (1ll << 30)) return SVOL_E_UNSUPPORTED;
    p = N256Args{(const h16_t*)c.A, (const h16_t*)c.B, c.C, c.bias, (const float*)c.res, c.lda, c.ldb, c.ldc, c.ldr, (int)M, (int)K, c.act,
                 (int)nrt, (int)rpw, (int)(c.kwrap / BK)};
    grid = dim3((unsigned)(nrt * ncg));
    return SVOL_OK;
}

int svol_gemm_n256_bf16(const GemmCall& c) {
    N256Args p; dim3 grid; bool bal;
    if (const int rc = n256_plan(c, p, grid, bal)) return rc;
    if (bal) hipLaunchKernelGGL(c.out_f32 ? gemm_n256_bal_bf16_f32 : gemm_n256_bal_bf16_b16, grid, dim3(512), 0, c.stream, p);
    else hipLaunchKernelGGL(c.out_f32 ? gemm_n256_bf16_f32 : gemm_n256_bf16_b16, grid, dim3(256), 0, c.stream, p);
    return hipGetLastError() == hipSuccess ? SVOL_OK : SVOL_E_LAUNCH;
}
```

### svol_amd/csrc/ln_row.h

```cpp
#pragma once
#include "common.h"

namespace {

template <int WPR>
struct LnOwner {
    static_assert(WPR == 1 || WPR == 4, "a row belongs to one wave or to the four waves of a workgroup");
    static __device__ __forceinline__ int lane() { return WPR == 1 ? threadIdx.x & 63 : threadIdx.x; }
    static __device__ __forceinline__ int col(int j) { return (lane() + 64 * WPR * j) * 4; }
    static __device__ __forceinline__ int64_t index() { return WPR == 1 ? (int64_t)blockIdx.x * 4 + (threadIdx.x >> 6) : (int64_t)blockIdx.x; }
    template <int N>
    static __device__ __forceinline__ float (*slots())[4] {
        if constexpr (WPR == 4) {
            __shared__ float s[N][4];
            return s;
        } else {
            return nullptr;
        }
    }
    template <int K>
    static __device__ __forceinline__ void sum(float (&v)[K], float (*slot)[4]) {
#pragma unroll
        for (int k = 0; k < K; ++k) v[k] = wave_sum(v[k]);
        if constexpr (WPR == 4) {
            if ((threadIdx.x & 63) == 0) {
#pragma unroll
                for (int k = 0; k < K; ++k) slot[k][threadIdx.x >> 6] = v[k];
            }
            __syncthreads();
#pragma unroll
            for (int k = 0; k < K; ++k) v[k] = (slot[k][0] + slot[k][1]) + (slot[k][2] + slot[k][3]);
        }
    }
};

template <typename T, int NP>
struct LnFwdRow {
    using Own = LnOwner<1>;
    Vec4<float> t[NP], gv[NP], bv[NP];
    Vec4<T> pv[NP];
    float v[NP][4], mu, rs;

    __device__ __forceinline__ void load(const float* __restrict__ x, const T* __restrict__ pos, int64_t row, const float* __restrict__ gamma,
                                         const float* __restrict__ beta, int D) {
        const float* xl = x + row * D + Own::col(0);
        const T* pl = pos + row * D + Own::col(0);
#pragma unroll
        for (int j = 0; j < NP; ++j) {
            if (Own::col(j) < D) {
                t[j].load(xl + 256 * j);
                pv[j].load(pl + 256 * j);
            }
        }
#pragma unroll
        for (int j = 0; j < NP; ++j) {
            const int c = Own::col(j);
            if (c < D) {
                gv[j].load(gamma + c);
                bv[j].load(beta + c);
            }
        }
    }
    __device__ __forceinline__ void stats(float scale, int D) {
#pragma clang fp contract(off)
        float s = 0.f;
#pragma unroll
        for (int j = 0; j < NP; ++j) {
            const int c = Own::col(j);
#pragma unroll
            for (int e = 0; e < 4; ++e) {
                v[j][e] = c < D ? t[j].get(e) * scale : 0.f;
                s += v[j][e];
            }
        }
        mu = wave_sum(s) / (float)D;
        float q = 0.f;
#pragma unroll
        for (int j = 0; j < NP; ++j) {
            if (Own::col(j) < D) {
#pragma unroll
                for (int e = 0; e < 4; ++e) { const float d = v[j][e] - mu; q += d * d; }
            }
        }
        rs = rsqrtf(wave_sum(q) / (float)D + 1e-5f);
    }
    __device__ __forceinline__ void store(int64_t row, float* __restrict__ y32, T* __restrict__ y, T* __restrict__ ypos, int D,
                                          float (*tp)[4]) const {
#pragma clang fp contract(off)
#pragma unroll
        for (int j = 0; j < NP; ++j) {
            const int c = Own::col(j);
            if (c < D) {
                Vec4<T> o, op;
                Vec4<float> o32;
#pragma unroll
                for (int e = 0; e < 4; ++e) {
                    const float r = __builtin_fmaf((v[j][e] - mu) * rs, gv[j].get(e), bv[j].get(e));
                    o.set(e, r);
                    o32.set(e, r);
                    op.set(e, r + pv[j].get(e));
                    if (tp) tp[j][e] = r + pv[j].get(e);
                }
                if (y32) o32.store(y32 + row * D + c);
                if (y) o.store(y + row * D + c);
                if (ypos) op.store(ypos + row * D + c);
            }
        }
    }
};

template <typename T, typename TX, int NP, int WPR>
struct LnBwdRows {
    using Own = LnOwner<WPR>;
    struct Row { Vec4<float> a32[NP]; Vec4<T> a[NP], b[NP]; Vec4<TX> xv[NP]; float mu, rs; };
    const float* __restrict__ dy32;
    const T* __restrict__ dy;
    const T* __restrict__ dy2;
    const TX* __restrict__ x;
    const float* __restrict__ mean;
    const float* __restrict__ rstd;
    int D;
    float acc[3][NP][4], gm[NP][4];

    __device__ __forceinline__ void init(const float* __restrict__ gamma) {
#pragma unroll
        for (int j = 0; j < NP; ++j) {
            const int c = Own::col(j);
#pragma unroll
            for (int e = 0; e < 4; ++e) {
                acc[0][j][e] = acc[1][j][e] = acc[2][j][e] = 0.f;
                gm[j][e] = c < D ? gamma[c + e] : 0.f;
            }
        }
    }
    __device__ __forceinline__ void fetch(int64_t row, Row& r) const {
#pragma unroll
        for (int j = 0; j < NP; ++j) {
            const int c = Own::col(j);
            if (c < D) {
                if (dy32) r.a32[j].load(dy32 + row * D + c);
                if (dy) r.a[j].load(dy + row * D + c);
                if (dy2) r.b[j].load(dy2 + row * D + c);
                r.xv[j].load(x + row * D + c);
            }
        }
        r.mu = mean[row];
        r.rs = rstd[row];
    }
    __device__ __forceinline__ void row(const Row& cur, int64_t row, float* __restrict__ dx32, T* __restrict__ dx, float p, float inv_keep,
                                        uint64_t seed, float (*slot)[4]) {
#pragma clang fp contract(off)
        const float mu = cur.mu, rs = cur.rs;
        float g[NP][4], xh[NP][4];
        float s[2] = {0.f, 0.f};
#pragma unroll
        for (int j = 0; j < NP; ++j) {
            const int c = Own::col(j);
            if (c < D) {
#pragma unroll
                for (int e = 0; e < 4; ++e) {
                    float d = (dy32 ? cur.a32[j].get(e) : 0.f) + (dy ? cur.a[j].get(e) : 0.f) + (dy2 ? cur.b[j].get(e) : 0.f);
                    if (p > 0.f) d *= dropout_scale(seed, (uint64_t)row, (uint32_t)(c + e), p, inv_keep);
                    const float h = (cur.xv[j].get(e) - mu) * rs;
                    xh[j][e] = h;
                    acc[0][j][e] = __builtin_fmaf(d, h, acc[0][j][e]);
                    acc[1][j][e] += d;
                    const float gg = d * gm[j][e];
                    g[j][e] = gg;
                    s[0] += gg;
                    s[1] += gg * h;
                }
            }
        }
        Own::sum(s, slot);
        const float s1 = s[0] / (float)D, s2 = s[1] / (float)D;
#pragma unroll
        for (int j = 0; j < NP; ++j) {
            const int c = Own::col(j);
            if (c < D) {
                Vec4<T> o;
                Vec4<float> o32;
#pragma unroll
                for (int e = 0; e < 4; ++e) {
                    const float ds = rs * __builtin_fmaf(-xh[j][e], s2, g[j][e] - s1);
                    acc[2][j][e] += ds;
                    o.set(e, ds);
                    o32.set(e, ds);
                }
                if (dx32) o32.store(dx32 + row * D + c);
                if (dx) o.store(dx + row * D + c);
            }
        }
    }
};

template <int WPR, int K, int NP>
__device__ __forceinline__ const float* ln_fold_columns(const float (&part)[K][NP][4], int D) {
    using Own = LnOwner<WPR>;
    __shared__ float red[K][NP * 256 * WPR];
    const int wave = threadIdx.x >> 6;
    for (int w = 0; w < (WPR == 1 ? 4 : 1); ++w) {
        if (WPR == 4 || wave == w) {
#pragma unroll
            for (int j = 0; j < NP; ++j) {
                const int c = Own::col(j);
                if (c < D) {
#pragma unroll
                    for (int e = 0; e < 4; ++e)
#pragma unroll
                        for (int k = 0; k < K; ++k) {
                            if (w == 0) red[k][c + e] = part[k][j][e];
                            else red[k][c + e] += part[k][j][e];
                        }
                }
            }
        }
        __syncthreads();
    }
    return &red[0][0];
}
template <int WPR, int K, int NP>
__device__ __forceinline__ void ln_fold_columns(const float (&part)[K][NP][4], float* const (&sink)[K], float* __restrict__ det_row, int D) {
    const float* red = ln_fold_columns<WPR>(part, D);
    for (int c = threadIdx.x; c < D; c += 256) {
#pragma unroll
        for (int k = 0; k < K; ++k) {
            const float v = red[k * NP * 256 * WPR + c];
            if (det_row) det_row[k * D + c] = v;
            else if (sink[k]) atomicAdd(sink[k] + c, v);
        }
    }
}

}
```

Before: 15350.

## Fuse LayerNorm forward/backward into N=256 GEMM epilogue for MLP FC2/FC1

Adds GEMM variants for the N=256 kernel that stage the output tile in the shared-memory ring and run LayerNorm forward (with residual reconstruction, pos add) or LayerNorm backward (with dgamma/dbeta/colsum reductions) inside the epilogue. The video-half block uses them for FC2+LN3 in forward and FC1-dgrad+LN2-bwd in backward, eliminating separate LN kernels and intermediate Y2/DY2 buffers. This removes global round-trips and kernel launches at the cost of heavier epilogues, extra syncs, and atomics for column sums.

```diff
diff --git a/include/svol_hip.h b/include/svol_hip.h
--- a/include/svol_hip.h
+++ b/include/svol_hip.h
@@ -80,6 +80,15 @@
 int svol_gemm_nt_dact(const void* A, int64_t lda, const void* B, int64_t ldb, void* C, int64_t ldc,
                       const void* aux, int64_t ldaux, int act, float* colsum, int64_t M, int64_t N, int64_t K,
                       int dtype, void* stream);
+
+int svol_gemm_nt_ln_fits(int64_t M, int64_t K, int dtype);
+int svol_gemm_nt_ln_fwd(const void* A, int64_t lda, const void* W, int64_t ldw, float* S, const float* bias, const float* res32,
+                        const float* res_x, const float* res_mean, const float* res_rstd, const float* res_gamma, const float* res_beta,
+                        const float* gamma, const float* beta, const void* pos, float* mean, float* rstd, float* y32, void* y, void* ypos,
+                        int64_t M, int64_t K, int dtype, int any_size, void* stream);
+int svol_gemm_nt_ln_bwd(const void* A, int64_t lda, const void* W, int64_t ldw, void* dy_out, const float* dy32, const float* x,
+                        const float* gamma, const float* mean, const float* rstd, float* dx32, void* dx, float* dgamma, float* dbeta,
+                        float* dx_colsum, int64_t M, int64_t K, int dtype, int any_size, void* stream);
 
 int svol_gemm_tn(const void* A, int64_t lda, const void* B, int64_t ldb, float* C, int64_t ldc, float* colsum,
                  int64_t Mc, int64_t N, int64_t K, int dtype, void* stream);
diff --git a/svol_amd/_lib.py b/svol_amd/_lib.py
--- a/svol_amd/_lib.py
+++ b/svol_amd/_lib.py
@@ -29,6 +29,9 @@
                      _int, _p],
     'svol_gemm_nt_dgelu': [_p, _i64, _p, _i64, _p, _i64, _p, _i64, _p, _i64, _i64, _i64, _int, _p],
     'svol_gemm_nt_dact': [_p, _i64, _p, _i64, _p, _i64, _p, _i64, _int, _p, _i64, _i64, _i64, _int, _p],
+    'svol_gemm_nt_ln_fits': [_i64, _i64, _int],
+    'svol_gemm_nt_ln_fwd': [_p, _i64, _p, _i64] + [_p] * 16 + [_i64, _i64, _int, _int, _p],
+    'svol_gemm_nt_ln_bwd': [_p, _i64, _p, _i64] + [_p] * 11 + [_i64, _i64, _int, _int, _p],
     'svol_gemm_tn': [_p, _i64, _p, _i64, _p, _i64, _p, _i64, _i64, _i64, _int, _p],
     'svol_gemm_tn_grouped': [_p, _i32, _int, _p],
     'svol_colsum': [_p, _i64, _p, _i64, _i64, _int, _p],
diff --git a/svol_amd/blocks.py b/svol_amd/blocks.py
--- a/svol_amd/blocks.py
+++ b/svol_amd/blocks.py
@@ -356,9 +356,14 @@
             ('M32', M * D * 4), ('M', M * D * e), ('MPOS', M * D * e)]
 
 
-def _vh_bwd_layout(B, L, D, H, F, e):
+def _vh_ln_epilogue(M, D, F, dt):
+    return D == 256 and bool(_lib.lib().svol_gemm_nt_ln_fits(M, F, ops._DT[dt]))
+
+
+def _vh_bwd_layout(B, L, D, H, F, e, fused=False):
     M = B * L
-    return [('DS32_3', M * D * 4), ('DS3', M * D * e), ('DPRE', M * F * e), ('DY2', M * D * e), ('DS32_2', M * D * 4), ('G2D', M * D * e),
+    return [('DS32_3', M * D * 4), ('DS3', M * D * e), ('DPRE', M * F * e)] + ([] if fused else [('DY2', M * D * e)]) + [
+            ('DS32_2', M * D * 4), ('G2D', M * D * e),
             ('DO', M * D * e), ('DQKV', M * 3 * D * e), ('DELTA', 3 * B * H * L * 4), ('DXQ', M * D * e),
             ('GATE_WS2', (B * L + B * H) * 4), ('DX32', M * D * 4)]
 
@@ -382,9 +387,12 @@
         x2, pos2, u = _c(x32.reshape(M, D)), _c(pos.reshape(M, D)), _c(u)
         assert x2.dtype == torch.float32 and pos2.dtype == dt and u.dtype == torch.float32
         wsb = ops.attn_ws_bytes(dt, B, H, L, L, D // H)
-        lay = _open(ctx, pl, VH, (B, L, D, H, F, dt), _dims(B, L, 0, D, H, F, dt, dt, wsb), len(params), dev,
+        ctx.ln_epi = _vh_ln_epilogue(M, D, F, dt)
+        no_y2 = ctx.ln_epi and u_next is None
+        lay = _open(ctx, pl, VH, (B, L, D, H, F, dt, no_y2), _dims(B, L, 0, D, H, F, dt, dt, wsb), len(params), dev,
                     lambda: _vh_fwd_layout(B, L, D, H, F, e),
-                    lambda: [('Y1_32', M * D * 4), ('Y2_32', M * D * 4), ('ATTN_WS', max(wsb, 16))], X32=x2, POS=pos2, U=u)
+                    lambda: [('Y1_32', M * D * 4)] + ([] if no_y2 else [('Y2_32', M * D * 4)]) + [('ATTN_WS', max(wsb, 16))],
+                    X32=x2, POS=pos2, U=u)
         tbl = ctx.tbl
         if sc_in is not None:
             assert sc_in.dtype == torch.float32 and sc_in.numel() == B * H * (L + 2) and sc_in.is_contiguous()
@@ -421,7 +429,7 @@
         dev = ctx.saved_tensors[0].device
         du = torch.zeros((B, H, D), dtype=torch.float32, device=dev)
         tbl.set('DU', du.data_ptr())
-        lay, tmp, bufs, gs = _open_bwd(ctx, dev, lambda: _vh_bwd_layout(B, L, D, H, F, _ESZ[dt]), DM32=dm32, DM=dm, DMPOS=dmpos)
+        lay, tmp, bufs, gs = _open_bwd(ctx, dev, lambda: _vh_bwd_layout(B, L, D, H, F, _ESZ[dt], ctx.ln_epi), DM32=dm32, DM=dm, DMPOS=dmpos)
         _call('svol_video_half_bwd', ctx, 1)
         wgrad.attn_backward(B * H * L * L)
         _attn_events(tbl, _maybe_events('attn_bwd', (B, H, L, L, D // H)))
diff --git a/svol_amd/csrc/blocks.hip b/svol_amd/csrc/blocks.hip
--- a/svol_amd/csrc/blocks.hip
+++ b/svol_amd/csrc/blocks.hip
@@ -164,6 +164,8 @@
     const int64_t M = d.B * d.L, D = d.D, F = d.F, dh = D / d.H;
     const int dt = d.dt, xf = dt != SVOL_F32;
 #define P(n) p[SVOL_VH_##n]
+    const bool ln_epi = D == 256 && svol_gemm_nt_ln_fits(M, F, dt) && !(P(U_NEXT) && P(GATE_WS_NEXT));
+    if (!P(Y2_32) && !ln_epi) return SVOL_E_INVALID;
     if (P(GATE_PRE))
         RUN(svol_gate_fwd_scored(f32(P(X32)), P(POS), f32(P(U)), f32(P(G1)), f32(P(BT1)), f32(P(Y1_32)), P(Y1), P(Y1POS), f32(P(A)),
                                  f32(P(MEAN1)), f32(P(RSTD1)), f32(P(GATE_WS)), d.B, d.L, D, d.H, dt, s));
@@ -183,6 +185,12 @@
     RUN(svol_layernorm_fwd(P(S2), xf, f32(P(G2)), f32(P(BT2)), f32(P(Y2_32)), P(Y2), nullptr, nullptr, 0, f32(P(MEAN2)), f32(P(RSTD2)), M,
                            D, 0.f, 0, nullptr, dt, s));
     RUN(svol_gemm_nt(P(Y2), D, nullptr, 0, P(W_FC1), D, P(HID), F, f32(P(B_FC1)), nullptr, SVOL_ACT_GELU_D, P(PRE), F, nullptr, 0, 0, M, F, D, dt, s));
+    if (ln_epi) {
+        RUN(svol_gemm_nt_ln_fwd(P(HID), F, P(W_FC2), F, f32(P(S3)), f32(P(B_FC2)), f32(P(Y2_32)), P(Y2_32) ? nullptr : f32(P(S2)),
+                                f32(P(MEAN2)), f32(P(RSTD2)), f32(P(G2)), f32(P(BT2)), f32(P(G3)), f32(P(BT3)), P(POS), f32(P(MEAN3)),
+                                f32(P(RSTD3)), f32(P(M32)), P(M), P(MPOS), M, F, dt, 0, s));
+        return SVOL_OK;
+    }
     RUN(nt_res(P(HID), F, P(W_FC2), F, P(S3), P(B_FC2), P(Y2_32), M, D, F, dt, s));
     if (P(U_NEXT) && P(GATE_WS_NEXT))
         RUN(svol_layernorm_gate_scores_fwd(f32(P(S3)), f32(P(G3)), f32(P(BT3)), f32(P(M32)), P(M), P(MPOS), P(POS), f32(P(MEAN3)),
@@ -200,13 +208,20 @@
     if (!d.ok() || d.L <= 0 || d.F <= 0) return SVOL_E_INVALID;
     const int64_t M = d.B * d.L, D = d.D, F = d.F, dh = D / d.H;
     const int dt = d.dt, xf = dt != SVOL_F32;
+    const bool ln_epi = D == 256 && svol_gemm_nt_ln_fits(M, F, dt);
+    if (phase != 2 && !P(DY2) && !ln_epi) return SVOL_E_INVALID;
     if (phase != 2) {
         RUN(svol_layernorm_bwd(f32(P(DM32)), P(DM), P(DMPOS), P(S3), xf, f32(P(G3)), f32(P(MEAN3)), f32(P(RSTD3)), f32(P(DS32_3)), P(DS3),
                                f32(P(DG3)), f32(P(DBT3)), f32(P(DB_FC2)), M, D, 0.f, 0, nullptr, dt, s));
         RUN(svol_gemm_nt_dact(P(DS3), D, P(W_FC2_T), D, P(DPRE), F, P(PRE), F, SVOL_ACT_GELU_D, f32(P(DB_FC1)), M, F, D, dt, s));
-        RUN(nt(P(DPRE), F, P(W_FC1_T), F, P(DY2), D, nullptr, nullptr, M, D, F, dt, s));
-        RUN(svol_layernorm_bwd(f32(P(DS32_3)), P(DY2), nullptr, P(S2), xf, f32(P(G2)), f32(P(MEAN2)), f32(P(RSTD2)), f32(P(DS32_2)), P(G2D),
-                               f32(P(DG2)), f32(P(DBT2)), f32(P(DB_O)), M, D, 0.f, 0, nullptr, dt, s));
+        if (ln_epi) {
+            RUN(svol_gemm_nt_ln_bwd(P(DPRE), F, P(W_FC1_T), F, P(DY2), f32(P(DS32_3)), f32(P(S2)), f32(P(G2)), f32(P(MEAN2)), f32(P(RSTD2)),
+                                    f32(P(DS32_2)), P(G2D), f32(P(DG2)), f32(P(DBT2)), f32(P(DB_O)), M, F, dt, 0, s));
+        } else {
+            RUN(nt(P(DPRE), F, P(W_FC1_T), F, P(DY2), D, nullptr, nullptr, M, D, F, dt, s));
+            RUN(svol_layernorm_bwd(f32(P(DS32_3)), P(DY2), nullptr, P(S2), xf, f32(P(G2)), f32(P(MEAN2)), f32(P(RSTD2)), f32(P(DS32_2)),
+                                   P(G2D), f32(P(DG2)), f32(P(DBT2)), f32(P(DB_O)), M, D, 0.f, 0, nullptr, dt, s));
+        }
         RUN(nt(P(G2D), D, P(W_O_T), D, P(DO), D, nullptr, nullptr, M, D, D, dt, s));
     }
     if (phase != 1) {
diff --git a/svol_amd/csrc/common.h b/svol_amd/csrc/common.h
--- a/svol_amd/csrc/common.h
+++ b/svol_amd/csrc/common.h
@@ -36,6 +36,7 @@
 #define svol_conv_nhwc_bf16_launch svol_conv_nhwc_f16_launch
 #define svol_gemm_ws_bf16 svol_gemm_ws_f16
 #define svol_gemm_n256_bf16 svol_gemm_n256_f16
+#define svol_gemm_n256_ln_bf16 svol_gemm_n256_ln_f16
 #define svol_attn_fwd_bf16_launch svol_attn_fwd_f16_launch
 #define svol_attn_bwd_bf16_launch svol_attn_bwd_f16_launch
 #define svol_attn_ws_floats_bf16 svol_attn_ws_floats_f16
diff --git a/svol_amd/csrc/gemm.hip b/svol_amd/csrc/gemm.hip
--- a/svol_amd/csrc/gemm.hip
+++ b/svol_amd/csrc/gemm.hip
@@ -653,6 +653,56 @@
     c.M = M; c.N = N; c.K = K; c.kwrap = K; c.act = act; c.epi = 1;
     c.stream = reinterpret_cast<hipStream_t>(stream);
     return gemm_nt_dispatch(c, nullptr, 0, dtype);
+}
+
+int svol_gemm_nt_ln_fits(int64_t M, int64_t K, int dtype) {
+    return svol_is16(dtype) && !svol_deterministic() && M >= 4096 && K >= 512 && K % 32 == 0;
+}
+
+static int gemm_nt_ln(const GemmCall& c, const LnEpilogue& e, bool backward, int any_size, int dtype) {
+    if (!svol_is16(dtype)) return dtype == SVOL_F32 ? SVOL_E_UNSUPPORTED : SVOL_E_INVALID;
+    if (!any_size && !svol_gemm_nt_ln_fits(c.M, c.K, dtype)) return SVOL_E_UNSUPPORTED;
+    if (c.K % 8 || c.lda % 8 || c.ldb % 8) return SVOL_E_UNSUPPORTED;
+    if (!aligned16(c.A) || !aligned16(c.B)) return SVOL_E_INVALID;
+    if (c.M > (1 << 30) || c.K > (1 << 30)) return SVOL_E_UNSUPPORTED;
+    return (dtype == SVOL_BF16 ? svol_gemm_n256_ln_bf16 : svol_gemm_n256_ln_f16)(c, e, backward, any_size != 0);
+}
+
+int svol_gemm_nt_ln_fwd(const void* A, int64_t lda, const void* W, int64_t ldw, float* S, const float* bias, const float* res32,
+                        const float* res_x, const float* res_mean, const float* res_rstd, const float* res_gamma, const float* res_beta,
+                        const float* gamma, const float* beta, const void* pos, float* mean, float* rstd, float* y32, void* y, void* ypos,
+                        int64_t M, int64_t K, int dtype, int any_size, void* stream) {
+    if (!A || !W || !S || !gamma || !beta || !mean || !rstd || (!y && !y32) || M < 0 || K <= 0) return SVOL_E_INVALID;
+    if ((ypos != nullptr) != (pos != nullptr)) return SVOL_E_INVALID;
+    if (res_x && (res32 || !res_mean || !res_rstd || !res_gamma || !res_beta)) return SVOL_E_INVALID;
+    const void* const v16[] = {S, bias, res32, res_x, res_gamma, res_beta, gamma, beta, pos, y32, y, ypos};
+    for (const void* v : v16)
+        if (!aligned16(v)) return SVOL_E_INVALID;
+    if (M == 0) return SVOL_OK;
+    GemmCall c{};
+    c.A = A; c.lda = lda; c.B = W; c.ldb = ldw; c.C = S; c.ldc = 256; c.bias = bias; c.res = res32; c.ldr = 256; c.out_f32 = 1;
+    c.M = M; c.N = 256; c.K = K; c.kwrap = K; c.stream = reinterpret_cast<hipStream_t>(stream);
+    LnEpilogue e{};
+    e.rx = res_x; e.rmu = res_mean; e.rrs = res_rstd; e.rg = res_gamma; e.rb = res_beta;
+    e.gamma = gamma; e.beta = beta; e.pos = pos; e.mean = mean; e.rstd = rstd; e.y32 = y32; e.y = y; e.ypos = ypos;
+    return gemm_nt_ln(c, e, false, any_size, dtype);
+}
+
+int svol_gemm_nt_ln_bwd(const void* A, int64_t lda, const void* W, int64_t ldw, void* dy_out, const float* dy32, const float* x,
+                        const float* gamma, const float* mean, const float* rstd, float* dx32, void* dx, float* dgamma, float* dbeta,
+                        float* dx_colsum, int64_t M, int64_t K, int dtype, int any_size, void* stream) {
+    if (!A || !W || !x || !gamma || !mean || !rstd || (!dx && !dx32) || !dgamma || !dbeta || M < 0 || K <= 0) return SVOL_E_INVALID;
+    const void* const v16[] = {dy_out, dy32, x, gamma, dx32, dx};
+    for (const void* v : v16)
+        if (!aligned16(v)) return SVOL_E_INVALID;
+    if (M == 0) return SVOL_OK;
+    GemmCall c{};
+    c.A = A; c.lda = lda; c.B = W; c.ldb = ldw; c.C = dy_out; c.ldc = 256;
+    c.M = M; c.N = 256; c.K = K; c.kwrap = K; c.stream = reinterpret_cast<hipStream_t>(stream);
+    LnEpilogue e{};
+    e.gamma = gamma; e.mean = const_cast<float*>(mean); e.rstd = const_cast<float*>(rstd); e.dy32 = dy32; e.x = x; e.dx32 = dx32; e.dx = dx;
+    e.dgamma = dgamma; e.dbeta = dbeta; e.dxsum = dx_colsum;
+    return gemm_nt_ln(c, e, true, any_size, dtype);
 }
 
 int svol_gemm_nt_dgelu(const void* A, int64_t lda, const void* B, int64_t ldb, void* C, int64_t ldc, const void* pre,
diff --git a/svol_amd/csrc/gemm_call.h b/svol_amd/csrc/gemm_call.h
--- a/svol_amd/csrc/gemm_call.h
+++ b/svol_amd/csrc/gemm_call.h
@@ -11,10 +11,24 @@
     hipStream_t stream;
 };
 
+struct LnEpilogue {
+    const float *rx, *rmu, *rrs, *rg, *rb;
+    const float *gamma, *beta;
+    const void* pos;
+    float *mean, *rstd;
+    float* y32;
+    void *y, *ypos;
+    const float *dy32, *x;
+    float* dx32;
+    void* dx;
+    float *dgamma, *dbeta, *dxsum;
+};
+
 #define SVOL_GEMM_H16_ENTRIES(T)                                                                                                  \
     int svol_gemm_nt_##T##_fast(const GemmCall& c);                                                                               \
     int svol_gemm_ws_##T(const GemmCall& c);                                                                                      \
     int svol_gemm_n256_##T(const GemmCall& c);                                                                                    \
+    int svol_gemm_n256_ln_##T(const GemmCall& c, const LnEpilogue& e, bool backward, bool any_size);                              \
     int svol_gemm_tn_##T##_fast(const svol_tn_problem& q, hipStream_t s);                                                         \
     int svol_gemm_tn_##T##_grouped(const svol_tn_problem* pr, int n, hipStream_t s);                                              \
     int svol_conv_wgrad_##T##_fast(const void* dz, const void* x, float* dwp, int64_t N, int64_t H, int64_t W, int64_t C,         \
diff --git a/svol_amd/csrc/gemm_n256_bf16.hip b/svol_amd/csrc/gemm_n256_bf16.hip
--- a/svol_amd/csrc/gemm_n256_bf16.hip
+++ b/svol_amd/csrc/gemm_n256_bf16.hip
@@ -1,6 +1,7 @@
 #include <type_traits>
 
 #include "gemm_call.h"
+#include "ln_row.h"
 
 namespace {
 
@@ -71,8 +72,148 @@
     }
 }
 
+template <bool BAL> struct LnStage {
+    static constexpr int nw = Ring<BAL>::waves, rows = 8 * nw, per_wave = 8;
+    static constexpr int ls32 = 260, ls16 = 264;
+    static_assert(rows * ls32 * 4 <= Ring<BAL>::bytes && 3 * 256 * 4 <= Ring<BAL>::bytes, "the staged chunk lives in the ring");
+};
+
 template <bool OUT_F32, bool BAL>
-__device__ __forceinline__ void gemm_n256_body(const N256Args& p) {
+__device__ __forceinline__ void n256_ln_epilogue(const N256Args& p, const LnEpilogue& q, const f32x4 (&acc)[8][4], char* smem, int bm,
+                                                 int rows, int ntile, int t0, int cnt) {
+    using St = LnStage<BAL>;
+    constexpr int NW = St::nw, NI = St::per_wave;
+    const int tid = threadIdx.x, lane = tid & 63;
+    const int wave = __builtin_amdgcn_readfirstlane(tid >> 6);
+    const int wm = wave >> 1, wn = wave & 1;
+    const int fr = lane & 15, fq = lane >> 4;
+    auto block_row = [&](int j, int mt) {
+        const int w = j >> 4;
+        const int t0j = BAL ? (w * ntile) >> 2 : w * 4;
+        const int cntj = BAL ? (((w + 1) * ntile) >> 2) - t0j : 4;
+        const int lr = (t0j + mt) * 16 + (j & 15);
+        return (mt < cntj && lr < rows) ? lr : -1;
+    };
+    __syncthreads();
+
+    if constexpr (OUT_F32) {
+        float* stage = reinterpret_cast<float*>(smem);
+        h16_t* y = reinterpret_cast<h16_t*>(q.y);
+        h16_t* ypos = reinterpret_cast<h16_t*>(q.ypos);
+        const h16_t* pos = reinterpret_cast<const h16_t*>(q.pos);
+        float* C = reinterpret_cast<float*>(p.C);
+        LnFwdRow<h16_t, 1> ln;
+        ln.load_affine(q.gamma, q.beta);
+#pragma unroll
+        for (int mt = 0; mt < 4; ++mt) {
+            Vec4<h16_t> pv[NI];
+#pragma unroll
+            for (int i = 0; i < NI; ++i) {
+                const int lr = block_row(wave + i * NW, mt);
+                pv[i].v = h16x4{(h16_t)0.f, (h16_t)0.f, (h16_t)0.f, (h16_t)0.f};
+                if (pos && lr >= 0) pv[i].load(pos + (int64_t)(bm + lr) * 256 + LnOwner<1>::col(0));
+            }
+            const int lr = (t0 + mt) * 16 + fr;
+            const int64_t m = bm + lr;
+            if (mt < cnt && lr < rows) {
+                float mu = 0.f, rs = 0.f;
+                if (q.rx) { mu = q.rmu[m]; rs = q.rrs[m]; }
+#pragma unroll
+                for (int pr = 0; pr < 4; ++pr) {
+                    const int n0 = wn * 128 + pr * 32 + fq * 8;
+                    float v[8];
+#pragma unroll
+                    for (int e = 0; e < 8; ++e) v[e] = acc[2 * pr + (e >> 2)][mt][e & 3];
+                    if (p.bias) {
+#pragma unroll
+                        for (int e = 0; e < 8; ++e) v[e] += p.bias[n0 + e];
+                    }
+                    if (q.rx) {
+                        const float* X = q.rx + m * 256 + n0;
+                        const f32x4 x0 = *reinterpret_cast<const f32x4*>(X), x1 = *reinterpret_cast<const f32x4*>(X + 4);
+#pragma unroll
+                        for (int e = 0; e < 4; ++e) {
+                            v[e] += ln_affine(x0[e], mu, rs, q.rg[n0 + e], q.rb[n0 + e]);
+                            v[4 + e] += ln_affine(x1[e], mu, rs, q.rg[n0 + 4 + e], q.rb[n0 + 4 + e]);
+                        }
+                    } else if (p.res) {
+                        const float* R = p.res + m * p.ldr + n0;
+                        const f32x4 r0 = *reinterpret_cast<const f32x4*>(R), r1 = *reinterpret_cast<const f32x4*>(R + 4);
+#pragma unroll
+                        for (int e = 0; e < 4; ++e) { v[e] += r0[e]; v[4 + e] += r1[e]; }
+                    }
+                    float* sp = stage + (wm * 16 + fr) * St::ls32 + n0;
+                    *reinterpret_cast<f32x4*>(sp) = f32x4{v[0], v[1], v[2], v[3]};
+                    *reinterpret_cast<f32x4*>(sp + 4) = f32x4{v[4], v[5], v[6], v[7]};
+                }
+            }
+            __syncthreads();
+#pragma unroll
+            for (int i = 0; i < NI; ++i) {
+                const int j = wave + i * NW;
+                const int lrj = block_row(j, mt);
+                if (lrj < 0) continue;
+                const int64_t row = bm + lrj;
+                ln.take_staged(stage + j * St::ls32, pv[i]);
+                ln.t[0].store(C + row * p.ldc + LnOwner<1>::col(0));
+                ln.stats(1.f, 256);
+                if (lane == 0) { q.mean[row] = ln.mu; q.rstd[row] = ln.rs; }
+                ln.store(row, q.y32, y, ypos, 256, nullptr);
+            }
+            __syncthreads();
+        }
+    } else {
+        h16_t* stage = reinterpret_cast<h16_t*>(smem);
+        using Rows = LnBwdRows<h16_t, float, 1, 1>;
+        Rows ln{q.dy32, stage, nullptr, q.x, q.mean, q.rstd, 256};
+        ln.init(q.gamma);
+        h16_t* dx = reinterpret_cast<h16_t*>(q.dx);
+#pragma unroll
+        for (int mt = 0; mt < 4; ++mt) {
+            typename Rows::Row cur, nxt;
+            bool have = false;
+            {
+                const int lr0 = block_row(wave, mt);
+                if (lr0 >= 0) { ln.fetch_global(bm + lr0, cur); have = true; }
+            }
+            const int lr = (t0 + mt) * 16 + fr;
+            const int64_t m = bm + lr;
+            if (mt < cnt && lr < rows) {
+#pragma unroll
+                for (int pr = 0; pr < 4; ++pr) {
+                    const int n0 = wn * 128 + pr * 32 + fq * 8;
+                    h16x8 o;
+#pragma unroll
+                    for (int e = 0; e < 8; ++e) o[e] = (h16_t)acc[2 * pr + (e >> 2)][mt][e & 3];
+                    if (p.C) *reinterpret_cast<h16x8*>(reinterpret_cast<h16_t*>(p.C) + m * p.ldc + n0) = o;
+                    *reinterpret_cast<h16x8*>(stage + (wm * 16 + fr) * St::ls16 + n0) = o;
+                }
+            }
+            __syncthreads();
+#pragma unroll
+            for (int i = 0; i < NI; ++i) {
+                const int j = wave + i * NW;
+                const int lrj = block_row(j, mt);
+                if (lrj < 0) continue;
+                const int64_t row = bm + lrj;
+                if (!have) ln.fetch_global(row, cur);
+                const int lrn = i + 1 < NI ? block_row(j + NW, mt) : -1;
+                if (lrn >= 0) ln.fetch_global(bm + lrn, nxt);
+                ln.take_staged(stage + j * St::ls16, cur);
+                ln.row(cur, row, q.dx32, dx, 0.f, 1.f, 0, nullptr);
+                cur = nxt;
+                have = lrn >= 0;
+            }
+            __syncthreads();
+        }
+        float* const sinks[3] = {q.dgamma, q.dbeta, q.dxsum};
+        ln_fold_columns<NW>(reinterpret_cast<float*>(smem), ln.acc, sinks, 256);
+    }
+}
+
+template <bool OUT_F32, bool BAL, int EPI = 0>
+__device__ __forceinline__ void gemm_n256_body(const N256Args& p, const LnEpilogue* q = nullptr) {
+    static_assert(EPI == 0 || OUT_F32 == (EPI == 1), "the forward rows are fp32, the backward's dy is 16-bit");
     using R = Ring<BAL>;
     constexpr int STG = R::stg;
     __shared__ __attribute__((aligned(1024))) char smem[R::bytes];
@@ -170,6 +311,10 @@
     for (; kt + STG <= nk; kt += STG) ring_pass<0, STG>(step, kt);
     ring_tail<0, STG>(step, kt, nk);
 
+    if constexpr (EPI != 0) {
+        n256_ln_epilogue<OUT_F32, BAL>(p, *q, acc, smem, bm, rows, ntile, t0, cnt);
+        return;
+    }
 #pragma unroll
     for (int mt = 0; mt < 4; ++mt) {
         const int lr = (t0 + mt) * 16 + fr;
@@ -217,6 +362,10 @@
 __global__ __launch_bounds__(256, 2) void gemm_n256_bf16_b16(N256Args p) { gemm_n256_body<false, false>(p); }
 __global__ __launch_bounds__(512, 2) void gemm_n256_bal_bf16_f32(N256Args p) { gemm_n256_body<true, true>(p); }
 __global__ __launch_bounds__(512, 2) void gemm_n256_bal_bf16_b16(N256Args p) { gemm_n256_body<false, true>(p); }
+__global__ __launch_bounds__(256, 2) void gemm_n256_bf16_lnf(N256Args p, LnEpilogue q) { gemm_n256_body<true, false, 1>(p, &q); }
+__global__ __launch_bounds__(256, 2) void gemm_n256_bf16_lnb(N256Args p, LnEpilogue q) { gemm_n256_body<false, false, 2>(p, &q); }
+__global__ __launch_bounds__(512, 2) void gemm_n256_bal_bf16_lnf(N256Args p, LnEpilogue q) { gemm_n256_body<true, true, 1>(p, &q); }
+__global__ __launch_bounds__(512, 2) void gemm_n256_bal_bf16_lnb(N256Args p, LnEpilogue q) { gemm_n256_body<false, true, 2>(p, &q); }
 
 }
 
@@ -229,9 +378,10 @@
     return n;
 }
 
-static int n256_plan(const GemmCall& c, N256Args& p, dim3& grid, bool& bal) {
+static int n256_plan(const GemmCall& c, N256Args& p, dim3& grid, bool& bal, bool any_size = false) {
     const int64_t M = c.M, N = c.N, K = c.K;
-    if (N % BN || K % BK || K < 512 || M < 4096) return SVOL_E_UNSUPPORTED;
+    if (N % BN || K % BK || M < 1) return SVOL_E_UNSUPPORTED;
+    if (!any_size && (K < 512 || M < 4096)) return SVOL_E_UNSUPPORTED;
     if (c.epi != 0 || c.pre || c.colscale) return SVOL_E_UNSUPPORTED;
     if (c.kwrap != K && (c.kwrap % BK || 2 * c.kwrap != K)) return SVOL_E_UNSUPPORTED;
     if (c.act != SVOL_ACT_NONE && ((c.act != SVOL_ACT_GELU && c.act != SVOL_ACT_RELU) || c.out_f32)) return SVOL_E_UNSUPPORTED;
@@ -260,3 +410,17 @@
     else hipLaunchKernelGGL(c.out_f32 ? gemm_n256_bf16_f32 : gemm_n256_bf16_b16, grid, dim3(256), 0, c.stream, p);
     return hipGetLastError() == hipSuccess ? SVOL_OK : SVOL_E_LAUNCH;
 }
+
+int svol_gemm_n256_ln_bf16(const GemmCall& c, const LnEpilogue& e, bool backward, bool any_size) {
+    if (c.N != BN || c.ldc != BN || c.act != SVOL_ACT_NONE || (c.out_f32 != 0) == backward || svol_deterministic()) return SVOL_E_UNSUPPORTED;
+    if (backward ? (c.bias || c.res) : (c.res && e.rx)) return SVOL_E_UNSUPPORTED;
+    if (c.res && c.ldr != BN) return SVOL_E_UNSUPPORTED;
+    N256Args p; dim3 grid; bool bal;
+    GemmCall g = c;
+    if (!g.C) g.C = const_cast<void*>(c.A);
+    if (const int rc = n256_plan(g, p, grid, bal, any_size)) return rc;
+    p.C = c.C;
+    if (bal) hipLaunchKernelGGL(backward ? gemm_n256_bal_bf16_lnb : gemm_n256_bal_bf16_lnf, grid, dim3(512), 0, c.stream, p, e);
+    else hipLaunchKernelGGL(backward ? gemm_n256_bf16_lnb : gemm_n256_bf16_lnf, grid, dim3(256), 0, c.stream, p, e);
+    return hipGetLastError() == hipSuccess ? SVOL_OK : SVOL_E_LAUNCH;
+}
diff --git a/svol_amd/csrc/ln_row.h b/svol_amd/csrc/ln_row.h
--- a/svol_amd/csrc/ln_row.h
+++ b/svol_amd/csrc/ln_row.h
@@ -34,6 +34,11 @@
     }
 };
 
+__device__ __forceinline__ float ln_affine(float x, float mu, float rs, float g, float b) {
+#pragma clang fp contract(off)
+    return __builtin_fmaf((x - mu) * rs, g, b);
+}
+
 template <typename T, int NP>
 struct LnFwdRow {
     using Own = LnOwner<1>;
@@ -61,6 +66,15 @@
             }
         }
     }
+    __device__ __forceinline__ void load_affine(const float* __restrict__ gamma, const float* __restrict__ beta) {
+        static_assert(NP == 1, "staged rows are one pass wide");
+        gv[0].load(gamma + Own::col(0));
+        bv[0].load(beta + Own::col(0));
+    }
+    __device__ __forceinline__ void take_staged(const float* xs, const Vec4<T>& posv) {
+        t[0].load(xs + Own::col(0));
+        pv[0] = posv;
+    }
     __device__ __forceinline__ void stats(float scale, int D) {
 #pragma clang fp contract(off)
         float s = 0.f;
@@ -95,7 +109,7 @@
                 Vec4<float> o32;
 #pragma unroll
                 for (int e = 0; e < 4; ++e) {
-                    const float r = __builtin_fmaf((v[j][e] - mu) * rs, gv[j].get(e), bv[j].get(e));
+                    const float r = ln_affine(v[j][e], mu, rs, gv[j].get(e), bv[j].get(e));
                     o.set(e, r);
                     o32.set(e, r);
                     op.set(e, r + pv[j].get(e));
@@ -147,6 +161,14 @@
         r.mu = mean[row];
         r.rs = rstd[row];
     }
+    __device__ __forceinline__ void fetch_global(int64_t row, Row& r) const {
+        static_assert(NP == 1 && WPR == 1, "staged rows are one pass wide, one wave per row");
+        if (dy32) r.a32[0].load(dy32 + row * D + Own::col(0));
+        r.xv[0].load(x + row * D + Own::col(0));
+        r.mu = mean[row];
+        r.rs = rstd[row];
+    }
+    __device__ __forceinline__ void take_staged(const T* dys, Row& r) const { r.a[0].load(dys + Own::col(0)); }
     __device__ __forceinline__ void row(const Row& cur, int64_t row, float* __restrict__ dx32, T* __restrict__ dx, float p, float inv_keep,
                                         uint64_t seed, float (*slot)[4]) {
 #pragma clang fp contract(off)
@@ -232,4 +254,33 @@
     }
 }
 
-}
+template <int NW, int K, int NP>
+__device__ __forceinline__ void ln_fold_columns(float* red, const float (&part)[K][NP][4], float* const (&sink)[K], int D) {
+    using Own = LnOwner<1>;
+    const int wave = threadIdx.x >> 6;
+    for (int w = 0; w < NW; ++w) {
+        if (wave == w) {
+#pragma unroll
+            for (int j = 0; j < NP; ++j) {
+                const int c = Own::col(j);
+                if (c < D) {
+#pragma unroll
+                    for (int e = 0; e < 4; ++e)
+#pragma unroll
+                        for (int k = 0; k < K; ++k) {
+                            if (w == 0) red[k * NP * 256 + c + e] = part[k][j][e];
+                            else red[k * NP * 256 + c + e] += part[k][j][e];
+                        }
+                }
+            }
+        }
+        __syncthreads();
+    }
+    for (int c = threadIdx.x; c < D; c += 64 * NW) {
+#pragma unroll
+        for (int k = 0; k < K; ++k)
+            if (sink[k]) atomicAdd(sink[k] + c, red[k * NP * 256 + c]);
+    }
+}
+
+}
```

New measurement: 15500 (median of 6 runs). No clear change (+1.0%).
